# lijx10/DeepI2P

Measured on AMD Instinct MI355X. Metric: frames/sec (img+pc infer + 60-restart GN pose) KITTI 20k-pt, 1/2/4/8 GPU, higher is better.
Workload: dtype f32 network (fp32-input MFMA; 3x3 convolutions, GEMM-shaped point layers and the per-point head: bf16 MFMA on exact three-way fp32 splits, fp32 accumulation) + f64 solver

## Files before the change

### deepi2p_amd/_lib.py

```python
import ctypes
import os

import torch

_HERE = os.path.dirname(os.path.abspath(__file__))
LIB_PATH = os.environ.get("DI2P_LIB") or os.path.join(_HERE, "lib", "libdeepi2p_hip.so")
_lib = None

c_void_p, c_int, c_float, c_double, c_ll = ctypes.c_void_p, ctypes.c_int, ctypes.c_float, ctypes.c_double, ctypes.c_longlong


class DeepI2PHipError(RuntimeError):
    pass


class SrcT(ctypes.Structure):
    _fields_ = [("ptr", c_void_p), ("gidx", c_void_p), ("batch_stride", c_ll), ("row_stride", c_int),
                ("channels", c_int), ("mode", c_int), ("group", c_int), ("pad_", c_int)]


class EpilogueT(ctypes.Structure):
    _fields_ = [("scale", c_void_p), ("shift", c_void_p), ("batch_bias", c_void_p), ("relu", c_int),
                ("group_max", c_int), ("g_table", c_void_p * 2), ("g_idx", c_void_p * 2), ("g_w", c_void_p * 2),
                ("g_nodes", c_int * 2), ("g_k", c_int * 2), ("transpose_out", c_int), ("group_max_out", c_void_p),
                ("planes_out", c_void_p)]


class HeadX3T(ctypes.Structure):
    _fields_ = [("src", c_void_p * 2), ("batch_stride", c_ll * 2), ("row_stride", c_int * 2), ("channels", c_int * 2),
                ("W0p", c_void_p), ("W1p", c_void_p), ("scale_shift", c_void_p), ("relu0", c_int), ("relu1", c_int),
                ("tab", c_void_p * 2), ("idx", c_void_p * 2), ("w", c_void_p * 2), ("nodes", c_int * 2),
                ("W2t", c_void_p), ("scale2", c_void_p), ("shift2", c_void_p), ("relu2", c_int), ("P", c_int)]


class HeadLabelsX3T(ctypes.Structure):
    _fields_ = [("y0", c_void_p), ("batch_stride", c_ll), ("row_stride", c_int), ("K", c_int),
                ("W1p", c_void_p), ("scale1", c_void_p), ("shift1", c_void_p), ("relu1", c_int),
                ("W2p", c_void_p), ("scale2", c_void_p), ("shift2", c_void_p), ("P", c_int),
                ("scores", c_void_p), ("coarse", c_void_p), ("fine", c_void_p)]


class SampleOptT(ctypes.Structure):
    _fields_ = [("mode", c_int), ("crop_top", c_int), ("img_scale", c_double), ("img_H", c_int), ("img_W", c_int), ("Hs", c_int), ("Ws", c_int),
                ("amplitude", c_double * 6), ("color_range", c_double * 8)]
    dataset, crop_bottom, resize_k, max_range = 0, 0, 0, 0.0


SRC_DENSE, SRC_GATHER, SRC_GROUP = 0, 1, 2

_SIGS = {
    "di2p_index_max_forward": [c_void_p, c_void_p, c_void_p, c_int, c_int, c_int, c_int, c_void_p, c_void_p],
    "di2p_index_max_values": [c_void_p, c_void_p, c_void_p, c_void_p, c_void_p, c_int, c_int, c_int, c_int, c_void_p, c_void_p],
    "di2p_ball_query_forward": [c_void_p, c_void_p, c_float, c_int, c_int, c_int, c_int, c_void_p],
    "di2p_knn_nodes": [c_void_p, c_void_p, c_void_p, c_void_p, c_int, c_int, c_int, c_int, c_void_p],
    "di2p_cluster_stats": [c_void_p, c_void_p, c_int, c_void_p, c_void_p, c_void_p, c_int, c_int, c_int, c_void_p],
    "di2p_build_point_input": [c_void_p] * 7 + [c_int, c_int, c_int, c_void_p],
    "di2p_interpolate": [c_void_p] * 4 + [c_int] * 5 + [c_void_p],
    "di2p_gather_neighbors": [c_void_p] * 4 + [c_int] * 4 + [c_void_p],
    "di2p_argmax_channels": [c_void_p, c_void_p, c_int, c_int, c_int, c_ll, c_void_p],
    "di2p_pointwise_gemm": [ctypes.POINTER(SrcT), c_int, c_void_p, c_void_p, c_int, c_int, c_int, c_int,
                            ctypes.POINTER(EpilogueT), c_void_p],
    "di2p_pointwise_gemm_x3": [ctypes.POINTER(SrcT), c_int, c_void_p, c_void_p, c_int, c_int, c_int, c_int,
                               ctypes.POINTER(EpilogueT), c_void_p],
    "di2p_pointwise_gemm_x3p": [c_void_p, c_void_p, c_void_p, c_int, c_int, c_int, c_int, ctypes.POINTER(EpilogueT), c_void_p],
    "di2p_bf16x3_pack": [c_void_p, c_int, c_int, c_void_p, c_void_p],
    "di2p_bf16x3_pack_conv3x3": [c_void_p, c_int, c_int, c_int, c_void_p, c_void_p],
    "di2p_batch_gemv": [c_void_p, c_int, c_int, c_void_p, c_int, c_void_p, c_int, c_void_p],
    "di2p_batch_gemv2": [c_void_p, c_int, c_int, c_void_p, c_int, c_int, c_void_p, c_int, c_void_p, c_int, c_void_p],
    "di2p_attention_pool": [c_void_p, c_void_p, c_void_p, c_int, c_int, c_int, c_int, c_void_p],
    "di2p_point_head": [c_void_p, c_int, c_void_p, c_int, c_void_p, c_void_p, c_void_p, c_void_p, c_int, c_void_p, c_void_p,
                        c_void_p, c_int, c_void_p, c_int, c_int, c_int, c_int, c_void_p],
    "di2p_point_chain": [c_void_p, c_int, c_void_p, c_int, c_void_p, c_void_p, c_void_p, c_void_p, c_int, c_void_p, c_void_p,
                         c_void_p, c_int, c_void_p, c_int, c_int, c_int, c_void_p],
    "di2p_conv2d": [c_void_p] * 6 + [c_int] * 11 + [c_void_p],
    "di2p_conv2d_ws": [c_void_p] * 6 + [c_int] * 11 + [c_void_p, c_ll, c_void_p],
    "di2p_maxpool3x3s2": [c_void_p, c_void_p, c_int, c_int, c_int, c_int, c_void_p],
    "di2p_global_avgpool": [c_void_p, c_void_p, c_int, c_int, c_int, c_void_p],
    "di2p_channel_max": [c_void_p, c_void_p, c_int, c_int, c_int, c_void_p],
    "di2p_initial_guess": [c_void_p] * 5 + [c_int, c_int, c_void_p],
    "di2p_solve_batched": [c_void_p] * 6 + [c_double, c_double, ctypes.POINTER(c_double), ctypes.POINTER(c_double)]
                          + [c_int] * 5 + [c_void_p, c_void_p, c_void_p, c_void_p, c_void_p, c_void_p],
    "di2p_solve_batched_f32": [c_void_p] * 6 + [c_double, c_double, ctypes.POINTER(c_double), ctypes.POINTER(c_double)]
                              + [c_int] * 5 + [c_void_p, c_void_p, c_void_p, c_void_p, c_void_p, c_void_p],
    "di2p_select_best": [c_void_p, c_void_p, c_void_p, c_int, c_int, c_int, c_void_p, c_void_p, c_void_p, c_void_p],
    "di2p_solver_residuals": [c_void_p] * 4 + [c_double, c_double, c_int, c_int, c_int, c_void_p, c_void_p, c_void_p, c_void_p],
    "di2p_f32_to_f64": [c_void_p, c_void_p, c_ll, c_void_p],
    "di2p_farthest_point_sampling": [c_void_p, c_void_p, c_void_p, c_void_p, c_int, c_int, c_int, c_void_p],
    "di2p_gather_points": [c_void_p, c_void_p, c_void_p, c_int, c_int, c_int, c_int, c_void_p],
    "di2p_project_labels": [c_void_p, c_void_p, c_int, c_void_p, c_float, c_float, c_float, c_void_p, c_void_p, c_void_p, c_int, c_int, c_void_p],
    "di2p_label_accuracy": [c_void_p, c_void_p, c_void_p, c_void_p, c_void_p, c_int, c_int, c_void_p],
    "di2p_pnp_ransac": [c_void_p] * 5 + [c_int, c_void_p, c_int, c_double, c_int, c_int, c_int, c_int] + [c_void_p] * 7,
    "di2p_draw_restarts": [ctypes.c_ulonglong, c_int, c_int, c_double, c_double, c_void_p, c_void_p, c_void_p],
    "di2p_random_choice": [ctypes.c_ulonglong, c_int, c_int, c_int, c_int, c_void_p, c_void_p, c_void_p],
    "di2p_random_choice_ragged": [ctypes.c_ulonglong, c_int, c_int, c_void_p, c_int, c_int, c_void_p, c_void_p, c_void_p],
    "di2p_voxel_down_sample": [c_void_p, c_void_p, c_int, c_int, c_int, c_double, c_double, c_int] + [c_void_p] * 9,
    "di2p_estimate_normals": [c_void_p, c_int, c_int, c_double, c_int, c_double] + [c_void_p] * 5,
    "di2p_nearest_raw": [c_void_p, c_void_p, c_void_p, c_int, c_int, c_double] + [c_void_p] * 5,
    "di2p_gather_ragged": [c_void_p] * 6 + [c_int, c_int] + [c_void_p] * 4,
    "di2p_pnp_pack": [c_void_p] * 4 + [c_int, c_int, c_int] + [c_void_p] * 3,
    "di2p_pnp_ransac_epnp": [c_void_p] * 5 + [c_int, c_void_p, c_int, c_double, c_int, c_int] + [c_void_p] * 7,
    "di2p_classifier_loss": [c_void_p] * 4 + [c_int, c_int, c_int, c_float, c_float, c_float] + [c_void_p] * 5,
    "di2p_adam_step": [c_void_p] * 4 + [c_ll, c_int, c_float, c_float, c_float, c_float, c_void_p],
    "di2p_pack_pc_label": [c_void_p, c_void_p, c_void_p, c_void_p, c_void_p, c_void_p, c_int, c_int, c_void_p],
    "di2p_stem_pack": [c_void_p, c_void_p, c_void_p],
    "di2p_conv7x7s2_stem": [c_void_p] * 5 + [c_int] * 4 + [c_void_p],
    "di2p_winograd_weight_transform": [c_void_p, c_void_p, c_int, c_int, c_void_p],
    "di2p_winograd_weight_transform_dgrad": [c_void_p, c_void_p, c_int, c_int, c_void_p],
    "di2p_conv3x3_winograd": [c_void_p] * 6 + [c_int] * 6 + [c_void_p],
    "di2p_conv3x3_x3": [c_void_p] * 6 + [c_int] * 7 + [c_void_p] * 4 + [c_int, c_void_p],
    "di2p_conv3x3_x3_supported": [c_int] * 7,
    "di2p_conv3x3_x3_plan": [c_int] * 7 + [ctypes.POINTER(ctypes.c_int32)],
    "di2p_head_x3_pack": [c_void_p, c_int, c_void_p, c_void_p],
    "di2p_stem_x3_pack": [c_void_p, c_void_p, c_void_p],
    "di2p_stem_x3_supported": [c_int, c_int],
    "di2p_stem_x3": [c_void_p] * 5 + [c_int] * 3 + [c_void_p],
    "di2p_point_head_x3": [ctypes.POINTER(HeadX3T), c_void_p, c_int, c_int, c_void_p],
    "di2p_head_labels_x3_pack": [c_void_p, c_int, c_int, c_void_p, c_void_p],
    "di2p_point_head_labels_x3": [ctypes.POINTER(HeadLabelsX3T), c_int, c_int, c_void_p],
    "di2p_bn_train_forward": [c_void_p] * 9 + [c_float, c_float, c_int, c_int, c_int, c_int, c_void_p, c_void_p],
    "di2p_bn_train_backward": [c_void_p] * 6 + [c_int] + [c_void_p] * 4 + [c_int, c_int, c_int, c_void_p, c_void_p],
    "di2p_channel_sum": [c_void_p, c_void_p, c_int, c_int, c_int, c_void_p, c_void_p],
    "di2p_bmm_rc": [c_void_p, c_ll, c_ll, c_void_p, c_ll, c_ll, c_void_p, c_int, c_int, c_int, c_int, c_float, c_int, c_void_p, c_ll, c_void_p],
    "di2p_rc_vec_ok": [c_void_p, c_ll, c_ll, c_int],
    "di2p_rc_route": [c_int] * 7 + [ctypes.POINTER(ctypes.c_int32)],
    "di2p_pointwise_route": [c_int] * 6 + [ctypes.POINTER(ctypes.c_int32)],
    "di2p_conv2d_route": [c_int] * 12 + [c_ll, ctypes.POINTER(ctypes.c_int32)],
    "di2p_winograd_route": [c_int] * 5 + [ctypes.POINTER(ctypes.c_int32)],
    "di2p_point_chain_route": [c_int] * 6 + [ctypes.POINTER(ctypes.c_int32)],
    "di2p_point_head_route": [c_int] * 8 + [ctypes.POINTER(ctypes.c_int32)],
    "di2p_bmm_km": [c_void_p, c_int, c_ll, c_void_p, c_int, c_ll, c_void_p, c_int, c_int, c_int, c_int, c_float, c_void_p],
    "di2p_gather_backward": [c_void_p, c_void_p, c_void_p, c_int, c_void_p, c_int, c_int, c_int, c_int, c_void_p, c_ll, c_void_p],
    "di2p_conv2d_wgrad": [c_void_p] * 3 + [c_int] * 9 + [c_void_p, c_ll, c_void_p],
    "di2p_conv2d_dgrad": [c_void_p] * 3 + [c_int] * 9 + [c_void_p],
    "di2p_maxpool3x3s2_backward": [c_void_p] * 3 + [c_int] * 4 + [c_void_p],
    "di2p_segment_max_backward": [c_void_p] * 4 + [c_int] * 4 + [c_void_p],
    "di2p_group_max_forward": [c_void_p, c_void_p, c_void_p, c_ll, c_int, c_void_p],
    "di2p_group_max_backward": [c_void_p, c_void_p, c_void_p, c_ll, c_int, c_void_p],
    "di2p_dropout_mask": [ctypes.c_ulonglong, c_int, c_float, c_ll, c_void_p, c_void_p],
    "di2p_apply_mask": [c_void_p, c_void_p, c_float, c_void_p, c_ll, c_void_p],
    "di2p_sample_draws": [ctypes.c_ulonglong, c_void_p, c_int, c_int, ctypes.POINTER(SampleOptT)] + [c_void_p] * 10,
    "di2p_image_prepare": [c_void_p, c_int, c_int, c_int, ctypes.POINTER(SampleOptT), c_void_p, c_void_p, c_int, c_int, c_int, c_void_p, c_void_p,
                           c_void_p],
    "di2p_transform_segments": [c_void_p] * 4 + [c_int, c_int] + [c_void_p] * 3,
    "di2p_gather_ragged_aug": [c_void_p] * 6 + [c_int, c_int, ctypes.c_ulonglong, c_void_p, c_int, c_double, c_double] + [c_void_p] * 4,
    "di2p_random_choice_dseed": [c_void_p, c_int, c_int, c_int, c_int, c_void_p, c_void_p, c_void_p],
    "di2p_random_choice_ragged_dseed": [c_void_p, c_int, c_int, c_void_p, c_int, c_int, c_void_p, c_void_p, c_void_p],
    "di2p_range_shuffle": [c_void_p, c_void_p, c_int, c_int, c_int, c_double, ctypes.c_ulonglong] + [c_void_p] * 6,
    "di2p_gather_ragged_aug_intensity": [c_void_p] * 5 + [c_int, c_int, ctypes.c_ulonglong, c_void_p, c_int, c_double, c_double] + [c_void_p] * 3,
    "di2p_sample_draws_ds": [ctypes.c_ulonglong, c_void_p, c_int, c_int, ctypes.POINTER(SampleOptT), c_int] + [c_void_p] * 10,
    "di2p_image_prepare_ds": [c_void_p, c_int, c_int, c_int, ctypes.POINTER(SampleOptT), c_int, c_int, c_void_p, c_void_p, c_void_p, c_int, c_int,
                              c_void_p, c_void_p, c_void_p],
    "di2p_estimate_normals_cells": [c_void_p, c_int, c_int, c_double, c_int, c_double] + [c_void_p] * 5,
    "di2p_compose_poses": [c_void_p, c_void_p, c_int, c_void_p, c_void_p],
    "di2p_pose_errors": [c_void_p, c_void_p, c_int, c_void_p, c_int, c_int, c_double, c_double, c_void_p, c_void_p, c_void_p, c_void_p],
    "di2p_eval_accumulate": [c_void_p] * 5 + [c_int, c_void_p, c_void_p],
    "di2p_eval_acc_reset": [c_void_p, c_void_p],
    "di2p_enu2cam_points": [c_void_p, c_void_p, c_int, c_int, c_void_p],
    "di2p_vis_classification": [c_void_p] * 6 + [c_int] * 10 + [c_void_p] * 3,
    "di2p_vis_registration": [c_void_p] * 5 + [c_int] * 7 + [c_void_p] * 3,
    "di2p_submap_build": [c_void_p] * 6 + [c_int] * 5 + [c_double, c_double, c_int] + [c_void_p] * 7,
    "di2p_submap_to_camera": [c_void_p] * 4 + [c_int, c_int, c_void_p, c_void_p],
    "di2p_pose_matrices": [c_void_p, c_int, c_void_p, c_void_p],
    "di2p_sweep_transforms": [c_void_p] * 5 + [c_int, c_int] + [c_void_p] * 3,
    "di2p_sweep_accumulate": [c_void_p] * 4 + [c_int] * 6 + [c_float, c_float] + [c_void_p] * 6,
    "di2p_world_trace": [c_void_p, c_void_p, c_int, c_int, c_void_p, c_void_p, c_int, c_void_p, c_void_p, c_void_p],
    "di2p_world_render_camera": [c_void_p, c_void_p, c_int, c_int, c_void_p, c_void_p, c_int, c_int, c_double] + [c_void_p] * 4,
    "di2p_world_render_scan": [c_void_p, c_void_p, c_int, c_int, c_void_p, c_void_p, c_void_p, c_int, c_int] + [c_double] * 4
                              + [ctypes.c_ulonglong, c_void_p, c_int] + [c_void_p] * 5,
    "di2p_world_render_profiles": [c_void_p, c_void_p, c_int, c_int, c_void_p, c_void_p, c_void_p, c_int, c_int] + [c_double] * 4
# ... 24 lines not shown
    "di2p_world_workspace_bytes": [c_int, c_int],
    "di2p_world_profiles_workspace_bytes": [c_int, c_int],
    "di2p_pose_information_workspace_bytes": [c_int, c_int],
}
EXPORTS = sorted(list(_SIGS) + ["di2p_last_error", "di2p_version", "di2p_solve_workspace_bytes", "di2p_solver_set_profile_buffer", "di2p_pnp_workspace_bytes",
                 "di2p_conv2d_workspace_bytes", "di2p_set_option", "di2p_get_option", "di2p_random_choice_workspace_bytes", "di2p_classifier_loss_workspace_bytes", "di2p_normals_cells_candidates"] + list(_WS_SIGS))


def load():
    global _lib
    if _lib is None:
        if not os.path.exists(LIB_PATH):
            raise DeepI2PHipError(
                "libdeepi2p_hip.so not found at %s -- build it with `python -m deepi2p_amd.build` "
                "(there is no CPU fallback)" % LIB_PATH)
        lib = ctypes.CDLL(LIB_PATH)
        for name, args in _SIGS.items():
            fn = getattr(lib, name)
            fn.argtypes = args
            fn.restype = c_int
        lib.di2p_last_error.restype = ctypes.c_char_p
        lib.di2p_version.restype = c_int
        lib.di2p_solve_workspace_bytes.restype = c_ll
        lib.di2p_solve_workspace_bytes.argtypes = [c_int, c_int, c_int]
        lib.di2p_pnp_workspace_bytes.restype = c_ll
        lib.di2p_pnp_workspace_bytes.argtypes = [c_int, c_int, c_int]
        lib.di2p_conv2d_workspace_bytes.restype = c_ll
        lib.di2p_conv2d_workspace_bytes.argtypes = [c_int] * 10
        lib.di2p_classifier_loss_workspace_bytes.restype = c_ll
        lib.di2p_classifier_loss_workspace_bytes.argtypes = [c_int, c_int]
        lib.di2p_random_choice_workspace_bytes.restype = c_ll
        lib.di2p_random_choice_workspace_bytes.argtypes = [c_int, c_int]
        for name, args in _WS_SIGS.items():
            fn = getattr(lib, name)
            fn.argtypes = args
            fn.restype = c_ll
        lib.di2p_normals_cells_candidates.restype = c_int
        lib.di2p_normals_cells_candidates.argtypes = []
        lib.di2p_set_option.restype = c_int
        lib.di2p_set_option.argtypes = [ctypes.c_char_p, c_ll]
        lib.di2p_get_option.restype = c_ll
        lib.di2p_get_option.argtypes = [ctypes.c_char_p]
        lib.di2p_solver_set_profile_buffer.restype = None
        lib.di2p_solver_set_profile_buffer.argtypes = [c_void_p]
        _lib = lib
    return _lib


TIMED = None
TIMED_TAG = None
WORK = None


def call(name, *args):
    lib = load()
    rec = TIMED is not None and name in TIMED
    if rec:
        e0, e1 = torch.cuda.Event(enable_timing=True), torch.cuda.Event(enable_timing=True)
        e0.record()
    rc = getattr(lib, name)(*args)
    if rec:
        e1.record()
        TIMED[name].append((e0, e1, TIMED_TAG))
    if rc != 0:
        raise DeepI2PHipError("%s failed (%d): %s" % (name, rc, lib.di2p_last_error().decode()))


def set_option(name, value):
    if load().di2p_set_option(name.encode(), int(value)) != 0:
        raise DeepI2PHipError("unknown option " + name)


def get_option(name):
    return int(load().di2p_get_option(name.encode()))


class option:

    def __init__(self, name, value):
        self.name, self.value = name, value

    def __enter__(self):
        self.old = get_option(self.name)
        set_option(self.name, self.value)

    def __exit__(self, *exc):
        set_option(self.name, self.old)


def ptr(t):
    return None if t is None else t.data_ptr()


def stream():
    return torch.cuda.current_stream().cuda_stream


def require_cuda(*tensors):
    for t in tensors:
        if t is None:
            continue
        if not t.is_cuda:
            raise RuntimeError("tensor must be a CUDA tensor/variable")
        if not t.is_contiguous():
            raise RuntimeError("tensor must be contiguous")
```

### deepi2p_amd/csrc/common.h

```cpp
#pragma once
#include <hip/hip_runtime.h>
#include <stdint.h>
#include <stdio.h>

#include "../../include/deepi2p_hip.h"

#define DI2P_WAVE 64

void di2p_set_error(const char* fmt, ...);

#define DI2P_CHECK_ARG(cond, msg)                                   \
    do {                                                            \
        if (!(cond)) {                                              \
            di2p_set_error("%s: %s", __func__, msg);                \
            return -1;                                              \
        }                                                           \
    } while (0)

#define DI2P_RETURN_LAUNCH()                                                        \
    do {                                                                            \
        hipError_t e_ = hipGetLastError();                                          \
        if (e_ != hipSuccess) {                                                     \
            di2p_set_error("%s: launch failed: %s", __func__, hipGetErrorString(e_)); \
            return (int)e_;                                                         \
        }                                                                           \
        return 0;                                                                   \
    } while (0)

static inline int di2p_cdiv(long long a, long long b) { return (int)((a + b - 1) / b); }

#define DI2P_OPTIONS(X) \
    X(CONV_NOSPLIT, "conv_nosplit", "DI2P_CONV_NOSPLIT", 0)                        \
    X(CONV_DEPTH1, "conv_depth1", "DI2P_CONV_DEPTH1", 0)                           \
    X(PW_NOVEC, "pw_novec", "DI2P_PW_NOVEC", 0)                                    \
    X(SOLVER_NOCULL, "solver_nocull", "DI2P_SOLVER_NOCULL", 0)                     \
    X(SOLVER_NOPREFILTER, "solver_noprefilter", "DI2P_SOLVER_NOPREFILTER", 0)      \
    X(SOLVER_TIER_SWEEPS, "solver_tier_sweeps", "DI2P_SOLVER_TIER_SWEEPS", 0)      \
    X(WINO_COB, "wino_cob", "DI2P_WINO_COB", 0)                                    \
    X(CONV_NOWINOGRAD, "conv_nowinograd", "DI2P_CONV_NOWINOGRAD", 0)               \
    X(WINO_KC, "wino_kc", "DI2P_WINO_KC", 0)                                       \
    X(CONV_NOSTEM, "conv_nostem", "DI2P_CONV_NOSTEM", 0)                           \
    X(WINO_REG, "wino_reg", "DI2P_WINO_REG", 0)                                    \
    X(SOLVER_NOCACHE, "solver_nocache", "DI2P_SOLVER_NOCACHE", 0)                  \
    X(SOLVER_PREP_SINGLE, "solver_prep_single", "DI2P_SOLVER_PREP_SINGLE", 0)      \
    X(SOLVER_PREP_BITONIC, "solver_prep_bitonic", "DI2P_SOLVER_PREP_BITONIC", 0)   \
    X(PW_X3, "pw_x3", "DI2P_PW_X3", 1)                                             \
    X(PW_NOCHAIN, "pw_nochain", "DI2P_PW_NOCHAIN", 0)                              \
    X(HEAD_REG, "head_reg", "DI2P_HEAD_REG", 0)                                    \
    X(CONV_S2SCALAR, "conv_s2scalar", "DI2P_CONV_S2SCALAR", 0)                     \
    X(CONV_X3, "conv_x3", "DI2P_CONV_X3", 31)                                      \
    X(CONV_X3_CFG, "conv_x3_cfg", "DI2P_CONV_X3_CFG", -1)                          \
    X(HEAD_X3, "head_x3", "DI2P_HEAD_X3", 1)                                       \
    X(HEAD_X3_TAB, "head_x3_tab", "DI2P_HEAD_X3_TAB", 1)                           \
    X(STEM_X3, "stem_x3", "DI2P_STEM_X3", 1)                                       \
    X(BN_UNFUSED, "bn_unfused", "DI2P_BN_UNFUSED", 0)                              \
    X(PW_X3_PLANES, "pw_x3_planes", "DI2P_PW_X3_PLANES", 1)                        \
    X(CONV_DGRAD_DENSE, "conv_dgrad_dense", "DI2P_CONV_DGRAD_DENSE", 0)            \
    X(RC_TILE64, "rc_tile64", "DI2P_RC_TILE64", 0)
enum Di2pOption {
#define DI2P_OPT_ENUM(ID, NAME, ENV, DEF) DI2P_OPT_##ID,
    DI2P_OPTIONS(DI2P_OPT_ENUM)
#undef DI2P_OPT_ENUM
    DI2P_OPT_COUNT
};
long long di2p_opt(int id);
int di2p_cu_count();
int di2p_allow_dynamic_lds(const void* kernel, size_t bytes, const char* who);
void di2p_pack_a32(const float* Wt, int K, int M, int tiles, int tile_stride, int step_stride, void* Wp, void* stream);
```

### deepi2p_amd/csrc/gemm.hip

```cpp
#include "bf16x3.h"
#include "mfma_tile.h"

#include <stdint.h>
#include <stdlib.h>

namespace {

struct LoaderWt {
    const float* Wt;
    int K, M;
    __device__ __forceinline__ float load(int k, int m) const { return (k < K && m < M) ? Wt[k * M + m] : 0.0f; }
};

struct SrcDev {
    const float* ptr[DI2P_MAX_SRC];
    const int* gidx[DI2P_MAX_SRC];
    long long batch_stride[DI2P_MAX_SRC];
    int row_stride[DI2P_MAX_SRC];
    int c_end[DI2P_MAX_SRC];
    int mode[DI2P_MAX_SRC];
    int group[DI2P_MAX_SRC];
    int n_src;
};

// ... 400 lines not shown
    __syncthreads();
    {
        LoaderWt4 la{tl.W1t, HEAD_M, HEAD_M};
        EpiDev e1{};
        e1.scale = tl.sc1; e1.shift = tl.sh1; e1.relu = tl.relu1; e1.group_max = 1;
        EpiPointwise ep{e1, nullptr, b, HEAD_M, N};
        ep.lds_tile = hbuf; ep.lds_n0 = j_blk; ep.lds_ld = HEAD_BN;
        mfma_gemm_block_blds<HeadCfg>(stage, la, hbuf, HEAD_BN, ep, HEAD_M, 0, j_blk);
    }
    __syncthreads();
    const int lane = threadIdx.x & 63, p = threadIdx.x >> 6;
    const int n = j_blk + lane;
    if (p < tl.P) {
        float a = 0.0f;
        for (int k0 = 0; k0 < HEAD_M; k0 += 16) {
            float w[16], h[16];
#pragma unroll
            for (int u = 0; u < 16; ++u) { w[u] = tl.W2t[(k0 + u) * tl.P + p]; h[u] = hbuf[(k0 + u) * HEAD_BN + lane]; }
#pragma unroll
            for (int u = 0; u < 16; ++u) a = fmaf(w[u], h[u], a);
        }
        if (tl.sc2) a *= tl.sc2[p];
        if (tl.sh2) a += tl.sh2[p];
        if (tl.relu2) a = fmaxf(a, 0.0f);
        if (n < N) out[((long long)b * tl.P + p) * N + n] = a;
    }
}

struct ChainTail {
    const float* W1t;
    const float* sc1;
    const float* sh1;
    const float* W2t;
    const float* sc2;
    const float* sh2;
    int relu1, relu2;
};

__device__ __forceinline__ void chain_rows_to_ksteps(const float (&v)[16], float* f) {
#pragma unroll
    for (int g = 0; g < 4; ++g) {
        auto p = __builtin_amdgcn_permlane32_swap(__float_as_uint(v[4 * g + 0]), __float_as_uint(v[4 * g + 1]), false, false);
        auto q = __builtin_amdgcn_permlane32_swap(__float_as_uint(v[4 * g + 2]), __float_as_uint(v[4 * g + 3]), false, false);
        f[4 * g + 0] = __uint_as_float(p[0]);
        f[4 * g + 1] = __uint_as_float(q[0]);
        f[4 * g + 2] = __uint_as_float(p[1]);
        f[4 * g + 3] = __uint_as_float(q[1]);
    }
}

#ifndef DI2P_CHAIN_WAVES
#define DI2P_CHAIN_WAVES 2
#endif
template <int M, int KS0, int NL, int TN>
__global__ __launch_bounds__(256) __attribute__((amdgpu_waves_per_eu(DI2P_CHAIN_WAVES, 8))) void point_chain_kernel(const float* __restrict__ X, long long x_bs, int x_rs, const float* __restrict__ W0t,
                                                           int K0, EpiDev e0, ChainTail tl, float* __restrict__ Y, int N, int nblk, int total) {
    constexpr int TM = M / 32, KS = M / 2, KSMAX = KS0 > KS ? KS0 : KS;
    extern __shared__ __attribute__((aligned(16))) float lds[];
    float* w0 = lds;
    float* w1 = w0 + 2 * KS0 * M;
    float* w2 = w1 + M * M;
    float* ss = w2 + (NL == 3 ? M * M : 0);
    for (int i = threadIdx.x; i < 2 * KS0 * M; i += 256) w0[i] = i < K0 * M ? W0t[i] : 0.0f;
    for (int i = threadIdx.x; i < M * M; i += 256) w1[i] = tl.W1t[i];
    if (NL == 3)
        for (int i = threadIdx.x; i < M * M; i += 256) w2[i] = tl.W2t[i];
    {
        const float* rows[6] = {e0.scale, e0.shift, tl.sc1, tl.sh1, NL == 3 ? tl.sc2 : nullptr, NL == 3 ? tl.sh2 : nullptr};
#pragma unroll
        for (int q = 0; q < 6; ++q)
            if (rows[q] && threadIdx.x < M) ss[q * M + threadIdx.x] = rows[q][threadIdx.x];
    }
    __syncthreads();
    if (e0.scale) e0.scale = ss;
    if (e0.shift) e0.shift = ss + M;
    const int lane = threadIdx.x & 63, wave = __builtin_amdgcn_readfirstlane(threadIdx.x >> 6);
    const int l31 = lane & 31, half = lane >> 5;
    EpiDev e1{}, e2{};
    e1.scale = tl.sc1 ? ss + 2 * M : nullptr; e1.shift = tl.sh1 ? ss + 3 * M : nullptr; e1.relu = tl.relu1; e1.group_max = 1;
    e2.scale = tl.sc2 ? ss + 4 * M : nullptr; e2.shift = tl.sh2 ? ss + 5 * M : nullptr; e2.relu = tl.relu2; e2.group_max = 1;

    float fn[TN][KS0];
    auto request = [&](int g) {
        const int fb = g / nblk, blk = g - fb * nblk;
        const float* Xb = X + (long long)fb * x_bs;
#pragma unroll
        for (int s = 0; s < KS0; ++s) {
            const int k = 2 * s + half;
#pragma unroll
            for (int j = 0; j < TN; ++j) {
                const float x = Xb[(long long)min(k, K0 - 1) * x_rs + min((blk * TN + j) * 32 + l31, N - 1)];
                fn[j][s] = k < K0 ? x : 0.0f;
            }
        }
    };
    const int g0 = blockIdx.x * 4 + wave, stride = gridDim.x * 4;
    if (g0 < total) request(g0);
    for (int g = g0; g < total; g += stride) {
        const int b = g / nblk, blk = g - b * nblk;
        EpiPointwise ep0{e0, nullptr, b, M, N}, ep1{e1, nullptr, b, M, N}, ep2{e2, nullptr, b, M, N};
        int n[TN], nc[TN];
#pragma unroll
        for (int j = 0; j < TN; ++j) { n[j] = (blk * TN + j) * 32 + l31; nc[j] = min(n[j], N - 1); }
        float f[TN][KSMAX];
#pragma unroll
        for (int j = 0; j < TN; ++j)
#pragma unroll
            for (int s = 0; s < KS0; ++s) f[j][s] = fn[j][s];
        request(min(g + stride, total - 1));
        f32x16 acc[TM][TN];
        auto zero = [&]() {
#pragma unroll
            for (int i = 0; i < TM; ++i)
#pragma unroll
                for (int j = 0; j < TN; ++j)
#pragma unroll
                    for (int r = 0; r < 16; ++r) acc[i][j][r] = 0.0f;
        };
        auto layer = [&](const float* w, auto ks_tag) {
            constexpr int STEPS = decltype(ks_tag)::value;
            const float* wl = w + half * M + l31;
#pragma unroll
            for (int s = 0; s < STEPS; ++s) {
                float a[TM];
#pragma unroll
                for (int i = 0; i < TM; ++i) a[i] = wl[2 * s * M + i * 32];
#pragma unroll
                for (int i = 0; i < TM; ++i)
#pragma unroll
                    for (int j = 0; j < TN; ++j) acc[i][j] = __builtin_amdgcn_mfma_f32_32x32x2f32(a[i], f[j][s], acc[i][j], 0, 0, 0);
            }
        };
        auto to_operands = [&](const EpiPointwise& ep) {
#pragma unroll
            for (int j = 0; j < TN; ++j)
#pragma unroll
                for (int i = 0; i < TM; ++i) {
                    float v[16];
                    ep.apply(i * 32 + 4 * half, nc[j], acc[i][j], v);
                    chain_rows_to_ksteps(v, &f[j][i * 16]);
                }
        };
        auto to_memory = [&](const EpiPointwise& ep) {
#pragma unroll
            for (int j = 0; j < TN; ++j)
#pragma unroll
                for (int i = 0; i < TM; ++i) {
                    float v[16];
                    ep.apply(i * 32 + 4 * half, nc[j], acc[i][j], v);
                    if (n[j] < N) {
#pragma unroll
                        for (int r = 0; r < 16; ++r)
                            Y[((long long)b * M + i * 32 + 4 * half + (r & 3) + 8 * (r >> 2)) * N + n[j]] = v[r];
                    }
                }
        };
        zero();
        layer(w0, std::integral_constant<int, KS0>{});
        to_operands(ep0);
        zero();
        layer(w1, std::integral_constant<int, KS>{});
        if (NL == 3) {
// ... 145 lines not shown
    const float* score;
    int HW, Mn, n;
    bool valid;
    __device__ __forceinline__ void column(int j) { n = j; valid = j < Mn; }
    __device__ __forceinline__ void begin_tile(int) {}
    __device__ __forceinline__ float load(int k) const { return (valid && k < HW) ? score[(long long)k * Mn + n] : 0.0f; }
};
struct EpiMean {
    float* out;
    int C, Mn;
    float inv_div;
    __device__ __forceinline__ void tile(int mrow0, int n, const f32x16& acc) {
        if (n >= Mn) return;
#pragma unroll
        for (int r = 0; r < 16; ++r) {
            const int m = mrow0 + (r & 3) + 8 * (r >> 2);
            if (m < C) out[(long long)m * Mn + n] = acc[r] / inv_div;
        }
    }
};
template <class Cfg>
__global__ __launch_bounds__(Cfg::THREADS) void attention_pool_kernel(const float* __restrict__ feat, const float* __restrict__ score,
                                                                       float* __restrict__ out, int C, int HW, int Mn) {
    extern __shared__ float lds[];
    const int b = blockIdx.z;
    LoaderFeat la{feat + (long long)b * C * HW, HW, C};
    LoaderScore lb{score + (long long)b * HW * Mn, HW, Mn, 0, false};
    EpiMean ep{out + (long long)b * C * Mn, C, Mn, (float)HW};
    mfma_gemm_block<Cfg>(lds, la, lb, ep, HW, blockIdx.y * Cfg::BM, blockIdx.x * Cfg::BN);
}

__device__ __forceinline__ float gemv_slice(const float* __restrict__ Wt, int M, int mc, int k0, const float* __restrict__ vb, int Kv, int slice) {
    const int per = (Kv + 3) / 4;
    const int kb = slice * per, ke = min(kb + per, Kv);
    float a0 = 0.0f, a1 = 0.0f, a2 = 0.0f, a3 = 0.0f;
    int k = kb;
    for (; k + 3 < ke; k += 4) {
        a0 += Wt[(long long)(k0 + k) * M + mc] * vb[k];
        a1 += Wt[(long long)(k0 + k + 1) * M + mc] * vb[k + 1];
        a2 += Wt[(long long)(k0 + k + 2) * M + mc] * vb[k + 2];
        a3 += Wt[(long long)(k0 + k + 3) * M + mc] * vb[k + 3];
    }
    for (; k < ke; ++k) a0 += Wt[(long long)(k0 + k) * M + mc] * vb[k];
    return (a0 + a1) + (a2 + a3);
}

__global__ __launch_bounds__(256) void batch_gemv_kernel(const float* __restrict__ Wt, int M, int k0, const float* __restrict__ v,
                                                         int Kv, int k1, const float* __restrict__ v1, int Kv1,
                                                         float* __restrict__ out) {
    __shared__ float part[2][4][64];
    const int b = blockIdx.y;
    const int lane = threadIdx.x & 63, slice = threadIdx.x >> 6;
    const int m = blockIdx.x * 64 + lane;
    const int mc = min(m, M - 1);
    part[0][slice][lane] = gemv_slice(Wt, M, mc, k0, v + (long long)b * Kv, Kv, slice);
    if (v1) part[1][slice][lane] = gemv_slice(Wt, M, mc, k1, v1 + (long long)b * Kv1, Kv1, slice);
    __syncthreads();
    if (slice == 0 && m < M) {
        float r = (part[0][0][lane] + part[0][1][lane]) + (part[0][2][lane] + part[0][3][lane]);
        if (v1) r += (part[1][0][lane] + part[1][1][lane]) + (part[1][2][lane] + part[1][3][lane]);
        out[(long long)b * M + m] = r;
    }
}

template <class Cfg>
void launch_pw(const SrcDev& s, const float* Wt, float* Y, int B, int M, int K, int N, const EpiDev& e, hipStream_t st) {
    const dim3 grid(di2p_cdiv(N, Cfg::BN), di2p_cdiv(M, Cfg::BM), B);
    hipLaunchKernelGGL(pointwise_gemm_kernel<Cfg>, grid, dim3(Cfg::THREADS), Cfg::LDS_FLOATS * sizeof(float), st, s, Wt, Y, M, K, N, e);
}

template <class Cfg>
void launch_pw_vec(bool dense, bool d2, const SrcDev& s, const float* Wt, float* Y, int B, int M, int K, int N, const EpiDev& e, hipStream_t st) {
    const dim3 grid(di2p_cdiv(N, Cfg::BN), di2p_cdiv(M, Cfg::BM), B);
    if (dense && d2)
        hipLaunchKernelGGL((pointwise_gemm_vec_kernel<Cfg, true, true>), grid, dim3(Cfg::THREADS), Cfg::LDS_FLOATS * sizeof(float), st, s, Wt, Y, M, K, N, e);
    else if (dense)
        hipLaunchKernelGGL((pointwise_gemm_vec_kernel<Cfg, true>), grid, dim3(Cfg::THREADS), Cfg::LDS_FLOATS * sizeof(float), st, s, Wt, Y, M, K, N, e);
    else if (d2)
        hipLaunchKernelGGL((pointwise_gemm_vec_kernel<Cfg, false, true>), grid, dim3(Cfg::THREADS), Cfg::LDS_FLOATS * sizeof(float), st, s, Wt, Y, M, K, N, e);
    else
        hipLaunchKernelGGL((pointwise_gemm_vec_kernel<Cfg, false>), grid, dim3(Cfg::THREADS), Cfg::LDS_FLOATS * sizeof(float), st, s, Wt, Y, M, K, N, e);
}


constexpr int X3_BM = 128, X3_BN = 128, X3_BK = 32, X3_KG = X3_BK / 8;


__device__ __forceinline__ void x3_clear(f32x16 (&acc)[2][2]) {
#pragma unroll
    for (int i = 0; i < 2; ++i)
#pragma unroll
        for (int j = 0; j < 2; ++j)
#pragma unroll
            for (int r = 0; r < 16; ++r) acc[i][j][r] = 0.0f;
}

__device__ __forceinline__ void x3_aload(const u32x4_t* __restrict__ Wp, int Mp, int kg, int row, u32x4_t (&af)[2][3]) {
#pragma unroll
    for (int i = 0; i < 2; ++i) {
        const u32x4_t* p = Wp + ((long long)kg * Mp + row + i * 32) * 3;
#pragma unroll
        for (int q = 0; q < 3; ++q) af[i][q] = p[q];
    }
}

__device__ __forceinline__ void x3_bfrag(const u32x2_t* bq, int sub, int half, int n, u32x4_t (&bf)[2][3]) {
// ... 516 lines not shown
    const HeadRoute rt = head_route(K0, n_src, srcs[0].channels, reg_range, e.g_table[0] && e.g_table[1] && e.g_k[0] == 3 && e.g_k[1] == 3, B, N,
                                    di2p_cu_count());
    if (rt.reg) {
        constexpr int KS0 = 48;
        const int nblk = rt.nblk;
        const long long total = rt.total;
        DI2P_CHECK_ARG(total < (1ll << 30), "too many column blocks");
        const int wgs = rt.wgs;
        const size_t lds_reg = (size_t)(2 * KS0 * HEAD_M + HEAD_M * HEAD_M + HEAD_M * 4 + 4 * HEAD_M) * sizeof(float);
        if (rt.g33) {
            if (di2p_allow_dynamic_lds((const void*)point_head_reg_kernel<true, KS0>, lds_reg, __func__)) return -1;
            hipLaunchKernelGGL((point_head_reg_kernel<true, KS0>), dim3(wgs), dim3(512), lds_reg, (hipStream_t)stream, s, W0t, K0, e, tl, out, N, nblk, (int)total);
        } else {
            if (di2p_allow_dynamic_lds((const void*)point_head_reg_kernel<false, KS0>, lds_reg, __func__)) return -1;
            hipLaunchKernelGGL((point_head_reg_kernel<false, KS0>), dim3(wgs), dim3(512), lds_reg, (hipStream_t)stream, s, W0t, K0, e, tl, out, N, nblk, (int)total);
        }
        DI2P_RETURN_LAUNCH();
    }
    const size_t lds = (HeadCfg::LDS_FLOATS + HEAD_M * HEAD_BN) * sizeof(float);
    if (rt.g33) {
        if (di2p_allow_dynamic_lds((const void*)point_head_kernel<true>, lds, __func__)) return -1;
        hipLaunchKernelGGL(point_head_kernel<true>, dim3(di2p_cdiv(N, HEAD_BN), B), dim3(HeadCfg::THREADS), lds, (hipStream_t)stream, s, W0t, K0, e, tl, out, N);
    } else {
        if (di2p_allow_dynamic_lds((const void*)point_head_kernel<false>, lds, __func__)) return -1;
        hipLaunchKernelGGL(point_head_kernel<false>, dim3(di2p_cdiv(N, HEAD_BN), B), dim3(HeadCfg::THREADS), lds, (hipStream_t)stream, s, W0t, K0, e, tl, out, N);
    }
    DI2P_RETURN_LAUNCH();
}

extern "C" int di2p_point_chain(const di2p_src_t* srcs, int n_src, const float* W0t, int K0, const di2p_epilogue_t* epi0,
                                const float* W1t, const float* scale1, const float* shift1, int relu1, const float* W2t,
                                const float* scale2, const float* shift2, int relu2, float* Y, int B, int M, int N, void* stream) {
    DI2P_CHECK_ARG(srcs && n_src == 1 && W0t && W1t && epi0, "fused chain: one dense source");
    DI2P_CHECK_ARG(M == 32 || M == 64, "fused chain: width 32 or 64 (use the separate layers otherwise)");
    DI2P_CHECK_ARG(K0 <= M, "fused chain: at most M input channels");
    DI2P_CHECK_ARG(B >= 0 && N >= 1 && K0 >= 1, "bad size");
    DI2P_CHECK_ARG(epi0->group_max <= 1 && !epi0->transpose_out && !epi0->planes_out, "fused chain: layer 0 takes scale/shift/relu/bias/gathered only");
    if (B == 0) return 0;
    DI2P_CHECK_ARG(Y && srcs[0].ptr && srcs[0].channels == K0 && srcs[0].mode == DI2P_SRC_DENSE, "fused chain: one dense source of K0 channels");
    DI2P_CHECK_ARG((long long)srcs[0].channels * srcs[0].row_stride < (1ll << 31), "per-frame source extent must fit 31 bits");
    EpiDev e;
    if (pw_epilogue(__func__, epi0, nullptr, M, N, false, e)) return -1;
    ChainTail tl{W1t, scale1, shift1, W2t, scale2, shift2, relu1, relu2};
    const float* X = srcs[0].ptr;
    const long long x_bs = srcs[0].batch_stride;
    const int x_rs = (int)srcs[0].row_stride;
    hipStream_t st = (hipStream_t)stream;
    const ChainRoute rt = chain_route(M, K0, W2t != nullptr, B, N, di2p_cu_count());
    DI2P_CHECK_ARG(rt.total < (1ll << 30), "too many column blocks");
#define DI2P_CHAIN_LAUNCH(MM, KS0, NL, TN)                                                                                          \
    do {                                                                                                                            \
        const size_t lds = (size_t)(2 * (KS0) * (MM) + ((NL) - 1) * (MM) * (MM) + 6 * (MM)) * sizeof(float);                        \
        hipLaunchKernelGGL((point_chain_kernel<MM, KS0, NL, TN>), dim3(rt.wgs), dim3(256), lds, st, X, x_bs, x_rs, W0t, K0, e, tl, Y, N, \
                           rt.nblk, (int)rt.total);                                                                                 \
    } while (0)
    const bool three = rt.layers == 3;
    if (M == 32) {
        if (rt.ks0 == 4) { if (three) DI2P_CHAIN_LAUNCH(32, 4, 3, DI2P_CHAIN_TN32); else DI2P_CHAIN_LAUNCH(32, 4, 2, DI2P_CHAIN_TN32); }
        else             { if (three) DI2P_CHAIN_LAUNCH(32, 16, 3, DI2P_CHAIN_TN32); else DI2P_CHAIN_LAUNCH(32, 16, 2, DI2P_CHAIN_TN32); }
    } else {
        if (rt.ks0 == 16) { if (three) DI2P_CHAIN_LAUNCH(64, 16, 3, DI2P_CHAIN_TN64); else DI2P_CHAIN_LAUNCH(64, 16, 2, DI2P_CHAIN_TN64); }
        else              { if (three) DI2P_CHAIN_LAUNCH(64, 32, 3, DI2P_CHAIN_TN64); else DI2P_CHAIN_LAUNCH(64, 32, 2, DI2P_CHAIN_TN64); }
    }
#undef DI2P_CHAIN_LAUNCH
    DI2P_RETURN_LAUNCH();
}

extern "C" int di2p_point_chain_route(int M, int K0, int layers, int B, int N, int cus, int32_t* out) {
    DI2P_CHECK_ARG(out && (M == 32 || M == 64) && K0 >= 1 && K0 <= M && (layers == 2 || layers == 3) && B >= 1 && N >= 1 && cus >= 1, "bad args");
    const ChainRoute rt = chain_route(M, K0, layers == 3, B, N, cus);
    DI2P_CHECK_ARG(rt.total < (1ll << 30), "too many column blocks");
    out[0] = M; out[1] = rt.ks0; out[2] = rt.layers; out[3] = rt.tn; out[4] = rt.nblk; out[5] = (int)rt.total; out[6] = rt.wgs; out[7] = rt.w;
    return 0;
}

extern "C" int di2p_point_head_route(int K0, int n_src, int c0, int reg_range, int g33, int B, int N, int cus, int32_t* out) {
    DI2P_CHECK_ARG(out && K0 >= 1 && n_src >= 1 && n_src <= DI2P_MAX_SRC && c0 >= 1 && c0 <= K0 && B >= 1 && N >= 4 && N % 4 == 0 && cus >= 1, "bad args");
    const HeadRoute rt = head_route(K0, n_src, c0, reg_range != 0, g33 != 0, B, N, cus);
    DI2P_CHECK_ARG(!rt.reg || rt.total < (1ll << 30), "too many column blocks");
    out[0] = rt.reg; out[1] = rt.g33; out[2] = rt.bn; out[3] = rt.nblk; out[4] = (int)rt.total; out[5] = rt.wgs;
    return 0;
}

extern "C" int di2p_batch_gemv(const float* Wt, int M, int k0, const float* v, int Kv, float* out, int B, void* stream) {
    DI2P_CHECK_ARG(Wt && v && out && M >= 1 && Kv >= 1 && k0 >= 0 && B >= 0, "bad args");
    if (B == 0) return 0;
    hipLaunchKernelGGL(batch_gemv_kernel, dim3(di2p_cdiv(M, 64), B), dim3(256), 0, (hipStream_t)stream, Wt, M, k0, v, Kv, 0,
                       (const float*)nullptr, 0, out);
    DI2P_RETURN_LAUNCH();
}

extern "C" int di2p_batch_gemv2(const float* Wt, int M, int k0, const float* v0, int Kv0, int k1, const float* v1, int Kv1,
                                float* out, int B, void* stream) {
    DI2P_CHECK_ARG(Wt && v0 && v1 && out && M >= 1 && Kv0 >= 1 && Kv1 >= 1 && k0 >= 0 && k1 >= 0 && B >= 0, "bad args");
    if (B == 0) return 0;
    hipLaunchKernelGGL(batch_gemv_kernel, dim3(di2p_cdiv(M, 64), B), dim3(256), 0, (hipStream_t)stream, Wt, M, k0, v0, Kv0, k1, v1, Kv1, out);
    DI2P_RETURN_LAUNCH();
}

extern "C" int di2p_attention_pool(const float* feat, const float* score, float* out, int B, int C, int HW, int Mn, void* stream) {
    DI2P_CHECK_ARG(feat && score && out && B >= 0 && C >= 1 && HW >= 1 && Mn >= 1, "bad args");
    if (B == 0) return 0;
    using Cfg = Cfg64x64;
    hipLaunchKernelGGL(attention_pool_kernel<Cfg>, dim3(di2p_cdiv(Mn, Cfg::BN), di2p_cdiv(C, Cfg::BM), B), dim3(Cfg::THREADS),
                       Cfg::LDS_FLOATS * sizeof(float), (hipStream_t)stream, feat, score, out, C, HW, Mn);
    DI2P_RETURN_LAUNCH();
}
```

### deepi2p_amd/csrc/head_x3.hip

```cpp
#include <stdint.h>

#include <type_traits>

#include "bf16x3.h"
#include "common.h"

namespace {

using bf16x3::u32x4_t;
using bf16x3::f32x16;

constexpr int HX_M = 128, HX_TM = 4, HX_TROW = HX_M + 4;

struct HxArgs {
    const float* src[2]; long long src_bs[2]; int src_rs[2]; int c0, K0;
    const u32x4_t* W0p; const u32x4_t* W1p;
    const float* ss;
    const float* tab[2]; const int* idx[2]; const float* gw[2]; int nodes[2];
    const float* W2t; const float* sc2; const float* sh2;
    float* out;
    int relu0, relu1, relu2, P, N, nblk, total, parts;
};

template <bool TAB_LDS, int KS0, int NW, int MINW, bool SYNC, bool DEEP, bool LEAN = false>
__global__ __launch_bounds__(NW * 64, MINW) void point_head_x3_kernel(const HxArgs a) {
    extern __shared__ __attribute__((aligned(16))) float lds[];
    float* ssl = lds;
    float* w2l = ssl + 4 * HX_M;
    float* tabl = w2l + 4 * HX_M;
    const int tid = threadIdx.x, lane = tid & 63, wave = __builtin_amdgcn_readfirstlane(tid >> 6);
    const int nl = lane & 31, h = lane >> 5;
    for (int i = tid; i < 4 * HX_M; i += NW * 64) {
        ssl[i] = a.ss[i];
        w2l[i] = (i & 3) < a.P ? a.W2t[(i >> 2) * a.P + (i & 3)] : 0.0f;
    }
    int g_first, g_stride, g_end, fb_fixed = 0;
    if (TAB_LDS) {
        const int fb = blockIdx.x / a.parts, part = blockIdx.x - fb * a.parts;
        fb_fixed = fb;
#pragma unroll
        for (int t = 0; t < 2; ++t) {
            const float* T = a.tab[t] + (long long)fb * a.nodes[t] * HX_M;
            float* L = tabl + (t == 0 ? 0 : a.nodes[0] * HX_TROW);
            for (int i = tid; i < a.nodes[t] * (HX_M / 4); i += NW * 64) {
                const int node = i / (HX_M / 4), c4 = i - node * (HX_M / 4);
                *reinterpret_cast<float4*>(L + node * HX_TROW + 4 * c4) = *reinterpret_cast<const float4*>(T + node * HX_M + 4 * c4);
            }
        }
        g_first = fb * a.nblk + part * NW + wave; g_stride = a.parts * NW; g_end = (fb + 1) * a.nblk;
    } else {
        g_first = blockIdx.x * NW + wave; g_stride = gridDim.x * NW; g_end = a.total;
    }
    __syncthreads();
    const __amdgpu_buffer_rsrc_t w0r = __builtin_amdgcn_make_buffer_rsrc((void*)a.W0p, 0, (a.K0 / 16) * HX_TM * 3 * 1024, 0x00020000);
    const __amdgpu_buffer_rsrc_t w1r = __builtin_amdgcn_make_buffer_rsrc((void*)a.W1p, 0, (HX_M / 16) * HX_TM * 3 * 1024, 0x00020000);

    int gi_n[6];
    float gw_n[6], x_n[KS0][8];
    const int trips = SYNC ? (g_end - (g_first - wave) + g_stride - 1) / g_stride : 0;
    for (int it = 0, g0 = g_first; SYNC ? it < trips : g0 < g_end; ++it, g0 += g_stride) {
        const bool live = g0 < g_end;
        const int g = SYNC ? min(g0, g_end - 1) : g0;
        asm volatile("" ::: "memory");
        int hq = 4 * h;
        asm volatile("" : "+v"(hq));
        const int fb = TAB_LDS ? fb_fixed : __builtin_amdgcn_readfirstlane(g / a.nblk);
        const int n = (g - fb * a.nblk) * 32 + nl, nc = min(n, a.N - 1);
        auto request_nb = [&](int gg, int (&gi_)[6], float (&gw_)[6]) __attribute__((always_inline)) {
            const int fq = TAB_LDS ? fb_fixed : __builtin_amdgcn_readfirstlane(gg / a.nblk);
            const int nq = min((gg - fq * a.nblk) * 32 + nl, a.N - 1);
#pragma unroll
            for (int t = 0; t < 2; ++t)
#pragma unroll
// ... 124 lines not shown
            for (int q2 = 0; q2 < 2; ++q2)
#pragma unroll
                for (int j = 0; j < 4; ++j) {
                    float X = v[8 * q2 + j], Y = v[8 * q2 + 4 + j];
                    asm volatile("s_nop 1\n\tv_permlane32_swap_b32 %0, %1" : "+v"(X), "+v"(Y));
                    f1[2 * i + q2][j] = X;
                    f1[2 * i + q2][4 + j] = Y;
                }
        }
#pragma unroll
        for (int i = 0; i < HX_TM; ++i)
#pragma unroll
            for (int r = 0; r < 16; ++r) acc[i][r] = 0.0f;
        {
            u32x4_t bfr[2][3];
            bf16x3::split8(f1[0], bfr[0][0], bfr[0][1], bfr[0][2]);
#pragma unroll
            for (int s = 0; s < 2 * HX_TM; ++s) {
                __builtin_amdgcn_sched_barrier(0);
                if (s + 1 < 2 * HX_TM) bf16x3::split8(f1[s + 1], bfr[(s + 1) & 1][0], bfr[(s + 1) & 1][1], bfr[(s + 1) & 1][2]);
                kstep(s & 1, bfr[s & 1], w1r, s + 1 < 2 * HX_TM ? s + 1 : -1);
#pragma unroll
                for (int u = 0; u < 6 * HX_TM; ++u) { __builtin_amdgcn_sched_group_barrier(0x008, 1, 0); __builtin_amdgcn_sched_group_barrier(0x002, 3, 0); }
            }
            __builtin_amdgcn_sched_barrier(0);
        }
        __builtin_amdgcn_sched_barrier(0);
        {
            const int gn = min(g + g_stride, g_end - 1);
            request_nb(gn, gi_n, gw_n);
#pragma unroll
            for (int s = 0; s < KS0; ++s) x_load(gn, s, x_n[s]);
        }
        __builtin_amdgcn_sched_barrier(0);
        float part[4] = {0.0f, 0.0f, 0.0f, 0.0f};
#pragma unroll
        for (int i = 0; i < HX_TM; ++i)
#pragma unroll
            for (int gq = 0; gq < 4; ++gq) {
                if (gq & 1) __builtin_amdgcn_sched_barrier(0);
                const int row = 32 * i + 8 * gq + hq;
                const float4 sc = *reinterpret_cast<const float4*>(ssl + 2 * HX_M + row);
                const float4 sh = *reinterpret_cast<const float4*>(ssl + 3 * HX_M + row);
                float y[4] = {acc[i][4 * gq + 0] * sc.x + sh.x, acc[i][4 * gq + 1] * sc.y + sh.y, acc[i][4 * gq + 2] * sc.z + sh.z, acc[i][4 * gq + 3] * sc.w + sh.w};
#pragma unroll
                for (int j = 0; j < 4; ++j) {
                    if (a.relu1) y[j] = fmaxf(y[j], 0.0f);
                    const float4 w = *reinterpret_cast<const float4*>(w2l + 4 * (row + j));
                    part[0] = fmaf(w.x, y[j], part[0]); part[1] = fmaf(w.y, y[j], part[1]);
                    part[2] = fmaf(w.z, y[j], part[2]); part[3] = fmaf(w.w, y[j], part[3]);
                }
                if (LEAN) asm volatile("" : "+v"(part[0]), "+v"(part[1]), "+v"(part[2]), "+v"(part[3]));
            }
#pragma unroll
        for (int p = 0; p < 4; ++p) {
            const float other = __builtin_bit_cast(float, __builtin_amdgcn_ds_bpermute((lane ^ 32) * 4, __builtin_bit_cast(int, part[p])));
            float o = (hq ? other : part[p]) + (hq ? part[p] : other);
            if (p < a.P) {
                if (a.sc2) o *= a.sc2[p];
                if (a.sh2) o += a.sh2[p];
                if (a.relu2) o = fmaxf(o, 0.0f);
                if (n < a.N && hq == 0 && live) a.out[((long long)fb * a.P + p) * a.N + n] = o;
            }
        }
    }
}

__global__ __launch_bounds__(256) void pack_a32_kernel(const float* __restrict__ Wt, unsigned short* __restrict__ Wp, int K, int M, int tiles,
                                                       int tile_stride, int step_stride) {
    const long long t = (long long)blockIdx.x * 256 + threadIdx.x;
    const int ks = K / 16;
    if (t >= (long long)tiles * ks * 64) return;
    const int lane = (int)(t & 63), s = (int)((t >> 6) % ks), tile = (int)((t >> 6) / ks);
    const int row = 32 * tile + (lane & 31), k0 = 16 * s + 8 * (lane >> 5);
    unsigned short* d = Wp + (((long long)tile * tile_stride + (long long)s * step_stride) * 3 * 64 + lane) * 8;
#pragma unroll
    for (int e = 0; e < 8; ++e) {
        const float v = row < M ? Wt[(long long)(k0 + e) * M + row] : 0.0f;
        float pl[3];
        bf16x3::split(v, pl[0], pl[1], pl[2]);
#pragma unroll
        for (int p = 0; p < 3; ++p) d[p * 64 * 8 + e] = bf16x3::bits(pl[p]);
    }
}

}

void di2p_pack_a32(const float* Wt, int K, int M, int tiles, int tile_stride, int step_stride, void* Wp, void* stream) {
    hipLaunchKernelGGL(pack_a32_kernel, dim3(di2p_cdiv((long long)tiles * (K / 16) * 64, 256)), dim3(256), 0, (hipStream_t)stream, Wt,
                       (unsigned short*)Wp, K, M, tiles, tile_stride, step_stride);
}

extern "C" long long di2p_head_x3_packed_bytes(int K) { return K >= 16 && K % 16 == 0 ? (long long)(K / 16) * HX_TM * 3 * 1024 : 0; }

extern "C" int di2p_head_x3_pack(const float* Wt, int K, void* Wp, void* stream) {
    DI2P_CHECK_ARG(Wt && Wp && K >= 16 && K % 16 == 0, "needs K % 16 == 0 (and 128 output channels)");
    DI2P_CHECK_ARG(((uintptr_t)Wp & 15) == 0, "packed weights must be 16-byte aligned");
    di2p_pack_a32(Wt, K, HX_M, HX_TM, 1, HX_TM, Wp, stream);
    DI2P_RETURN_LAUNCH();
}

extern "C" int di2p_point_head_x3(const di2p_head_x3_t* hd, float* out, int B, int N, void* stream) {
    DI2P_CHECK_ARG(hd && out, "null pointer");
    DI2P_CHECK_ARG(B >= 0 && N >= 1, "bad size");
    DI2P_CHECK_ARG(hd->src[0] && hd->src[1] && hd->W0p && hd->W1p && hd->scale_shift && hd->W2t, "null operand");
    DI2P_CHECK_ARG(hd->channels[0] >= 16 && hd->channels[0] % 16 == 0 && hd->channels[1] >= 16 && hd->channels[1] % 16 == 0, "source channels must be multiples of 16");
    DI2P_CHECK_ARG(hd->P >= 1 && hd->P <= 4, "1..4 outputs");
    for (int t = 0; t < 2; ++t) DI2P_CHECK_ARG(hd->tab[t] && hd->idx[t] && hd->nodes[t] >= 1, "both gathered tables (3 neighbours each) are required");
    DI2P_CHECK_ARG(((uintptr_t)hd->W0p & 15) == 0 && ((uintptr_t)hd->W1p & 15) == 0 && ((uintptr_t)hd->tab[0] & 15) == 0 && ((uintptr_t)hd->tab[1] & 15) == 0 &&
                   ((uintptr_t)hd->scale_shift & 15) == 0, "16-byte alignment of the packed weights, the tables and the scale / shift rows");
    for (int t = 0; t < 2; ++t)
        DI2P_CHECK_ARG((long long)hd->channels[t] * hd->row_stride[t] * 4 < (1ll << 31), "per-frame source extent must fit 31 bits");
    if (B == 0) return 0;
    HxArgs a{};
    for (int t = 0; t < 2; ++t) {
        a.src[t] = hd->src[t]; a.src_bs[t] = hd->batch_stride[t]; a.src_rs[t] = hd->row_stride[t];
        a.tab[t] = hd->tab[t]; a.idx[t] = hd->idx[t]; a.gw[t] = hd->w[t]; a.nodes[t] = hd->nodes[t];
    }
    a.c0 = hd->channels[0]; a.K0 = hd->channels[0] + hd->channels[1];
    a.W0p = (const u32x4_t*)hd->W0p; a.W1p = (const u32x4_t*)hd->W1p; a.ss = hd->scale_shift;
    a.W2t = hd->W2t; a.sc2 = hd->scale2; a.sh2 = hd->shift2; a.out = out;
    a.relu0 = hd->relu0; a.relu1 = hd->relu1; a.relu2 = hd->relu2; a.P = hd->P; a.N = N;
    a.nblk = di2p_cdiv(N, 32); a.total = B * a.nblk;
    hipStream_t st = (hipStream_t)stream;
    const size_t lds_small = (size_t)8 * HX_M * sizeof(float);
    const size_t lds_tab = lds_small + (size_t)(hd->nodes[0] + hd->nodes[1]) * HX_TROW * sizeof(float);
    const long long opt = di2p_opt(DI2P_OPT_HEAD_X3_TAB);
    DI2P_CHECK_ARG(a.K0 == 96, "this build instantiates the head for 96 dense channels (32 + 64: first_pointnet + second_pointnet)");
    if (opt != 0 && lds_tab <= 160 * 1024) {
        const int cus = di2p_cu_count();
        int parts = di2p_cdiv(cus, B);
        while (parts > 1 && a.nblk < parts * 16) --parts;
        a.parts = parts;
        if (opt == 2) {
            if (di2p_allow_dynamic_lds((const void*)point_head_x3_kernel<true, 6, 4, 1, false, true>, lds_tab, __func__)) return -1;
            hipLaunchKernelGGL((point_head_x3_kernel<true, 6, 4, 1, false, true>), dim3(B * parts), dim3(256), lds_tab, st, a);
        } else {
            if (di2p_allow_dynamic_lds((const void*)point_head_x3_kernel<true, 6, 8, 2, false, false, true>, lds_tab, __func__)) return -1;
            hipLaunchKernelGGL((point_head_x3_kernel<true, 6, 8, 2, false, false, true>), dim3(B * parts), dim3(512), lds_tab, st, a);
        }
    } else {
        const int grid = (int)(a.total / 4 < 1ll * di2p_cu_count() ? di2p_cdiv(a.total, 4) : di2p_cu_count());
        hipLaunchKernelGGL((point_head_x3_kernel<false, 6, 4, 1, false, true>), dim3(grid), dim3(256), lds_small, st, a);
    }
    DI2P_RETURN_LAUNCH();
}
```

### deepi2p_amd/csrc/solver_aux.hip

```cpp
#include "common.h"
#include "pose_diff.h"
#include "solver_model.h"

namespace {

__global__ __launch_bounds__(64) void select_best_kernel(const double* __restrict__ params, const double* __restrict__ cost,
                                                         const int* __restrict__ has_inside, int np, int R, int* __restrict__ best,
                                                         double* __restrict__ P, double* __restrict__ best_cost) {
    const int f = blockIdx.x, lane = threadIdx.x;
    double bc = __builtin_inf();
    int bi = 0x7fffffff;
    for (int r = lane; r < R; r += 64) {
        const double c = cost[(long long)f * R + r];
        if (c < bc || (c == bc && r < bi)) { bc = c; bi = r; }
    }
#pragma unroll
    for (int o = 32; o > 0; o >>= 1) {
        const double oc = __shfl_xor(bc, o);
        const int oi = __shfl_xor(bi, o);
        if (oc < bc || (oc == bc && oi < bi)) { bc = oc; bi = oi; }
    }
    if (lane != 0) return;
    double* Pf = P + (long long)f * 16;
    for (int i = 0; i < 16; ++i) Pf[i] = (i % 5 == 0) ? 1.0 : 0.0;
    if (has_inside && has_inside[f] == 0) {
        best[f] = -1;
        best_cost[f] = 1e4;
        return;
    }
    if (bi == 0x7fffffff) bi = 0;
    params_to_pose(params + ((long long)f * R + bi) * np, np, Pf);
    best[f] = bi;
    best_cost[f] = cost[(long long)f * R + bi];
}

__global__ __launch_bounds__(1024) void initial_guess_kernel(const double* __restrict__ points, const int* __restrict__ labels,
                                                             double* __restrict__ yaw0, int* __restrict__ labels_out,
                                                             int* __restrict__ has_inside, int N) {
    __shared__ double s_a[1024], s_b[1024], s_c[1024];
    const int f = blockIdx.x, tid = threadIdx.x;
    const double* px = points + (long long)f * 3 * N;
    const double* pz = px + 2 * (long long)N;
    const int* lab = labels + (long long)f * N;
    double sx = 0, sz = 0, cnt = 0;
    for (int n = tid; n < N; n += 1024)
        if (lab[n] == 1) { sx += px[n]; sz += pz[n]; cnt += 1.0; }
    s_a[tid] = sx; s_b[tid] = sz; s_c[tid] = cnt;
    __syncthreads();
    for (int o = 512; o > 0; o >>= 1) {
        if (tid < o) { s_a[tid] += s_a[tid + o]; s_b[tid] += s_b[tid + o]; s_c[tid] += s_c[tid + o]; }
        __syncthreads();
    }
    const double count = s_c[0];
    const double mx = s_a[0] / count, mz = s_b[0] / count;
    __syncthreads();
    if (!(count > 0.0)) {
        if (tid == 0) { yaw0[f] = 0.0; has_inside[f] = 0; }
        for (int n = tid; n < N; n += 1024) labels_out[(long long)f * N + n] = lab[n];
        return;
    }
    const double kPi = 3.14159265358979323846;
    double a = fmod(atan2(mz, mx) - kPi / 2 + kPi, 2 * kPi);
    if (a < 0) a += 2 * kPi;
    a -= kPi;
    const double c = cos(a), s = sin(a);
    double zmin = __builtin_inf();
    for (int n = tid; n < N; n += 1024)
        if (lab[n] == 1) zmin = fmin(zmin, -s * px[n] + c * pz[n]);
    s_a[tid] = zmin;
    __syncthreads();
    for (int o = 512; o > 0; o >>= 1) {
        if (tid < o) s_a[tid] = fmin(s_a[tid], s_a[tid + o]);
        __syncthreads();
    }
    const double thr = s_a[0] - 10.0;
    for (int n = tid; n < N; n += 1024) {
        const double zr = -s * px[n] + c * pz[n];
        labels_out[(long long)f * N + n] = zr > thr ? lab[n] : -1;
    }
    if (tid == 0) { yaw0[f] = a; has_inside[f] = 1; }
}

template <int NP>
__global__ __launch_bounds__(256) void residuals_kernel(const double* __restrict__ points, const int* __restrict__ labels,
                                                        const double* __restrict__ Kmat, const double* __restrict__ params, double H,
                                                        double W, int N, double* __restrict__ residuals, int* __restrict__ counts,
                                                        double* __restrict__ cost_out) {
    __shared__ int s_scan[256];
    __shared__ double s_cost[256];
    __shared__ int s_base;
    const int f = blockIdx.x, tid = threadIdx.x;
    const double* px = points + (long long)f * 3 * N;
    const int* lab = labels + (long long)f * N;
    const double* Kf = Kmat + (long long)f * 9;
    const Cam k{Kf[0], Kf[4], Kf[2], Kf[5], H - 1.0, W - 1.0};
    const double* x = params + (long long)f * NP;
    double xr[NP];
    for (int i = 0; i < NP; ++i) xr[i] = x[i];
    Rot<NP> rot;
    make_rot<NP>(xr, rot);
    double* out = residuals + (long long)f * 3 * N;
    if (tid == 0) s_base = 0;
    double cost = 0.0;
    __syncthreads();
    for (int n0 = 0; n0 < N; n0 += 256) {
        const int n = n0 + tid;
        int nr = 0;
        double rv[3] = {0, 0, 0};
        if (n < N && (lab[n] == 0 || lab[n] == 1)) {
            const Proj p = project_point<NP>(rot, xr, k, px[n], px[N + n], px[2 * (long long)N + n]);
            nr = lab[n] == 1 ? 3 : 1;
            residual_rows<false>(lab[n], p.pix_x, p.pix_y, p.p2, k, rv);
            const double s = rv[0] * rv[0] + rv[1] * rv[1] + rv[2] * rv[2];
            cost += 0.5 * log1p(s);
            const double sq = sqrt(1.0 / (1.0 + s));
            for (int i = 0; i < 3; ++i) rv[i] *= sq;
        }
        s_scan[tid] = nr;
        __syncthreads();
        for (int o = 1; o < 256; o <<= 1) {
            const int v = tid >= o ? s_scan[tid - o] : 0;
            __syncthreads();
            s_scan[tid] += v;
            __syncthreads();
        }
        const int excl = s_scan[tid] - nr + s_base;
        for (int i = 0; i < nr; ++i) out[excl + i] = rv[i];
        __syncthreads();
        if (tid == 255) s_base += s_scan[255];
        __syncthreads();
// ... 191 lines not shown
    }
    status[f] = st;
    sigma_t[f] = sqrt(tr_t);
    sigma_r[f] = sqrt(tr_r) * (180.0 / 3.14159265358979323846);
}

__global__ __launch_bounds__(64) void restart_consensus_kernel(const double* __restrict__ params, const double* __restrict__ cost,
                                                               const int* __restrict__ best, const int* __restrict__ has_inside, int np, int R,
                                                               double t_tol, double r_tol_deg, int* __restrict__ finite_out,
                                                               int* __restrict__ agree_out, double* __restrict__ gap) {
    const int f = blockIdx.x, lane = threadIdx.x;
    const int b = best[f];
    if ((has_inside && has_inside[f] == 0) || b < 0 || b >= R) {
        if (lane == 0) { finite_out[f] = 0; agree_out[f] = 0; gap[f] = __builtin_nan(""); }
        return;
    }
    double G[16], A[16];
    params_to_pose(params + ((long long)f * R + b) * np, np, G);
    int n_finite = 0, n_agree = 0;
    double other = __builtin_inf();
    for (int r = lane; r < R; r += 64) {
        const double c = cost[(long long)f * R + r];
        if (!isfinite(c)) continue;
        n_finite += 1;
        params_to_pose(params + ((long long)f * R + r) * np, np, A);
        double t, ang;
        di2p_pose_diff(A, G, t, ang);
        if (t < t_tol && ang < r_tol_deg) n_agree += 1;
        else other = fmin(other, c);
    }
#pragma unroll
    for (int o = 32; o > 0; o >>= 1) {
        n_finite += __shfl_xor(n_finite, o);
        n_agree += __shfl_xor(n_agree, o);
        other = fmin(other, __shfl_xor(other, o));
    }
    if (lane == 0) { finite_out[f] = n_finite; agree_out[f] = n_agree; gap[f] = other - cost[(long long)f * R + b]; }
}

}

extern "C" int di2p_select_best(const double* params, const double* cost, const int32_t* has_inside, int is_2d, int F, int R,
                                int32_t* best, double* P, double* best_cost, void* stream) {
    DI2P_CHECK_ARG(params && cost && best && P && best_cost && F >= 0 && R >= 1, "bad args");
    if (F == 0) return 0;
    hipLaunchKernelGGL(select_best_kernel, dim3(F), dim3(64), 0, (hipStream_t)stream, params, cost, has_inside, is_2d ? 4 : 6, R, best, P, best_cost);
    DI2P_RETURN_LAUNCH();
}

extern "C" int di2p_initial_guess(const double* points, const int32_t* labels, double* yaw0, int32_t* labels_out,
                                  int32_t* has_inside, int F, int N, void* stream) {
    DI2P_CHECK_ARG(points && labels && yaw0 && labels_out && has_inside && F >= 0 && N >= 0, "bad args");
    if (F == 0) return 0;
    hipLaunchKernelGGL(initial_guess_kernel, dim3(F), dim3(1024), 0, (hipStream_t)stream, points, labels, yaw0, labels_out, has_inside, N);
    DI2P_RETURN_LAUNCH();
}

extern "C" int di2p_solver_residuals(const double* points, const int32_t* labels, const double* K, const double* params, double H,
                                     double W, int is_2d, int F, int N, double* residuals, int32_t* counts, double* cost,
                                     void* stream) {
    DI2P_CHECK_ARG(points && labels && K && params && residuals && counts && cost && F >= 0 && N >= 0, "bad args");
    if (F == 0) return 0;
    if (is_2d)
        hipLaunchKernelGGL(residuals_kernel<4>, dim3(F), dim3(256), 0, (hipStream_t)stream, points, labels, K, params, H, W, N, residuals, counts, cost);
    else
        hipLaunchKernelGGL(residuals_kernel<6>, dim3(F), dim3(256), 0, (hipStream_t)stream, points, labels, K, params, H, W, N, residuals, counts, cost);
    DI2P_RETURN_LAUNCH();
}

static int info_chunks(int N) { return N > 0 ? (N + INFO_CHUNK - 1) / INFO_CHUNK : 1; }

extern "C" long long di2p_pose_information_workspace_bytes(int F, int N) {
    if (F < 0 || N < 0) return 0;
    return (long long)F * info_chunks(N) * INFO_STRIDE * (long long)sizeof(double);
}

extern "C" int di2p_pose_information(const float* points, const int32_t* labels, const double* K, const double* params, double H, double W,
                                     int is_2d, int F, int N, double* info, double* grad, double* cost, int32_t* active, void* workspace,
                                     void* stream) {
    DI2P_CHECK_ARG(F >= 0 && N >= 0, "bad size");
    if (F == 0) return 0;
    DI2P_CHECK_ARG(points && labels && K && params && info && grad && cost && active && workspace, "null pointer");
    const int C = info_chunks(N);
    DI2P_CHECK_ARG(C <= 65535, "N too large");
    double* partial = (double*)workspace;
    if (is_2d) {
        hipLaunchKernelGGL(info_partial_kernel<4>, dim3(F, C), dim3(256), 0, (hipStream_t)stream, points, labels, K, params, H, W, N, C, partial);
        hipLaunchKernelGGL(info_finish_kernel<4>, dim3(F), dim3(64), 0, (hipStream_t)stream, (const double*)partial, C, info, grad, cost, active);
    } else {
        hipLaunchKernelGGL(info_partial_kernel<6>, dim3(F, C), dim3(256), 0, (hipStream_t)stream, points, labels, K, params, H, W, N, C, partial);
        hipLaunchKernelGGL(info_finish_kernel<6>, dim3(F), dim3(64), 0, (hipStream_t)stream, (const double*)partial, C, info, grad, cost, active);
    }
    DI2P_RETURN_LAUNCH();
}

extern "C" int di2p_gather_best_params(const double* params, const int32_t* best, int is_2d, int F, int R, double* out, void* stream) {
    DI2P_CHECK_ARG(F >= 0 && R >= 1, "bad size (F >= 0, R >= 1)");
    if (F == 0) return 0;
    DI2P_CHECK_ARG(params && best && out, "null pointer");
    const int np = is_2d ? 4 : 6;
    hipLaunchKernelGGL(gather_best_kernel, dim3(di2p_cdiv((long long)F * np, 64)), dim3(64), 0, (hipStream_t)stream, params, best, F, R, np, out);
    DI2P_RETURN_LAUNCH();
}

extern "C" int di2p_pose_covariance(const double* info, const double* params, const int32_t* has_inside, const double* lb_host,
                                    const double* ub_host, int is_2d, int F, double* cov, int32_t* free_mask, int32_t* status, double* sigma_t,
                                    double* sigma_r, void* stream) {
// ... 23 lines not shown
```

### deepi2p_amd/networks.py

```python
import torch
import torch.nn as nn

from . import _lib, ops
from .ops import Src

BN_EPS = 1e-5


class _Holder(nn.Module):
    pass


def _register(root, key, tensor, is_buffer):
    parts = key.split(".")
    mod = root
    for p in parts[:-1]:
        if p not in mod._modules:
            mod.add_module(p, _Holder())
        mod = mod._modules[p]
    if is_buffer:
        mod.register_buffer(parts[-1], tensor)
    else:
        mod.register_parameter(parts[-1], nn.Parameter(tensor, requires_grad=False))

# ... 129 lines not shown
    return x


def _run_split_pn(dense_srcs, dense_rows, node_feats, node_rows, idx, layers, N):
    Wt, scale, shift, act = layers[0]
    M = Wt.shape[1]
    B = node_feats.shape[0]
    head = (Wt[dense_rows[0]:dense_rows[1]], scale, shift, act)
    chain = [head] + list(layers[1:])
    if ops.point_chain_ok(dense_srcs, chain, N):
        G = ops.pointwise_gemm([Src(node_feats)], Wt[node_rows[0]:node_rows[1]], M, node_feats.shape[2], transpose_out=True)
        return ops.point_chain(dense_srcs, chain, N, gathered=[(G, idx.reshape(B, N, 1), None)])
    x = _run_split_layer(dense_srcs, dense_rows, node_feats, node_rows, idx, layers[0], N)
    return _run_pn(x, layers[1:])


class PCEncoder(_PackedModule):
    def __init__(self, opt, Ca: int, Cb: int, Cg: int, prefix=""):
        super().__init__()
        self.opt, self.Ca, self.Cb, self.Cg = opt, Ca, Cb, Cg
        spec = (_pn_spec("first_pointnet", 7, [Ca // 2] * 3, True)
                + _pn_spec("second_pointnet", Ca, [Ca, Ca], True)
                + _c2d_spec("knnlayer.layers_before.0", 3 + Ca, Cb) + _c2d_spec("knnlayer.layers_before.1", Cb, Cb)
                + _c2d_spec("knnlayer.layers_after.0", 2 * Cb, 2 * Cb) + _c2d_spec("knnlayer.layers_after.1", 2 * Cb, Cb)
                + _pn_spec("final_pointnet", 3 + Cb, [Cg // 2, Cg], True))
        _materialise(self, spec)

    def _pack(self):
        if self._packed is None:
            sd = self._sd()
            p = {"first": _pn_pack(sd, "first_pointnet"), "second": _pn_pack(sd, "second_pointnet"),
                 "final": _pn_pack(sd, "final_pointnet")}
            for name in ("layers_before.0", "layers_before.1", "layers_after.0", "layers_after.1"):
                q = "knnlayer." + name
                p[name] = _fold(sd, q + ".conv", q + ".norm")
            self._packed = p
        return self._packed

    def _group_index(self, B, Mb, K, device):
        key = (B, Mb, K, str(device))
        cache = self.__dict__.setdefault("_gidx_cache", {})
        if key not in cache:
            cache[key] = (torch.arange(Mb * K, dtype=torch.int32, device=device) // K).unsqueeze(0).expand(B, -1).contiguous()
            torch.cuda.current_stream().synchronize()
        return cache[key]

    def forward_device(self, pc, intensity, sn, node_a, node_b):
        if pc.size(2) != self.opt.input_pt_num:
            raise RuntimeError("N must equal opt.input_pt_num (the reference bakes it in, networks_pc.py:44-45)")
        p = self._pack()
        B, N, Ma, Mb = pc.size(0), pc.size(2), node_a.size(2), node_b.size(2)
        idx_a, w_a = ops.knn_nodes(pc, node_a, self.opt.k_interp_point_a, want_weights=True)
        cluster_mean, mask, min_idx = ops.cluster_stats(pc, idx_a, Ma)
        pc_centers, aug = ops.build_point_input(pc, intensity, sn, cluster_mean, min_idx)
        first = _run_pn(aug, p["first"])
        _, first_max = ops.index_max(first, min_idx, Ma, return_values=True, mask=mask)
        Ch = first.shape[1]
        second = _run_split_pn([Src(first)], (0, Ch), first_max, (Ch, 2 * Ch), min_idx, p["second"], N)
        _, node_a_features = ops.index_max(second, min_idx, Ma, return_values=True, mask=mask)
        K = self.opt.k_ab
        knn_I = ops.knn_nodes(node_b, cluster_mean, K)
        coord = ops.gather_neighbors(cluster_mean, node_b, knn_I)
        y = _run_split_layer([Src(coord)], (0, 3), node_a_features, (3, 3 + node_a_features.shape[1]), knn_I.view(B, Mb * K),
                             p["layers_before.0"], Mb * K)
        pow2 = K & (K - 1) == 0 and K <= 32
        Cb1 = p["layers_before.1"][0].shape[1]
        pl = [pow2 and ops.x3_planes_link(p["layers_before.1"], p["layers_after.0"][0][Cb1:2 * Cb1], B, Mb * K),
              pow2 and ops.x3_planes_link(p["layers_after.0"], p["layers_after.1"][0], B, Mb * K)]
        if pow2:
            y, fmax = _run_layer([Src(y)], p["layers_before.1"], Mb * K, group_max=K, also_full=True, planes_out=pl[0])
            Cb = y.shape[1]
        else:
            y = _run_layer([Src(y)], p["layers_before.1"], Mb * K)
            Cb = y.shape[1]
            fmax = ops.channel_max(y.view(B, Cb * Mb, K)).view(B, Cb, Mb)
        y = _run_split_layer([y if pl[0] else Src(y)], (Cb, 2 * Cb), fmax, (0, Cb), self._group_index(B, Mb, K, pc.device), p["layers_after.0"], Mb * K,
                             planes_out=pl[1])
        if pow2:
            node_b_features = _run_layer([y if pl[1] else Src(y)], p["layers_after.1"], Mb * K, group_max=K)
        else:
            y = _run_layer([Src(y)], p["layers_after.1"], Mb * K)
            node_b_features = ops.channel_max(y.view(B, y.shape[1] * Mb, K)).view(B, y.shape[1], Mb)
        final = _run_layer([Src(node_b), Src(node_b_features)], p["final"][0], Mb)
        final = _run_pn(final, p["final"][1:])
        global_feature = ops.channel_max(final).unsqueeze(2)
        ref_tuple = (pc_centers, cluster_mean, idx_a, first, second, node_a_features, node_b_features, global_feature)
        return ref_tuple, dict(w_a=w_a, min_idx=min_idx, mask=mask, knn_I=knn_I)

    def forward(self, pc, intensity, sn, node_a, node_b):
        t, _ = self.forward_device(pc, intensity, sn, node_a, node_b)
        return t[0], t[1], t[2].long(), t[3], t[4], t[5], t[6], t[7]


def _block_conv3x3(blk, n, x, stride, residual=None):
    Wt, sc, sh, _ = blk["c" + n]
    Cout = Wt.shape[1]
    kernel, cfg = ops.conv_route(x.shape, (Cout, x.shape[1], 3, 3), stride, 1)
    if kernel == "x3" and stride == 2:
        _, sd_, shd, _ = blk["ds"]
        return ops.conv3x3_x3(x, blk["X" + n], Cout, sc, sh, 2, True, downsample=(blk["Xd"], sd_, shd), cfg=cfg)
    if kernel == "x3":
        return ops.conv3x3_x3(x, blk["X" + n], Cout, sc, sh, 1, True, residual=residual, cfg=cfg), None
    if kernel == "winograd":
        return ops.conv3x3_winograd(x, blk["U" + n], sc, sh, True, residual=residual), None
    return ops.conv2d(x, Wt, sc, sh, 3, 3, stride, 1, True, residual=residual, tap_major=True), None


class ImageEncoder(_PackedModule):
# ... 63 lines not shown
                identity = x
                if "ds" in blk:
                    Wd, sd_, shd, _ = blk["ds"]
                    identity = ops.conv2d(x, Wd, sd_, shd, 1, 1, blk["stride"], 0, False, tap_major=True)
            x, _ = _block_conv3x3(blk, "2", y, 1, identity)
            if blk["last_of_stage"]:
                stage_out[blk["stage"]] = x
        return stage_out[3], stage_out[4], ops.global_avgpool(stage_out[4])


class KeypointDetector(_PackedModule):
    fuse_head = True

    def __init__(self, opt):
        super().__init__()
        self.opt = opt
        self.pc_encoder = PCEncoder(opt, Ca=64, Cb=256, Cg=512)
        self.img_encoder = ImageEncoder(opt)
        self.H_fine_res = int(round(opt.img_H / opt.img_fine_resolution_scale))
        self.W_fine_res = int(round(opt.img_W / opt.img_fine_resolution_scale))
        L = self.H_fine_res * self.W_fine_res
        spec = (_pn_spec("node_b_attention_pn", 256 + 512, [256, L], False)
                + _pn_spec("node_b_pn", 256 + 512 + 512 + 512, [1024, 512, 512], False)
                + _pn_spec("node_a_attention_pn", 64 + 512, [256, L * 4], False)
                + _pn_spec("node_a_pn", 64 + 256 + 512, [512, 128, 128], False))
        if opt.is_fine_resolution:
            spec += _pn_spec("per_point_pn", 736, [256, 256, 2 + L], False)
        else:
            spec += _pn_spec("per_point_pn", 736, [128, 128, 2], False)
        _materialise(self, spec)

    def _pack(self):
        if self._packed is None:
            sd = {k: v for k, v in self.state_dict().items() if not k.startswith(("pc_encoder.", "img_encoder."))}
            p = {n: _pn_pack(sd, n) for n in ("node_b_attention_pn", "node_b_pn", "node_a_attention_pn", "node_a_pn", "per_point_pn")}
            Wt = p["node_b_pn"][0][0]
            p["node_b_pn_dense_Wt"] = torch.cat((Wt[0:256], Wt[768:1280]), dim=0).contiguous()
            l0, l1, l2 = p["per_point_pn"]
            if (l0[0].is_cuda and tuple(l0[0].shape) == (736, 128) and tuple(l1[0].shape) == (128, 128) and l2[0].shape[0] == 128
                    and l2[0].shape[1] <= 4 and not l0[0].requires_grad):
                ones = torch.ones(128, device=l0[0].device)
                p["head_x3"] = {"W0p": ops.head_x3_pack(l0[0][640:736].contiguous()), "W1p": ops.head_x3_pack(l1[0]),
                                "ss": torch.stack((l0[1] if l0[1] is not None else ones, l0[2], l1[1] if l1[1] is not None else ones, l1[2])).contiguous(),
                                "relu0": l0[3], "relu1": l1[3], "W2t": l2[0], "sc2": l2[1], "sh2": l2[2], "relu2": l2[3]}
            if (l0[0].is_cuda and l0[0].shape[1] == 256 and tuple(l1[0].shape) == (256, 256) and l2[0].shape[0] == 256 and l2[0].shape[1] >= 3
                    and not l2[3] and not l0[0].requires_grad):
                p["head_labels_x3"] = {"W1p": ops.head_labels_pack(l1[0]), "W2p": ops.head_labels_pack(l2[0]), "P": int(l2[0].shape[1]),
                                       "sc1": l1[1] if l1[1] is not None else torch.ones(256, device=l1[0].device), "sh1": l1[2],
                                       "relu1": l1[3], "sc2": l2[1], "sh2": l2[2]}
            self._packed = p
        return self._packed

    def forward(self, pc, intensity, sn, node_a, node_b, img):
        p, B, N, first, second, idx_a, idx_pb, gathered = self._trunk(pc, intensity, sn, node_a, node_b, img)
        Wt, sc, sh, act = p["per_point_pn"][0]
        M0 = Wt.shape[1]
        G_a, ex_w_a = gathered[0][0], gathered[0][2]
        G_b, w_pb = gathered[1][0], gathered[1][2]
        l1, l2 = p["per_point_pn"][1], p["per_point_pn"][2]
        if ("head_x3" in p and self.fuse_head and _lib.get_option("head_x3") and first.shape[1] == 32 and second.shape[1] == 64
                and idx_a.shape[-1] == 3 and idx_pb.shape[-1] == 3):
            scores = ops.point_head_x3(first, second, p["head_x3"],
                                       [(G_a, idx_a.reshape(B, N, 3), ex_w_a), (G_b, idx_pb.reshape(B, N, 3), w_pb)], N)
        elif M0 == 128 and l1[0].shape[1] == 128 and l2[0].shape[1] <= 4 and N % 4 == 0 and self.fuse_head:
            scores = ops.point_head([Src(first), Src(second)], (Wt[640:736], sc, sh, act), l1, l2, N, gathered=gathered)
        else:
            h = ops.pointwise_gemm([Src(first), Src(second)], Wt[640:736], M0, N, scale=sc, shift=sh, relu=act, gathered=gathered)
            scores = _run_pn(h, p["per_point_pn"][1:], x3=False if M0 == 128 else None)
        coarse = scores[:, 0:2, :]
        if self.opt.is_fine_resolution:
            return coarse, scores[:, 2:, :]
        return coarse

    def predict_labels(self, pc, intensity, sn, node_a, node_b, img, scores_out=None):
        if not self.opt.is_fine_resolution:
            return ops.argmax_channels(self.forward(pc, intensity, sn, node_a, node_b, img)), None
        p, B, N, first, second, idx_a, idx_pb, gathered = self._trunk(pc, intensity, sn, node_a, node_b, img)
        Wt, sc, sh, act = p["per_point_pn"][0]
        M0 = Wt.shape[1]
        h = ops.pointwise_gemm([Src(first), Src(second)], Wt[640:736], M0, N, scale=sc, shift=sh, relu=act, gathered=gathered)
        if "head_labels_x3" not in p:
            raise RuntimeError("predict_labels: the fine head has no labels-only kernel for per_point_pn %s"
                               % [tuple(l[0].shape) for l in p["per_point_pn"]])
        return ops.point_head_labels(h, p["head_labels_x3"], N, scores_out=scores_out)

    def _trunk(self, pc, intensity, sn, node_a, node_b, img):
        ops.require_cuda(pc, intensity, sn, node_a, node_b, img)
        p = self._pack()
        B, N, Ma, Mb = pc.size(0), pc.size(2), node_a.size(2), node_b.size(2)
        (pc_center, cluster_mean, idx_a, first, second, node_a_features, node_b_features, global_feature), ex = \
            self.pc_encoder.forward_device(pc, intensity, sn, node_a, node_b)
        s16, s32, iglob = self.img_encoder(img)
        s16f = s16.view(B, s16.size(1), -1)
        s32f = s32.view(B, s32.size(1), -1)
        ig = iglob.view(B, -1)
        gf = global_feature.view(B, -1)

        Wt, sc, sh, act = p["node_b_attention_pn"][0]
        h = ops.pointwise_gemm([Src(node_b_features)], Wt[0:256], Wt.shape[1], Mb, scale=sc, shift=sh, relu=act,
                               batch_bias=ops.batch_gemv(Wt, 256, ig))
        score_b = _run_pn(h, p["node_b_attention_pn"][1:])
        w_s32 = ops.attention_pool(s32f, score_b)
        Wt, sc, sh, act = p["node_b_pn"][0]
        bias = ops.batch_gemv2(Wt, 256, gf, 1280, ig)
        h = ops.pointwise_gemm([Src(node_b_features), Src(w_s32)], p["node_b_pn_dense_Wt"], Wt.shape[1], Mb,
                               scale=sc, shift=sh, relu=act, batch_bias=bias)
        up_b = _run_pn(h, p["node_b_pn"][1:])
        idx_pb, w_pb = ops.knn_nodes(pc, node_b, self.opt.k_interp_point_b, want_weights=True)
        Wt, sc, sh, act = p["node_a_attention_pn"][0]
        h = ops.pointwise_gemm([Src(node_a_features)], Wt[0:64], Wt.shape[1], Ma, scale=sc, shift=sh, relu=act,
                               batch_bias=ops.batch_gemv(Wt, 64, ig))
        score_a = _run_pn(h, p["node_a_attention_pn"][1:])
        w_s16 = ops.attention_pool(s16f, score_a)
        idx_ab, w_ab = ops.knn_nodes(node_a, node_b, self.opt.k_interp_ab, want_weights=True)
        interp_ab = ops.interpolate(up_b, idx_ab, w_ab)
        h = _run_layer([Src(node_a_features), Src(interp_ab), Src(w_s16)], p["node_a_pn"][0], Ma)
        up_a = _run_pn(h, p["node_a_pn"][1:])
        Wt, sc, sh, act = p["per_point_pn"][0]
        M0 = Wt.shape[1]
        G_a = ops.pointwise_gemm([Src(up_a)], Wt[0:128], M0, Ma, transpose_out=True)
        G_b = ops.pointwise_gemm([Src(up_b)], Wt[128:640], M0, Mb, transpose_out=True)
        gathered = [(G_a, idx_a, ex["w_a"]), (G_b, idx_pb, w_pb)]
        return p, B, N, first, second, idx_a, idx_pb, gathered

    def intermediates(self, pc, intensity, sn, node_a, node_b, img):
        p = self._pack()
        B, N, Ma, Mb = pc.size(0), pc.size(2), node_a.size(2), node_b.size(2)
        t, ex = self.pc_encoder.forward_device(pc, intensity, sn, node_a, node_b)
        s16, s32, iglob = self.img_encoder(img)
        return dict(pc_center=t[0], cluster_mean=t[1], a_min_k_idx=t[2], first_pn_out=t[3], second_pn_out=t[4],
                    node_a_features=t[5], node_b_features=t[6], global_feature=t[7], s16=s16, s32=s32, img_global=iglob,
                    w_a=ex["w_a"], knn_I=ex["knn_I"])


def model_state_dict_convert_auto(sd):
    if len(sd) and all(k.startswith("module.") for k in sd):
        return {k[len("module."):]: v for k, v in sd.items()}
    return sd


class MMClassifer:

    fine = True

    def __init__(self, opt, writer=None):
        self.opt = opt
        self.writer = writer
        opt.is_fine_resolution = self.fine if not hasattr(opt, "is_fine_resolution") else opt.is_fine_resolution
        self.device = getattr(opt, "device", torch.device("cuda", 0))
        self.detector = KeypointDetector(opt).to(self.device).eval()
        self.pc = self.intensity = self.sn = self.node_a = self.node_b = self.P = self.img = self.K = None

    def load_model(self, model_path):
        self.detector.load_state_dict(model_state_dict_convert_auto(torch.load(model_path, map_location="cpu")))

    def set_input(self, pc, intensity, sn, node_a, node_b, P, img, K):
        def put(name, t):
            cur = getattr(self, name)
            if cur is None or cur.shape != t.shape or cur.dtype != t.dtype:
                cur = torch.empty(t.shape, dtype=t.dtype, device=self.device)
                setattr(self, name, cur)
            cur.copy_(t, non_blocking=True)
        for n, t in (("pc", pc), ("intensity", intensity), ("sn", sn), ("node_a", node_a), ("node_b", node_b),
                     ("P", P), ("img", img), ("K", K)):
            put(n, t)

    def forward(self, pc, intensity, sn, node_a, node_b, img):
        return self.detector(pc, intensity, sn, node_a, node_b, img)

    def _trainer(self):
        if getattr(self, "_trainer_obj", None) is None:
            from .training import ClassifierTrainer
            self._trainer_obj = ClassifierTrainer(self.detector, self.opt, lr=self._lr())
        return self._trainer_obj

    def _lr(self):
        if getattr(self, "old_lr_detector", None) is None:
            self.old_lr_detector = float(getattr(self.opt, "lr", 1e-3))
        return self.old_lr_detector

    def save_network(self, network, save_filename):
        import os
        save_path = os.path.join(getattr(self.opt, "checkpoints_dir", "."), save_filename)
        torch.save({k: v.detach().clone().cpu() for k, v in network.state_dict().items()}, save_path)

    def update_learning_rate(self, ratio):
        lr_detector = max(self._lr() * ratio, 0.00001)
        if getattr(self, "_trainer_obj", None) is not None:
            self._trainer_obj.adam.lr = lr_detector
        print('update detector learning rate: %f -> %f' % (self.old_lr_detector, lr_detector))
        self.old_lr_detector = lr_detector

    def _record(self, L, prefix):
        setattr(self, prefix + "_loss_dict", {"loss": L["loss"], "coarse": L["coarse"], "fine": L["fine"]})
        setattr(self, prefix + "_accuracy", {"coarse_accuracy": L["coarse_accuracy"], "fine_accuracy": L["fine_accuracy"]})

    def optimize(self):
        self.detector.train()
        self._record(self._trainer().optimize(self.pc, self.intensity, self.sn, self.node_a, self.node_b, self.img, self.K, self.P), "train")

    def test_model(self):
        self._record(self._trainer().test_model(self.pc, self.intensity, self.sn, self.node_a, self.node_b, self.img, self.K, self.P), "test")
        self.detector.eval()

    def inference_labels(self):
        out = self.forward(self.pc, self.intensity, self.sn, self.node_a, self.node_b, self.img)
        return ops.argmax_channels(out[0] if self.opt.is_fine_resolution else out)

    def inference_labels_fine(self):
        return self.detector.predict_labels(self.pc, self.intensity, self.sn, self.node_a, self.node_b, self.img)

    def inference_pass(self):
        out = self.forward(self.pc, self.intensity, self.sn, self.node_a, self.node_b, self.img)
        if self.opt.is_fine_resolution:
            coarse, fine = out
            return ops.argmax_channels(coarse).long(), ops.argmax_channels(fine).long()
        return ops.argmax_channels(out).long()


class MMClassiferCoarse(MMClassifer):

    fine = False

    def __init__(self, opt, writer=None):
        opt.is_fine_resolution = False
        super().__init__(opt, writer)
```

### deepi2p_amd/ops.py

```python
import ctypes
import weakref

import torch

from . import _lib
from ._lib import EpilogueT, SrcT, call, ptr, require_cuda, stream

_f32, _i32, _f64 = torch.float32, torch.int32, torch.float64
MAX_GK = 16


def _chk(t, dtype, name):
    if t.dtype != dtype:
        raise RuntimeError("%s must be %s, got %s" % (name, dtype, t.dtype))


def _work(name, macs):
    if _lib.WORK is not None:
        _lib.WORK[name] = _lib.WORK.get(name, 0) + macs


def index_max(data, index, K, return_values=False, mask=None):
    require_cuda(data, index, mask)
    _chk(data, _f32, "data")
# ... 322 lines not shown
        e.planes_out = ptr(Y.t)
        if group_max > 1:
            Ymax = torch.empty((B, M, Nout), dtype=_f32, device=Wt.device)
            e.group_max_out = ptr(Ymax)
        y_ptr = None
    elif also_full and group_max > 1:
        Y = torch.empty((B, M, N), dtype=_f32, device=Wt.device)
        Ymax = torch.empty((B, M, Nout), dtype=_f32, device=Wt.device)
        e.group_max_out = ptr(Ymax)
        y_ptr = ptr(Y)
    else:
        Y = torch.empty((B, Nout, M) if transpose_out else (B, M, Nout), dtype=_f32, device=Wt.device)
        y_ptr = ptr(Y)
    if Wp is not None:
        _work("di2p_pointwise_gemm_x3", B * M * K * N)
        if from_planes:
            call("di2p_pointwise_gemm_x3p", ptr(srcs[0].t), ptr(Wp), y_ptr, B, M, K, N, ctypes.byref(e), stream())
        else:
            call("di2p_pointwise_gemm_x3", arr, len(srcs), ptr(Wp), y_ptr, B, M, K, N, ctypes.byref(e), stream())
        return (Y, Ymax) if Ymax is not None else Y
    _work("di2p_pointwise_gemm", B * M * K * N)
    call("di2p_pointwise_gemm", arr, len(srcs), ptr(Wt), ptr(Y), B, M, K, N, ctypes.byref(e), stream())
    return (Y, Ymax) if Ymax is not None else Y


def point_head(srcs, layer0, layer1, layer2, N, batch_bias=None, gathered=None):
    Wt0, sc0, sh0, act0 = layer0
    Wt1, sc1, sh1, act1 = layer1
    Wt2, sc2, sh2, act2 = layer2
    B = srcs[0].t.shape[0]
    M, P = Wt0.shape[1], Wt2.shape[1]
    require_cuda(Wt0, Wt1, Wt2, sc0, sh0, sc1, sh1, sc2, sh2, batch_bias)
    e = EpilogueT()
    e.scale, e.shift, e.batch_bias = ptr(sc0), ptr(sh0), ptr(batch_bias)
    e.relu, e.group_max, e.transpose_out = int(bool(act0)), 1, 0
    _fill_gathered(e, gathered, B, M, N)
    out = torch.empty((B, P, N), dtype=_f32, device=Wt0.device)
    _work("di2p_point_head", B * N * (Wt0.shape[0] * M + M * M + M * P))
    call("di2p_point_head", _fill_srcs(srcs), len(srcs), ptr(Wt0), Wt0.shape[0], ctypes.byref(e), ptr(Wt1), ptr(sc1), ptr(sh1),
         int(bool(act1)), ptr(Wt2), ptr(sc2), ptr(sh2), int(bool(act2)), ptr(out), B, M, P, N, stream())
    return out


def head_x3_pack(Wt):
    require_cuda(Wt)
    K, M = Wt.shape
    if M != 128 or K % 16 or not Wt.is_contiguous():
        raise RuntimeError("head_x3_pack needs a contiguous f32[K,128] with K % 16 == 0")
    Wp = torch.empty((_lib.load().di2p_head_x3_packed_bytes(K),), dtype=torch.uint8, device=Wt.device)
    call("di2p_head_x3_pack", ptr(Wt), K, ptr(Wp), stream())
    return Wp


def point_head_x3(src0, src1, packed, gathered, N):
    require_cuda(src0, src1, packed["W0p"], packed["W1p"], packed["ss"], packed["W2t"], packed["sc2"], packed["sh2"])
    B = src0.shape[0]
    P = packed["W2t"].shape[1]
    k0 = int(src0.shape[1]) + int(src1.shape[1])
    hb = _lib.load().di2p_head_x3_packed_bytes
    if k0 % 16 or packed["W0p"].numel() * packed["W0p"].element_size() != hb(k0) or packed["W1p"].numel() * packed["W1p"].element_size() != hb(128):
        raise RuntimeError("point_head_x3: W0p / W1p must be head_x3_pack of the [%d,128] dense rows and of the [128,128] second layer" % k0)
    for name, n in (("ss", 4 * 128), ("W2t", 128 * P), ("sc2", P), ("sh2", P)):
        if packed[name] is None and name in ("sc2", "sh2"):
            continue
        _chk(packed[name], _f32, "point_head_x3 " + name)
        if packed[name].numel() < n:
            raise RuntimeError("point_head_x3: %s holds %d values, needs %d" % (name, packed[name].numel(), n))
    if tuple(packed["W2t"].shape) != (128, P) or not 1 <= P <= 4:
        raise RuntimeError("point_head_x3: W2t must be f32[128,P] with P <= 4")
    h = _lib.HeadX3T()
    for t, x in enumerate((src0, src1)):
        _chk(x, _f32, "head source")
        if x.dim() != 3 or x.shape[2] != N or x.stride(2) != 1:
            raise RuntimeError("head sources must be [B, ch, N] with unit column stride")
        h.src[t], h.batch_stride[t], h.row_stride[t], h.channels[t] = ptr(x), x.stride(0), x.stride(1), x.shape[1]
    for t, (tab, gi, gw) in enumerate(gathered):
        require_cuda(tab, gi, gw)
        _chk(tab, _f32, "gathered table")
        _chk(gi, _i32, "gathered index")
        if tuple(tab.shape[0::2]) != (B, 128) or tuple(gi.shape) != (B, N, 3) or (gw is not None and tuple(gw.shape) != (B, N, 3)):
            raise RuntimeError("the head takes node tables [B,nodes,128] with three neighbours per point")
        h.tab[t], h.idx[t], h.w[t], h.nodes[t] = ptr(tab), ptr(gi), ptr(gw), tab.shape[1]
    h.W0p, h.W1p, h.scale_shift = ptr(packed["W0p"]), ptr(packed["W1p"]), ptr(packed["ss"])
    h.relu0, h.relu1, h.relu2, h.P = int(bool(packed["relu0"])), int(bool(packed["relu1"])), int(bool(packed["relu2"])), P
    h.W2t, h.scale2, h.shift2 = ptr(packed["W2t"]), ptr(packed["sc2"]), ptr(packed["sh2"])
    out = torch.empty((B, P, N), dtype=_f32, device=src0.device)
    _work("di2p_point_head_x3", B * N * ((src0.shape[1] + src1.shape[1]) * 128 + 128 * 128 + 128 * P))
    call("di2p_point_head_x3", ctypes.byref(h), ptr(out), B, N, stream())
    return out


def head_labels_pack(Wt):
    require_cuda(Wt)
    _chk(Wt, _f32, "head_labels_pack weights")
    if Wt.dim() != 2 or Wt.shape[0] % 16 or Wt.shape[0] < 16:
        raise RuntimeError("head_labels_pack needs a contiguous f32[K,M] with K % 16 == 0")
    K, M = int(Wt.shape[0]), int(Wt.shape[1])
    Wp = torch.empty((_lib.load().di2p_head_labels_x3_packed_bytes(K, M),), dtype=torch.uint8, device=Wt.device)
    call("di2p_head_labels_x3_pack", ptr(Wt), K, M, ptr(Wp), stream())
    return Wp


def point_head_labels(y0, packed, N, scores_out=None):
    require_cuda(y0, packed["W1p"], packed["W2p"], packed["sc1"], packed["sh1"], packed["sc2"], packed["sh2"], scores_out)
    _chk(y0, _f32, "point_head_labels y0")
    P = int(packed["P"])
    if y0.dim() != 3 or y0.shape[1] != 256 or y0.shape[2] != N or y0.stride(2) != 1:
        raise RuntimeError("point_head_labels: y0 must be f32[B,256,N] with unit column stride")
    B = int(y0.shape[0])
    hb = _lib.load().di2p_head_labels_x3_packed_bytes
    if P < 3 or packed["W1p"].numel() * packed["W1p"].element_size() != hb(256, 256) or packed["W2p"].numel() * packed["W2p"].element_size() != hb(256, P):
        raise RuntimeError("point_head_labels: W1p / W2p must be head_labels_pack of the [256,256] layer 1 and of the [256,%d] layer 2 (P >= 3)" % P)
    for name, n in (("sc1", 256), ("sh1", 256), ("sc2", P), ("sh2", P)):
        if packed[name] is None:
            if name in ("sc2", "sh2"):
                continue
            raise RuntimeError("point_head_labels: %s is required" % name)
        _chk(packed[name], _f32, "point_head_labels " + name)
        if packed[name].numel() != n:
            raise RuntimeError("point_head_labels: %s holds %d values, needs %d" % (name, packed[name].numel(), n))
    if scores_out is not None:
        _chk(scores_out, _f32, "point_head_labels scores_out")
        if tuple(scores_out.shape) != (B, P, N) or scores_out.device != y0.device:
            raise RuntimeError("point_head_labels: scores_out must be f32[%d,%d,%d] on the device of y0" % (B, P, N))
    h = _lib.HeadLabelsX3T()
    h.y0, h.batch_stride, h.row_stride, h.K = ptr(y0), y0.stride(0), y0.stride(1), 256
    h.W1p, h.scale1, h.shift1, h.relu1 = ptr(packed["W1p"]), ptr(packed["sc1"]), ptr(packed["sh1"]), int(bool(packed["relu1"]))
    h.W2p, h.scale2, h.shift2, h.P = ptr(packed["W2p"]), ptr(packed["sc2"]), ptr(packed["sh2"]), P
    coarse = torch.empty((B, N), dtype=_i32, device=y0.device)
    fine = torch.empty((B, N), dtype=_i32, device=y0.device)
    h.scores, h.coarse, h.fine = ptr(scores_out), ptr(coarse), ptr(fine)
    _work("di2p_point_head_labels_x3", B * N * 256 * (256 + P))
    call("di2p_point_head_labels_x3", ctypes.byref(h), B, N, stream())
    return coarse, fine


def point_chain_ok(srcs, layers, N):
    if len(layers) not in (2, 3) or len(srcs) != 1 or _lib.get_option("pw_nochain"):
        return False
    M = layers[0][0].shape[1]
    if M not in (32, 64) or layers[0][0].shape[0] > M or any(tuple(l[0].shape) != (M, M) for l in layers[1:]):
        return False
    if any(l[0].requires_grad or not l[0].is_contiguous() for l in layers):
        return False
    return srcs[0].mode == _lib.SRC_DENSE and srcs[0].t.stride(2) == 1


def point_chain(srcs, layers, N, batch_bias=None, gathered=None):
    Wt0, sc0, sh0, act0 = layers[0]
    Wt1, sc1, sh1, act1 = layers[1]
    Wt2, sc2, sh2, act2 = layers[2] if len(layers) == 3 else (None, None, None, False)
    B = srcs[0].t.shape[0]
    M = Wt0.shape[1]
    require_cuda(Wt0, Wt1, Wt2, sc0, sh0, sc1, sh1, sc2, sh2, batch_bias)
    e = EpilogueT()
    e.scale, e.shift, e.batch_bias = ptr(sc0), ptr(sh0), ptr(batch_bias)
    e.relu, e.group_max, e.transpose_out = int(bool(act0)), 1, 0
    _fill_gathered(e, gathered, B, M, N)
    out = torch.empty((B, M, N), dtype=_f32, device=Wt0.device)
    _work("di2p_point_chain", B * N * (Wt0.shape[0] * M + (len(layers) - 1) * M * M))
    call("di2p_point_chain", _fill_srcs(srcs), len(srcs), ptr(Wt0), Wt0.shape[0], ctypes.byref(e), ptr(Wt1), ptr(sc1), ptr(sh1),
         int(bool(act1)), ptr(Wt2), ptr(sc2), ptr(sh2), int(bool(act2)), ptr(out), B, M, N, stream())
    return out


def batch_gemv(Wt, k0, v):
    require_cuda(Wt, v)
    B, Kv = v.shape
    M = Wt.shape[1]
    out = torch.empty((B, M), dtype=_f32, device=Wt.device)
    call("di2p_batch_gemv", ptr(Wt), M, int(k0), ptr(v), Kv, ptr(out), B, stream())
    return out


def batch_gemv2(Wt, k0, v0, k1, v1):
    require_cuda(Wt, v0, v1)
    B = v0.shape[0]
    M = Wt.shape[1]
    out = torch.empty((B, M), dtype=_f32, device=Wt.device)
    call("di2p_batch_gemv2", ptr(Wt), M, int(k0), ptr(v0), v0.shape[1], int(k1), ptr(v1), v1.shape[1], ptr(out), B, stream())
    return out


def attention_pool(feat, score):
    require_cuda(feat, score)
    B, C, HW = feat.shape
    Mn = score.shape[2]
    out = torch.empty((B, C, Mn), dtype=_f32, device=feat.device)
    call("di2p_attention_pool", ptr(feat), ptr(score), ptr(out), B, C, HW, Mn, stream())
    return out


def _conv_operands(who, x, Cout, KH, KW, stride, pad, scale, shift, residual):
    _chk(x, _f32, who + " input")
    if x.dim() != 4:
        raise RuntimeError("%s takes x f32[B,Cin,H,W]" % who)
    B, Cin, H, W = x.shape
    OH, OW = (H + 2 * pad - KH) // stride + 1, (W + 2 * pad - KW) // stride + 1
    for name, v in (("scale", scale), ("shift", shift)):
        if v is None or v.dtype != _f32:
            raise RuntimeError("%s %s must be %s, got %s" % (who, name, _f32, None if v is None else v.dtype))
        if v.numel() < Cout:
            raise RuntimeError("%s: %s holds %d values, needs %d" % (who, name, v.numel(), Cout))
    if residual is not None:
        _chk(residual, _f32, who + " residual")
        if residual.shape != (B, Cout, OH, OW):
            raise RuntimeError("%s: residual must be f32%s, got %s" % (who, (B, Cout, OH, OW), tuple(residual.shape)))
    return B, Cin, H, W, OH, OW


def conv_route(x_shape, w_shape, stride, pad, training=False):
    B, Cin, H, W = x_shape
    Cout, _, KH, KW = w_shape
    if KH == KW == 3 and pad == 1 and Cin % 16 == 0 and stride in (1, 2):
        bit = 4 if stride == 2 else max(0, min(3, int(Cout).bit_length() - 7))
        wanted = not training or (stride == 1 and (B >= 16 or Cout >= 256))
        if wanted and _lib.get_option("conv_x3") >> bit & 1 and conv3x3_x3_supported(x_shape, Cout, stride):
            small = training and B < 16 and _lib.get_option("conv_x3_cfg") < 0 and conv3x3_x3_supported(x_shape, Cout, stride, cfg=3)
            return "x3", 3 if small else -1
        if stride == 1 and Cout % 32 == 0 and W % 2 == 0 and W >= 4 and (training or not _lib.get_option("conv_nowinograd")):
            return "winograd", None
    return ("direct_tap" if Cin % 16 == 0 else "direct"), None


def conv2d(x, Wt, scale, shift, KH, KW, stride, pad, relu, residual=None, tap_major=False):
    require_cuda(x, Wt, scale, shift, residual)
    _chk(Wt, _f32, "conv2d Wt")
    Cout = Wt.shape[-1]
    B, Cin, H, W, OH, OW = _conv_operands("conv2d", x, Cout, KH, KW, stride, pad, scale, shift, residual)
    if tuple(Wt.shape) != (KH * KW * Cin, Cout):
        raise RuntimeError("conv2d: Wt must be f32[KH*KW*Cin, Cout] = [%d, %d], got %s" % (KH * KW * Cin, Cout, tuple(Wt.shape)))
    y = torch.empty((B, Cout, OH, OW), dtype=_f32, device=x.device)
    args = (ptr(x), ptr(Wt), ptr(scale), ptr(shift), ptr(residual), ptr(y), B, Cin, H, W, Cout, KH, KW,
            stride, pad, int(bool(relu)), int(bool(tap_major)))
# ... 161 lines not shown
    require_cuda(w)
    U = torch.empty((16, Cin, Cout), dtype=_f32, device=w.device)
    call("di2p_winograd_weight_transform", ptr(w), ptr(U), Cin, Cout, stream())
    return U


def winograd_weights_dgrad(weight):
    Cout, Cin, KH, KW = weight.shape
    if (KH, KW) != (3, 3) or weight.dtype != _f32:
        raise RuntimeError("winograd_weights_dgrad needs an f32 3x3 filter bank")
    w = weight.detach().contiguous()
    require_cuda(w)
    U = torch.empty((16, Cout, Cin), dtype=_f32, device=w.device)
    call("di2p_winograd_weight_transform_dgrad", ptr(w), ptr(U), Cout, Cin, stream())
    return U


def conv3x3_winograd(x, U, scale, shift, relu, residual=None):
    require_cuda(x, U, scale, shift, residual)
    _chk(U, _f32, "conv3x3_winograd U")
    Cout = U.shape[-1]
    B, Cin, H, W, _, _ = _conv_operands("conv3x3_winograd", x, Cout, 3, 3, 1, 1, scale, shift, residual)
    if tuple(U.shape) != (16, Cin, Cout):
        raise RuntimeError("U must be f32[16, Cin, Cout] = [16, %d, %d], got %s" % (Cin, Cout, tuple(U.shape)))
    y = torch.empty((B, Cout, H, W), dtype=_f32, device=x.device)
    _work("di2p_conv3x3_winograd", B * Cout * Cin * 16 * ((H + 1) // 2) * ((W + 1) // 2))
    call("di2p_conv3x3_winograd", ptr(x), ptr(U), ptr(scale), ptr(shift), ptr(residual), ptr(y), B, Cin, H, W, Cout, int(bool(relu)), stream())
    return y


def maxpool3x3s2(x):
    require_cuda(x)
    B, C, H, W = x.shape
    y = torch.empty((B, C, (H - 1) // 2 + 1, (W - 1) // 2 + 1), dtype=_f32, device=x.device)
    call("di2p_maxpool3x3s2", ptr(x), ptr(y), B, C, H, W, stream())
    return y


def global_avgpool(x):
    require_cuda(x)
    B, C, H, W = x.shape
    y = torch.empty((B, C, 1, 1), dtype=_f32, device=x.device)
    call("di2p_global_avgpool", ptr(x), ptr(y), B, C, H * W, stream())
    return y


def _dbl3(v):
    a = (ctypes.c_double * 3)()
    for i in range(3):
        a[i] = float(v[i])
    return a


def initial_guess(points64, labels):
    require_cuda(points64, labels)
    F, _, N = points64.shape
    yaw0 = torch.empty((F,), dtype=_f64, device=points64.device)
    labels_out = torch.empty_like(labels)
    has_inside = torch.empty((F,), dtype=_i32, device=points64.device)
    call("di2p_initial_guess", ptr(points64), ptr(labels), ptr(yaw0), ptr(labels_out), ptr(has_inside), F, N, stream())
    return yaw0, labels_out, has_inside


def solve_batched(points, labels, K, init_y, init_T, H, W, lb, ub, max_iter, is_2d, yaw0=None, sweeps=None, workspace=None):
    require_cuda(points, labels, K, init_y, init_T, yaw0, workspace)
    _chk(labels, _i32, "labels")
    _chk(K, _f64, "K")
    _chk(init_y, _f64, "init_y")
    _chk(init_T, _f64, "init_T")
    F, _, N = points.shape
    R = init_y.shape[1]
    npar = 4 if is_2d else 6
    params = torch.empty((F, R, npar), dtype=_f64, device=points.device)
    cost = torch.empty((F, R), dtype=_f64, device=points.device)
    iters = torch.empty((F, R), dtype=_i32, device=points.device)
    name = "di2p_solve_batched" if points.dtype == _f64 else "di2p_solve_batched_f32"
    if points.dtype not in (_f64, _f32):
        raise RuntimeError("points must be float64 or float32")
    need = _lib.load().di2p_solve_workspace_bytes(F, R, N)
    if workspace is None:
        ws = torch.empty((need,), dtype=torch.uint8, device=points.device)
    else:
        ws = workspace
        _chk(ws, torch.uint8, "workspace")
        if ws.device != points.device:
            raise RuntimeError("workspace must be on the points' device")
        if ws.numel() < need:
            raise RuntimeError("workspace has %d bytes, di2p_solve_workspace_bytes(%d, %d, %d) = %d" % (ws.numel(), F, R, N, need))
    call(name, ptr(points), ptr(labels), ptr(K), ptr(init_y), ptr(init_T), ptr(yaw0), float(H), float(W), _dbl3(lb),
         _dbl3(ub), int(max_iter), int(bool(is_2d)), F, R, N, ptr(params), ptr(cost), ptr(iters), ptr(sweeps), ptr(ws), stream())
    return params, cost, iters


def select_best(params, cost, is_2d, has_inside=None):
    require_cuda(params, cost, has_inside)
    F, R = cost.shape
    best = torch.empty((F,), dtype=_i32, device=cost.device)
    P = torch.empty((F, 4, 4), dtype=_f64, device=cost.device)
    bc = torch.empty((F,), dtype=_f64, device=cost.device)
    call("di2p_select_best", ptr(params), ptr(cost), ptr(has_inside), int(bool(is_2d)), F, R, ptr(best), ptr(P), ptr(bc), stream())
    return best, P, bc


def solver_residuals(points64, labels, K, params, H, W, is_2d):
    require_cuda(points64, labels, K, params)
    F, _, N = points64.shape
    res = torch.empty((F, 3 * N), dtype=_f64, device=points64.device)
    counts = torch.empty((F,), dtype=_i32, device=points64.device)
    cost = torch.empty((F,), dtype=_f64, device=points64.device)
    call("di2p_solver_residuals", ptr(points64), ptr(labels), ptr(K), ptr(params), float(H), float(W), int(bool(is_2d)),
         F, N, ptr(res), ptr(counts), ptr(cost), stream())
    return res, counts, cost

# ... 99 lines not shown
```

### deepi2p_amd/pipeline.py

```python
import time

import torch

from . import ops

INPUT_NAMES = ("pc", "intensity", "sn", "node_a", "node_b", "img")
K_NAME = "K"
P_NAME, MASK_NAME = "P", "frame_mask"
VISUALIZE = (None, "registration", "classification", "both")


class Slot:

    def __init__(self, index, stream):
        self.index, self.stream = index, stream
        self.devs, self.cur, self.host = [{}], 0, {}
        self.graphs = {}
        self.set_done = [torch.cuda.Event(), torch.cuda.Event()]
        self.done = torch.cuda.Event(enable_timing=True)
        self.start = torch.cuda.Event(enable_timing=True)
        self.outputs = None
        self.busy = False
        self.host_flat, self.dev_flats = None, []
        self.copy_bytes = None
# ... 132 lines not shown
                                 "or build an executor for that shape" % (k, tuple(host_batch[k].shape), tuple(slot.host[k].shape)))
        if self.evaluate:
            self._validate_truth(slot, host_batch)

    def _validate_truth(self, slot, host_batch):
        B = slot.host[MASK_NAME].shape[0]
        if P_NAME not in host_batch:
            raise ValueError("evaluate=True: the host batch has no ground-truth pose %r ([B,3,4] or [B,4,4])" % P_NAME)
        if tuple(host_batch[P_NAME].shape) not in ((B, 3, 4), (B, 4, 4)):
            raise ValueError("evaluate=True: %r must be [%d,3,4] or [%d,4,4], got %s" % (P_NAME, B, B, tuple(host_batch[P_NAME].shape)))
        if MASK_NAME in host_batch and tuple(host_batch[MASK_NAME].shape) != (B,):
            raise ValueError("evaluate=True: %r must be i32 [%d], got %s" % (MASK_NAME, B, tuple(host_batch[MASK_NAME].shape)))

    def _stage(self, slot, host_batch):
        for k in INPUT_NAMES:
            slot.host[k].copy_(host_batch[k])
        if K_NAME in host_batch:
            slot.host[K_NAME].copy_(host_batch[K_NAME])
        else:
            slot.host[K_NAME].copy_(self._K64_host)
        if self.evaluate:
            self._stage_truth(slot, host_batch)

    def _stage_truth(self, slot, host_batch):
        P = slot.host[P_NAME]
        P.copy_(torch.eye(4, dtype=torch.float64))
        if P_NAME in host_batch:
            gt = torch.as_tensor(host_batch[P_NAME])
            P[:, :gt.shape[1]].copy_(gt)
        if MASK_NAME in host_batch:
            slot.host[MASK_NAME].copy_(torch.as_tensor(host_batch[MASK_NAME]))
        else:
            slot.host[MASK_NAME].fill_(1)

    def _stage_example(self, slot, example_batch):
        self._stage(slot, {k: example_batch[k] for k in INPUT_NAMES + (P_NAME, MASK_NAME) if k in example_batch})

    def _slot_ready(self, slot):
        """Called once per slot when its buffers exist."""

    def _step(self, slot, with_h2d):
        if with_h2d:
            slot.copy_in()
        d = slot.dev
        if self.step_fn is not None:
            return self.step_fn(slot, d)
        return self._solve_part(slot, self._net_part(slot))

    def _net_part(self, slot):
        d = slot.dev
        if self.pnp:
            coarse, fine = self.mm.detector.predict_labels(d["pc"], d["intensity"], d["sn"], d["node_a"], d["node_b"], d["img"])
            return {"pred": coarse, "fine_pred": fine}
        logits = self.mm.detector(d["pc"], d["intensity"], d["sn"], d["node_a"], d["node_b"], d["img"])
        coarse = logits[0] if isinstance(logits, tuple) else logits
        net = {"pred": ops.argmax_channels(coarse)}
        if isinstance(logits, tuple):
            net["fine_pred"] = ops.argmax_channels(logits[1])
        return net

    def _solve_part(self, slot, net):
        d = slot.dev
        if self.pnp:
            coarse, fine = self.labels_override if self.labels_override is not None else (net["pred"], net["fine_pred"])
            out = self.pipe(d["pc"], coarse, fine, d[K_NAME], self.restarts)
            out.update(net)
            return self._finish(slot, out)
        labels = self.labels_override if self.labels_override is not None else net["pred"]
        kw = {"confidence": True} if self.confidence else {}
        out = self.pipe(d["pc"], labels, d[K_NAME], self.restarts, **kw)
        out.update(net)
        return self._finish(slot, out)

    def _finish(self, slot, out):
        if self.evaluate:
            out = self._eval_part(slot, out)
        return out if self.visualize is None else self._vis_part(slot, out)

    def _eval_truth(self, slot):
        d = slot.dev
        return d[P_NAME], d[P_NAME].to(torch.float32), d[K_NAME].to(torch.float32), d[MASK_NAME]

    def _eval_part(self, slot, out):
        from . import evaluation, prep
        d = slot.dev
        P_gt, P32, K32, mask = self._eval_truth(slot)
        fine_scale = 1.0 / self.pipe.scale if self.pnp else 32
        if self.visualize in ("classification", "both"):
            coarse_gt, fine_gt, slot.vis_pxpy = prep.project_labels(d["pc"], P32, K32, self.pipe.H, self.pipe.W, fine_scale, want_pxpy=True)
        else:
            coarse_gt, fine_gt = prep.project_labels(d["pc"], P32, K32, self.pipe.H, self.pipe.W, fine_scale)
        fine_pred = out.get("fine_pred")
        accuracy = prep.label_accuracy(out["pred"], coarse_gt, fine_pred, fine_gt if fine_pred is not None else None)
        rte, rre, flags = evaluation.pose_errors(out["P"], P_gt, None if self.pnp else out["cost"], frame=getattr(self.pipe, "frame", "cam"))
        slot.eval_acc.update(rte, rre, flags, mask, accuracy)
        out.update(rte=rte, rre=rre, flags=flags, accuracy=accuracy, coarse_gt=coarse_gt, fine_gt=fine_gt)
        return out

    def _vis_part(self, slot, out):
        from . import evaluation, visualization
        d = slot.dev
        if "registration" in slot.vis:
            pc, P = d["pc"], out["P"]
            if getattr(self.pipe, "enu", False):
                pc, P = evaluation.enu2cam_points(pc), out["P_cam"]
            out["vis_registration"] = visualization.registration_overlay_into(pc, P, d[K_NAME], out["pred"], d["img"], *slot.vis["registration"])
        if "classification" in slot.vis:
            canvas, workspace = slot.vis["classification"]
            fine_pred = out.get("fine_pred")
# ... 254 lines not shown
```

### deepi2p_amd/registration.py

```python
import math

import numpy as np
import torch

from . import ops

__version__ = "deepi2p_amd-1"


def _hip_dev():
    if not torch.cuda.is_available():
        raise RuntimeError("deepi2p_amd.registration needs a HIP device (there is no CPU fallback)")
    return torch.device("cuda", torch.cuda.current_device())


def solvePGivenK_batched(points, labels, K, init_y_angles, init_Ts, H, W, t_xyz_lower_bound, t_xyz_upper_bound,
                         max_iter, is_2d, return_all=False):
    dev = _hip_dev()
    pts = torch.as_tensor(np.ascontiguousarray(points, dtype=np.float64), device=dev).unsqueeze(0)
    lab = torch.as_tensor(np.ascontiguousarray(labels).astype(np.int32), device=dev).unsqueeze(0)
    Kt = torch.as_tensor(np.ascontiguousarray(K, dtype=np.float64), device=dev).reshape(1, 3, 3)
    ys = torch.as_tensor(np.ascontiguousarray(init_y_angles, dtype=np.float64), device=dev).reshape(1, -1)
    R = ys.shape[1]
    Ts = torch.as_tensor(np.ascontiguousarray(init_Ts, dtype=np.float64), device=dev).reshape(1, R, 3)
    params, cost, iters = ops.solve_batched(pts, lab, Kt, ys, Ts, H, W, t_xyz_lower_bound, t_xyz_upper_bound,
                                            max_iter, is_2d)
    npar = params.shape[2]
    _, P, _ = ops.select_best(params.view(R, 1, npar), cost.view(R, 1), is_2d)
    best, _, _ = ops.select_best(params, cost, is_2d)
    out = (P.cpu().numpy(), cost.view(-1).cpu().numpy(), int(best.item()))
    if return_all:
        out = out + (params.view(R, npar).cpu().numpy(), iters.view(-1).cpu().numpy())
    return out


def solvePGivenK(points, labels, K, init_y_angle, init_T, H, W, t_xyz_lower_bound, t_xyz_upper_bound, max_iter,
                 is_debug, is_2d):
    dev = _hip_dev()
    pts = torch.as_tensor(np.ascontiguousarray(points, dtype=np.float64), device=dev).unsqueeze(0)
    lab = torch.as_tensor(np.ascontiguousarray(labels).astype(np.int32), device=dev).unsqueeze(0)
    Kt = torch.as_tensor(np.ascontiguousarray(K, dtype=np.float64), device=dev).reshape(1, 3, 3)
    ys = torch.tensor([[float(init_y_angle)]], dtype=torch.float64, device=dev)
    Ts = torch.as_tensor(np.ascontiguousarray(init_T, dtype=np.float64), device=dev).reshape(1, 1, 3)
    params, cost, iters = ops.solve_batched(pts, lab, Kt, ys, Ts, H, W, t_xyz_lower_bound, t_xyz_upper_bound,
                                            max_iter, is_2d)
    _, P, _ = ops.select_best(params, cost, is_2d)
    res, counts, fcost = ops.solver_residuals(pts, lab, Kt, params.view(1, -1), H, W, is_2d)
    n = int(counts.item())
    if is_debug:
        print("deepi2p_amd solvePGivenK: iterations=%d final_cost=%.6g" % (int(iters.item()), float(fcost.item())))
    return P[0].cpu().numpy(), float(fcost.item()), res[0, :n].cpu().numpy()


def get_P_diff(P_pred_np, P_gt_np):
    from scipy.spatial.transform import Rotation
    P_diff = np.dot(np.linalg.inv(P_pred_np), P_gt_np)
    t_diff = np.linalg.norm(P_diff[0:3, 3])
    angles = Rotation.from_matrix(P_diff[0:3, 0:3]).as_euler("xzy", degrees=True)
# ... 48 lines not shown
def solve_P_random_perturb(pc_np, coarse_predictions_np, K_np, H, W, init_t_amplitude, init_y_angle, ry_sigma,
                           t_lowerbound, t_upperbound, iteration_num, is_2d, thread_num=None, rng=None,
                           restarts=None, max_iter=500):
    if restarts is None:
        ys, Ts = restart_list(init_y_angle, ry_sigma, init_t_amplitude, iteration_num, thread_num, rng)
    else:
        ys, Ts = restarts
    if len(ys) == 0:
        return None, 1e20, None
    P, cost, best, params, _ = solvePGivenK_batched(pc_np, coarse_predictions_np, K_np, ys, Ts, H, W, t_lowerbound,
                                                    t_upperbound, max_iter, is_2d, return_all=True)
    dev = _hip_dev()
    pts = torch.as_tensor(np.ascontiguousarray(pc_np, dtype=np.float64), device=dev).unsqueeze(0)
    lab = torch.as_tensor(np.ascontiguousarray(coarse_predictions_np).astype(np.int32), device=dev).unsqueeze(0)
    Kt = torch.as_tensor(np.ascontiguousarray(K_np, dtype=np.float64), device=dev).reshape(1, 3, 3)
    res, counts, _ = ops.solver_residuals(pts, lab, Kt, torch.as_tensor(params[best:best + 1], device=dev), H, W, is_2d)
    return P[best], float(cost[best]), res[0, :int(counts.item())].cpu().numpy()


class RegistrationPipeline:
    CONFIDENCE_KEYS = ("info", "grad", "cov", "cov_status", "free_mask", "sigma_t", "sigma_r", "active", "agree", "finite", "gap")

    def __init__(self, H, W, R=60, ry_sigma=10 * math.pi / 180, init_t_amplitude=10.0,
                 t_lowerbound=(-5, -0.1, -10), t_upperbound=(5, 0.1, 10), max_iter=500, is_2d=True, seed=0, frame="cam",
                 confidence=False, agree_tol=(2.0, 5.0)):
        from . import evaluation
        self.enu, self.frame = bool(evaluation.check_frame(frame)), frame
        self.confidence = bool(confidence)
        self.agree_tol = (float(agree_tol[0]), float(agree_tol[1]))
        self._convert = {}
        self.H, self.W, self.R = H, W, R
        self.ry_sigma, self.amp = ry_sigma, init_t_amplitude
        self.lb, self.ub = list(t_lowerbound), list(t_upperbound)
        self.max_iter, self.is_2d = max_iter, is_2d
        self.rng = np.random.default_rng(seed)

    def draw(self, F, device):
        noise, Ts = draw_restarts(self.rng, self.R, self.ry_sigma, self.amp, F=F)
        return (torch.as_tensor(noise, dtype=torch.float64, device=device),
                torch.as_tensor(Ts, dtype=torch.float64, device=device))

    def draw_on_device(self, F, device, seed):
        noise = torch.empty((F, self.R), dtype=torch.float64, device=device)
        Ts = torch.empty((F, self.R, 3), dtype=torch.float64, device=device)
        ops.call("di2p_draw_restarts", int(seed), F, self.R, float(self.ry_sigma), float(self.amp), ops.ptr(noise), ops.ptr(Ts),
                 ops.stream())
        return noise, Ts

    def __call__(self, pc_f32, labels_i32, K_f64, restarts, confidence=None):
        F, _, N = pc_f32.shape
        if self.enu:
            from . import evaluation
            pc_f32 = evaluation.enu2cam_points(pc_f32)
        pts64 = torch.empty((F, 3, N), dtype=torch.float64, device=pc_f32.device)
        ops.call("di2p_f32_to_f64", ops.ptr(pc_f32), ops.ptr(pts64), F * 3 * N, ops.stream())
        yaw0, lab_front, has_inside = ops.initial_guess(pts64, labels_i32)
        noise, Ts = restarts
        sweeps = torch.empty(noise.shape, dtype=torch.int32, device=pc_f32.device)
        params, cost, iters = ops.solve_batched(pc_f32, lab_front, K_f64, noise, Ts, self.H, self.W, self.lb, self.ub,
                                                self.max_iter, self.is_2d, yaw0=yaw0, sweeps=sweeps)
        best, P, bc = ops.select_best(params, cost, self.is_2d, has_inside=has_inside)
        out = dict(P=P, cost=bc, best=best, yaw0=yaw0, costs=cost, iters=iters, sweeps=sweeps, params=params, labels_front=lab_front)
        if self.enu:
            out["P_cam"], out["P"] = P, compose_convert(self._convert, P)
        if self.confidence if confidence is None else confidence:
            out.update(self._confidence(pc_f32, lab_front, K_f64, params, cost, best, has_inside))
        return out

    def _confidence(self, pc_f32, lab_front, K_f64, params, cost, best, has_inside):
        x = ops.gather_best_params(params, best, self.is_2d)
        info, grad, _, active = ops.pose_information(pc_f32, lab_front, K_f64, x, self.H, self.W, self.is_2d)
        cov, free_mask, status, sigma_t, sigma_r = ops.pose_covariance(info, x, self.lb, self.ub, self.is_2d, has_inside=has_inside)
        finite, agree, gap = ops.restart_consensus(params, cost, best, self.is_2d, self.agree_tol[0], self.agree_tol[1], has_inside=has_inside)
        return dict(info=info, grad=grad, cov=cov, cov_status=status, free_mask=free_mask, sigma_t=sigma_t, sigma_r=sigma_r, active=active,
                    agree=agree, finite=finite, gap=gap)


def compose_convert(cache, P_cam):
    key = (P_cam.device, P_cam.shape[0])
    if key not in cache:
        from . import evaluation
        cache[key] = evaluation.convert_matrices(P_cam.shape[0], P_cam.device)
    P = torch.empty_like(P_cam)
    ops.call("di2p_compose_poses", ops.ptr(P_cam), ops.ptr(cache[key]), P_cam.shape[0], ops.ptr(P), ops.stream())
    return P
```

### include/deepi2p_hip.h

```cpp
#ifndef DEEPI2P_HIP_H
#define DEEPI2P_HIP_H

#include <stdint.h>

#ifdef __cplusplus
extern "C" {
#endif

const char* di2p_last_error(void);
int di2p_version(void);
int di2p_set_option(const char* name, long long value);
long long di2p_get_option(const char* name);

int di2p_index_max_forward(const float* data, const int32_t* index, int32_t* max_idx,
                           int B, int C, int N, int K, void* workspace, void* stream);
int di2p_index_max_values(const float* data, const int32_t* index, const float* mask, float* max_val,
                          int32_t* max_idx, int B, int C, int N, int K, void* workspace, void* stream);

int di2p_ball_query_forward(const float* node_to_point_dist, int32_t* out_idx, float radius, int K,
                            int B, int M, int N, void* stream);

int di2p_knn_nodes(const float* query, const float* nodes, int32_t* idx, float* weights,
                   int B, int Nq, int M, int k, void* stream);
int di2p_cluster_stats(const float* pc, const int32_t* knn_idx, int idx_stride, float* cluster_mean,
// ... 9 lines not shown

#define DI2P_MAX_SRC 3
#define DI2P_MAX_GK 16
enum { DI2P_SRC_DENSE = 0,
       DI2P_SRC_GATHER = 1,
       DI2P_SRC_GROUP = 2     };
typedef struct {
    const float* ptr;
    const int32_t* gidx;
    long long batch_stride;
    int row_stride;
    int channels;
    int mode;
    int group;
    int pad_;
} di2p_src_t;

typedef struct {
    const float* scale;
    const float* shift;
    const float* batch_bias;
    int relu;
    int group_max;
    const float* g_table[2];
    const int32_t* g_idx[2];
    const float* g_w[2];
    int g_nodes[2];
    int g_k[2];
    int transpose_out;
    float* group_max_out;
    void* planes_out;
} di2p_epilogue_t;

int di2p_pointwise_gemm(const di2p_src_t* srcs_host, int n_src, const float* Wt, float* Y,
                        int B, int M, int K, int N, const di2p_epilogue_t* epi_host, void* stream);
long long di2p_bf16x3_packed_bytes(int K, int M);
int di2p_bf16x3_pack(const float* Wt, int K, int M, void* Wp, void* stream);
int di2p_bf16x3_pack_conv3x3(const float* W, int Cout, int Cin, int dgrad, void* Wp, void* stream);
int di2p_pointwise_gemm_x3(const di2p_src_t* srcs_host, int n_src, const void* Wp, float* Y,
                           int B, int M, int K, int N, const di2p_epilogue_t* epi_host, void* stream);
long long di2p_bf16x3_planes_bytes(int B, int C, int N);
int di2p_pointwise_gemm_x3p(const void* planes, const void* Wp, float* Y,
                            int B, int M, int K, int N, const di2p_epilogue_t* epi_host, void* stream);

int di2p_point_head(const di2p_src_t* srcs_host, int n_src, const float* W0t, int K0, const di2p_epilogue_t* epi0_host,
                    const float* W1t, const float* scale1, const float* shift1, int relu1,
                    const float* W2t, const float* scale2, const float* shift2, int relu2,
                    float* out, int B, int M, int P, int N, void* stream);

int di2p_point_chain(const di2p_src_t* srcs_host, int n_src, const float* W0t, int K0, const di2p_epilogue_t* epi0_host,
                     const float* W1t, const float* scale1, const float* shift1, int relu1, const float* W2t,
                     const float* scale2, const float* shift2, int relu2, float* Y, int B, int M, int N, void* stream);

int di2p_batch_gemv(const float* Wt, int M, int k0, const float* v, int Kv, float* out, int B, void* stream);
int di2p_batch_gemv2(const float* Wt, int M, int k0, const float* v0, int Kv0, int k1, const float* v1, int Kv1,
                     float* out, int B, void* stream);

int di2p_attention_pool(const float* feat, const float* score, float* out, int B, int C, int HW, int Mn, void* stream);

int di2p_conv2d(const float* x, const float* Wt, const float* scale, const float* shift,
                const float* residual, float* y, int B, int Cin, int H, int W, int Cout,
                int KH, int KW, int stride, int pad, int relu, int tap_major, void* stream);
int di2p_conv2d_ws(const float* x, const float* Wt, const float* scale, const float* shift,
                   const float* residual, float* y, int B, int Cin, int H, int W, int Cout,
                   int KH, int KW, int stride, int pad, int relu, int tap_major,
                   void* workspace, long long workspace_bytes, void* stream);
long long di2p_conv2d_workspace_bytes(int B, int Cin, int H, int W, int Cout, int KH, int KW, int stride, int pad,
                                      int tap_major);
int di2p_winograd_weight_transform(const float* weight, float* U, int Cin, int Cout, void* stream);
int di2p_winograd_weight_transform_dgrad(const float* weight, float* U, int Cin_g, int Cout_g, void* stream);
int di2p_conv3x3_winograd(const float* x, const float* U, const float* scale, const float* shift, const float* residual, float* y, int B,
                          int Cin, int H, int W, int Cout, int relu, void* stream);
int di2p_pointwise_route(int M, int K, int N, int B, int dense, int wt_aligned, int32_t* out);
int di2p_conv2d_route(int B, int Cin, int H, int W, int Cout, int KH, int KW, int stride, int pad, int tap_major, int x_aligned,
                      int wt_aligned, long long workspace_bytes, int32_t* out);
int di2p_winograd_route(int B, int Cin, int H, int W, int Cout, int32_t* out);
int di2p_point_chain_route(int M, int K0, int layers, int B, int N, int cus, int32_t* out);
int di2p_point_head_route(int K0, int n_src, int c0, int reg_range, int g33, int B, int N, int cus, int32_t* out);
typedef struct {
    const float* src[2]; long long batch_stride[2]; int row_stride[2]; int channels[2];
    const void* W0p; const void* W1p; const float* scale_shift; int relu0, relu1;
    const float* tab[2]; const int32_t* idx[2]; const float* w[2]; int nodes[2];
    const float* W2t; const float* scale2; const float* shift2; int relu2, P;
} di2p_head_x3_t;
long long di2p_head_x3_packed_bytes(int K);
int di2p_head_x3_pack(const float* Wt, int K, void* Wp, void* stream);
int di2p_point_head_x3(const di2p_head_x3_t* h, float* out, int B, int N, void* stream);
typedef struct {
    const float* y0; long long batch_stride; int row_stride; int K;
    const void* W1p; const float* scale1; const float* shift1; int relu1;
    const void* W2p; const float* scale2; const float* shift2; int P;
    float* scores; int32_t* coarse; int32_t* fine;
} di2p_head_labels_x3_t;
long long di2p_head_labels_x3_packed_bytes(int K, int P);
int di2p_head_labels_x3_pack(const float* Wt, int K, int P, void* Wp, void* stream);
int di2p_point_head_labels_x3(const di2p_head_labels_x3_t* h, int B, int N, void* stream);
int di2p_conv3x3_x3_supported(int B, int Cin, int H, int W, int Cout, int stride, int cfg);
int di2p_conv3x3_x3_plan(int B, int Cin, int H, int W, int Cout, int stride, int cfg, int32_t* out);
int di2p_conv3x3_x3(const float* x, const void* Wp, const float* scale, const float* shift, const float* residual, float* y, int B,
                    int Cin, int H, int W, int Cout, int stride, int relu, const void* Wp_ds, const float* scale_ds,
                    const float* shift_ds, float* y_ds, int cfg, void* stream);
int di2p_stem_pack(const float* weight, float* Wp, void* stream);
int di2p_conv7x7s2_stem(const float* x, const float* Wp, const float* scale, const float* shift, float* y, int B, int H, int W, int relu,
                        void* stream);
int di2p_maxpool3x3s2(const float* x, float* y, int B, int C, int H, int W, void* stream);
long long di2p_stem_x3_packed_bytes(void);
int di2p_stem_x3_pack(const float* weight, void* Wp, void* stream);
int di2p_stem_x3_supported(int H, int W);
int di2p_stem_x3(const float* x, const void* Wp, const float* scale, const float* shift, float* y, int B, int H, int W, void* stream);
int di2p_global_avgpool(const float* x, float* y, int B, int C, int HW, void* stream);
int di2p_channel_max(const float* x, float* y, int B, int C, int N, void* stream);

int di2p_initial_guess(const double* points, const int32_t* labels, double* yaw0, int32_t* labels_out,
                       int32_t* has_inside, int F, int N, void* stream);
int di2p_solve_batched(const double* points, const int32_t* labels, const double* K,
                       const double* init_y, const double* init_T, const double* yaw0,
                       double H, double W, const double* lb_host, const double* ub_host,
                       int max_iter, int is_2d, int F, int R, int N,
                       double* params, double* cost, int32_t* iters, int32_t* sweeps , void* workspace, void* stream);
int di2p_solve_batched_f32(const float* points, const int32_t* labels, const double* K,
                           const double* init_y, const double* init_T, const double* yaw0,
                           double H, double W, const double* lb_host, const double* ub_host,
                           int max_iter, int is_2d, int F, int R, int N,
                           double* params, double* cost, int32_t* iters, int32_t* sweeps , void* workspace, void* stream);
long long di2p_solve_workspace_bytes(int F, int R, int N);
void di2p_solver_set_profile_buffer(void* buf);
int di2p_select_best(const double* params, const double* cost, const int32_t* has_inside, int is_2d,
                     int F, int R, int32_t* best, double* P, double* best_cost, void* stream);
int di2p_solver_residuals(const double* points, const int32_t* labels, const double* K,
                          const double* params, double H, double W, int is_2d, int F, int N,
                          double* residuals, int32_t* counts, double* cost, void* stream);

int di2p_farthest_point_sampling(const float* pts, const int32_t* init_idx, int32_t* idx_out, float* nodes_out,
                                 int B, int M, int k, void* stream);
int di2p_gather_points(const float* src, const int32_t* idx, float* out, int B, int C, int Nsrc, int Nout, void* stream);
int di2p_project_labels(const float* pc, const float* P, int p_rows, const float* K, float H, float W, float fine_scale,
                        int32_t* coarse, int32_t* fine, float* pxpy, int B, int N, void* stream);
int di2p_label_accuracy(const int32_t* coarse_pred, const int32_t* coarse_gt, const int32_t* fine_pred,
                        const int32_t* fine_gt, float* out, int B, int N, void* stream);
int di2p_pack_pc_label(const float* pc, const int32_t* coarse_pred, const int32_t* coarse_gt, const int32_t* fine_pred,
                       const int32_t* fine_gt, double* out, int B, int N, void* stream);

long long di2p_pnp_workspace_bytes(int F, int N, int iters);
int di2p_pnp_pack(const float* pc, const int32_t* coarse, const int32_t* fine, const float* pixels, int W_fine, int F, int N,
                  float* corr, int32_t* n_corr, void* stream);
int di2p_pnp_ransac(const float* pc, const int32_t* coarse, const int32_t* fine, const float* pixels,
                    const double* K_scaled, int W_fine, const int32_t* samples, int iters, double reproj_err,
                    int refine_rounds, int refine_iters, int F, int N, double* P_out, double* outlier_ratio, int32_t* n_inliers,
                    int32_t* n_corr, int32_t* best, void* workspace, void* stream);
int di2p_pnp_ransac_epnp(const float* pc, const int32_t* coarse, const int32_t* fine, const float* pixels,
                         const double* K_scaled, int W_fine, const int32_t* samples, int iters, double reproj_err, int F, int N,
                         double* P_out, double* outlier_ratio, int32_t* n_inliers, int32_t* n_corr, int32_t* best,
                         void* workspace, void* stream);

int di2p_f32_to_f64(const float* in, double* out, long long n, void* stream);

int di2p_draw_restarts(unsigned long long seed, int F, int R, double ry_sigma, double t_amplitude, double* ry_noise,
                       double* init_T, void* stream);
long long di2p_random_choice_workspace_bytes(int B, int n_src);
int di2p_random_choice(unsigned long long seed, int stream_id, int B, int n_src, int n_out, int32_t* idx_out, void* workspace,
                       void* stream);

long long di2p_random_choice_ragged_workspace_bytes(int B, int max_src);
int di2p_random_choice_ragged(unsigned long long seed, int stream_id, int B, const int32_t* offsets, int max_src, int n_out, int32_t* idx_out,
                              void* workspace, void* stream);

long long di2p_scan_prep_workspace_bytes(int B, int cap);
// ... 154 lines not shown
```

Before: 5152.

## Fuse point input build, head argmax, batched gemvs, and f32 initial guess

Adds four default-on paths. The point-input construction (centering by cluster mean, intensity, normals) is folded into the first point-chain layer. The head kernel writes argmax labels directly. Several batch gemvs become one multi-segment launch. The initial guess reads f32 points directly. Together these aim to cut launches, intermediate tensors and the f32-to-f64 conversion pass, at the cost of more kernel variants and a possible precision difference in the initial guess.

```diff
diff --git a/deepi2p_amd/_lib.py b/deepi2p_amd/_lib.py
--- a/deepi2p_amd/_lib.py
+++ b/deepi2p_amd/_lib.py
@@ -31,6 +31,11 @@
                 ("W0p", c_void_p), ("W1p", c_void_p), ("scale_shift", c_void_p), ("relu0", c_int), ("relu1", c_int),
                 ("tab", c_void_p * 2), ("idx", c_void_p * 2), ("w", c_void_p * 2), ("nodes", c_int * 2),
                 ("W2t", c_void_p), ("scale2", c_void_p), ("shift2", c_void_p), ("relu2", c_int), ("P", c_int)]
+
+
+class GemvSegT(ctypes.Structure):
+    _fields_ = [("Wt", c_void_p), ("M", c_int), ("k0", c_int), ("v0", c_void_p), ("Kv0", c_int), ("k1", c_int), ("v1", c_void_p), ("Kv1", c_int),
+                ("out", c_void_p)]
 
 
 class HeadLabelsX3T(ctypes.Structure):
@@ -67,17 +72,21 @@
     "di2p_bf16x3_pack_conv3x3": [c_void_p, c_int, c_int, c_int, c_void_p, c_void_p],
     "di2p_batch_gemv": [c_void_p, c_int, c_int, c_void_p, c_int, c_void_p, c_int, c_void_p],
     "di2p_batch_gemv2": [c_void_p, c_int, c_int, c_void_p, c_int, c_int, c_void_p, c_int, c_void_p, c_int, c_void_p],
+    "di2p_batch_gemv_multi": [ctypes.POINTER(GemvSegT), c_int, c_int, c_void_p],
     "di2p_attention_pool": [c_void_p, c_void_p, c_void_p, c_int, c_int, c_int, c_int, c_void_p],
     "di2p_point_head": [c_void_p, c_int, c_void_p, c_int, c_void_p, c_void_p, c_void_p, c_void_p, c_int, c_void_p, c_void_p,
                         c_void_p, c_int, c_void_p, c_int, c_int, c_int, c_int, c_void_p],
     "di2p_point_chain": [c_void_p, c_int, c_void_p, c_int, c_void_p, c_void_p, c_void_p, c_void_p, c_int, c_void_p, c_void_p,
                          c_void_p, c_int, c_void_p, c_int, c_int, c_int, c_void_p],
+    "di2p_point_chain_input": [c_void_p] * 5 + [c_int, c_void_p, c_void_p, c_void_p, c_void_p, c_void_p, c_void_p, c_int, c_void_p, c_void_p,
+                               c_void_p, c_int, c_void_p, c_int, c_int, c_int, c_void_p],
     "di2p_conv2d": [c_void_p] * 6 + [c_int] * 11 + [c_void_p],
     "di2p_conv2d_ws": [c_void_p] * 6 + [c_int] * 11 + [c_void_p, c_ll, c_void_p],
     "di2p_maxpool3x3s2": [c_void_p, c_void_p, c_int, c_int, c_int, c_int, c_void_p],
     "di2p_global_avgpool": [c_void_p, c_void_p, c_int, c_int, c_int, c_void_p],
     "di2p_channel_max": [c_void_p, c_void_p, c_int, c_int, c_int, c_void_p],
     "di2p_initial_guess": [c_void_p] * 5 + [c_int, c_int, c_void_p],
+    "di2p_initial_guess_f32": [c_void_p] * 5 + [c_int, c_int, c_void_p],
     "di2p_solve_batched": [c_void_p] * 6 + [c_double, c_double, ctypes.POINTER(c_double), ctypes.POINTER(c_double)]
                           + [c_int] * 5 + [c_void_p, c_void_p, c_void_p, c_void_p, c_void_p, c_void_p],
     "di2p_solve_batched_f32": [c_void_p] * 6 + [c_double, c_double, ctypes.POINTER(c_double), ctypes.POINTER(c_double)]
@@ -115,6 +124,7 @@
     "di2p_stem_x3_supported": [c_int, c_int],
     "di2p_stem_x3": [c_void_p] * 5 + [c_int] * 3 + [c_void_p],
     "di2p_point_head_x3": [ctypes.POINTER(HeadX3T), c_void_p, c_int, c_int, c_void_p],
+    "di2p_point_head_x3_labels": [ctypes.POINTER(HeadX3T), c_void_p, c_void_p, c_int, c_int, c_void_p],
     "di2p_head_labels_x3_pack": [c_void_p, c_int, c_int, c_void_p, c_void_p],
     "di2p_point_head_labels_x3": [ctypes.POINTER(HeadLabelsX3T), c_int, c_int, c_void_p],
     "di2p_bn_train_forward": [c_void_p] * 9 + [c_float, c_float, c_int, c_int, c_int, c_int, c_void_p, c_void_p],
@@ -245,16 +255,17 @@
 WORK = None
 
 
-def call(name, *args):
+def call(name, *args, book=None):
     lib = load()
-    rec = TIMED is not None and name in TIMED
+    book = book or name
+    rec = TIMED is not None and book in TIMED
     if rec:
         e0, e1 = torch.cuda.Event(enable_timing=True), torch.cuda.Event(enable_timing=True)
         e0.record()
     rc = getattr(lib, name)(*args)
     if rec:
         e1.record()
-        TIMED[name].append((e0, e1, TIMED_TAG))
+        TIMED[book].append((e0, e1, TIMED_TAG))
     if rc != 0:
         raise DeepI2PHipError("%s failed (%d): %s" % (name, rc, lib.di2p_last_error().decode()))
 
diff --git a/deepi2p_amd/csrc/common.h b/deepi2p_amd/csrc/common.h
--- a/deepi2p_amd/csrc/common.h
+++ b/deepi2p_amd/csrc/common.h
@@ -56,7 +56,11 @@
     X(BN_UNFUSED, "bn_unfused", "DI2P_BN_UNFUSED", 0)                              \
     X(PW_X3_PLANES, "pw_x3_planes", "DI2P_PW_X3_PLANES", 1)                        \
     X(CONV_DGRAD_DENSE, "conv_dgrad_dense", "DI2P_CONV_DGRAD_DENSE", 0)            \
-    X(RC_TILE64, "rc_tile64", "DI2P_RC_TILE64", 0)
+    X(RC_TILE64, "rc_tile64", "DI2P_RC_TILE64", 0)                                 \
+    X(GUESS_F32, "guess_f32", "DI2P_GUESS_F32", 1)                                 \
+    X(GEMV_MULTI, "gemv_multi", "DI2P_GEMV_MULTI", 1)                              \
+    X(HEAD_LABELS, "head_labels", "DI2P_HEAD_LABELS", 1)                           \
+    X(CHAIN_INPUT, "chain_input", "DI2P_CHAIN_INPUT", 1)
 enum Di2pOption {
 #define DI2P_OPT_ENUM(ID, NAME, ENV, DEF) DI2P_OPT_##ID,
     DI2P_OPTIONS(DI2P_OPT_ENUM)
diff --git a/deepi2p_amd/csrc/gemm.hip b/deepi2p_amd/csrc/gemm.hip
--- a/deepi2p_amd/csrc/gemm.hip
+++ b/deepi2p_amd/csrc/gemm.hip
@@ -476,9 +476,15 @@
 #ifndef DI2P_CHAIN_WAVES
 #define DI2P_CHAIN_WAVES 2
 #endif
-template <int M, int KS0, int NL, int TN>
+struct ChainPointIn {
+    const float* pc; const float* intensity; const float* sn; const float* cluster_mean; const int* min_idx;
+    float* centers;
+    int nodes;
+};
+template <int M, int KS0, int NL, int TN, bool PIN = false>
 __global__ __launch_bounds__(256) __attribute__((amdgpu_waves_per_eu(DI2P_CHAIN_WAVES, 8))) void point_chain_kernel(const float* __restrict__ X, long long x_bs, int x_rs, const float* __restrict__ W0t,
-                                                           int K0, EpiDev e0, ChainTail tl, float* __restrict__ Y, int N, int nblk, int total) {
+                                                           int K0, EpiDev e0, ChainTail tl, float* __restrict__ Y, int N, int nblk, int total, ChainPointIn pin) {
+    static_assert(!PIN || KS0 == 4, "the point input has seven rows");
     constexpr int TM = M / 32, KS = M / 2, KSMAX = KS0 > KS ? KS0 : KS;
     extern __shared__ __attribute__((aligned(16))) float lds[];
     float* w0 = lds;
@@ -505,8 +511,31 @@
     e2.scale = tl.sc2 ? ss + 4 * M : nullptr; e2.shift = tl.sh2 ? ss + 5 * M : nullptr; e2.relu = tl.relu2; e2.group_max = 1;
 
     float fn[TN][KS0];
-    auto request = [&](int g) {
+    auto request = [&](int g, bool first_visit) {
         const int fb = g / nblk, blk = g - fb * nblk;
+        if constexpr (PIN) {
+            const long long fN = (long long)fb * N;
+            const float* p = pin.pc + 3 * fN;
+            const float* nrm = pin.sn + 3 * fN;
+            const float* cm = pin.cluster_mean + (long long)fb * 3 * pin.nodes;
+            float* ctr_out = pin.centers + 3 * fN;
+#pragma unroll
+            for (int j = 0; j < TN; ++j) {
+                const int nj = (blk * TN + j) * 32 + l31, col = min(nj, N - 1);
+                const bool store = first_visit && nj < N;
+                const int node = pin.min_idx[fN + col];
+                const float c01 = cm[half * pin.nodes + node], c2 = cm[2 * pin.nodes + node];
+                if (store) ctr_out[(long long)half * N + col] = c01;
+                if (store && half == 0) ctr_out[2 * (long long)N + col] = c2;
+                fn[j][0] = __fsub_rn(p[(long long)half * N + col], c01);
+                const float zi = half ? pin.intensity[fN + col] : p[2 * (long long)N + col];
+                fn[j][1] = half ? zi : __fsub_rn(zi, c2);
+                fn[j][2] = nrm[(long long)half * N + col];
+                const float s2 = nrm[2 * (long long)N + col];
+                fn[j][3] = half ? 0.0f : s2;
+            }
+            return;
+        }
         const float* Xb = X + (long long)fb * x_bs;
 #pragma unroll
         for (int s = 0; s < KS0; ++s) {
@@ -519,7 +548,7 @@
         }
     };
     const int g0 = blockIdx.x * 4 + wave, stride = gridDim.x * 4;
-    if (g0 < total) request(g0);
+    if (g0 < total) request(g0, true);
     for (int g = g0; g < total; g += stride) {
         const int b = g / nblk, blk = g - b * nblk;
         EpiPointwise ep0{e0, nullptr, b, M, N}, ep1{e1, nullptr, b, M, N}, ep2{e2, nullptr, b, M, N};
@@ -531,7 +560,7 @@
         for (int j = 0; j < TN; ++j)
 #pragma unroll
             for (int s = 0; s < KS0; ++s) f[j][s] = fn[j][s];
-        request(min(g + stride, total - 1));
+        request(min(g + stride, total - 1), g + stride < total);
         f32x16 acc[TM][TN];
         auto zero = [&]() {
 #pragma unroll
@@ -783,6 +812,40 @@
     const int b = blockIdx.y;
     const int lane = threadIdx.x & 63, slice = threadIdx.x >> 6;
     const int m = blockIdx.x * 64 + lane;
+    const int mc = min(m, M - 1);
+    part[0][slice][lane] = gemv_slice(Wt, M, mc, k0, v + (long long)b * Kv, Kv, slice);
+    if (v1) part[1][slice][lane] = gemv_slice(Wt, M, mc, k1, v1 + (long long)b * Kv1, Kv1, slice);
+    __syncthreads();
+    if (slice == 0 && m < M) {
+        float r = (part[0][0][lane] + part[0][1][lane]) + (part[0][2][lane] + part[0][3][lane]);
+        if (v1) r += (part[1][0][lane] + part[1][1][lane]) + (part[1][2][lane] + part[1][3][lane]);
+        out[(long long)b * M + m] = r;
+    }
+}
+
+struct GemvMulti {
+    di2p_gemv_seg_t seg[DI2P_MAX_GEMV_SEG];
+    int first[DI2P_MAX_GEMV_SEG + 1];
+    int n;
+};
+
+__global__ __launch_bounds__(256) void batch_gemv_multi_kernel(const GemvMulti a) {
+    __shared__ float part[2][4][64];
+    int si = 0;
+#pragma unroll
+    for (int i = 1; i < DI2P_MAX_GEMV_SEG; ++i)
+        if (i < a.n && (int)blockIdx.x >= a.first[i]) si = i;
+    const float* Wt = a.seg[0].Wt; const float* v = a.seg[0].v0; const float* v1 = a.seg[0].v1; float* out = a.seg[0].out;
+    int M = a.seg[0].M, k0 = a.seg[0].k0, Kv = a.seg[0].Kv0, k1 = a.seg[0].k1, Kv1 = a.seg[0].Kv1, first = a.first[0];
+#pragma unroll
+    for (int i = 1; i < DI2P_MAX_GEMV_SEG; ++i)
+        if (si == i) {
+            Wt = a.seg[i].Wt; v = a.seg[i].v0; v1 = a.seg[i].v1; out = a.seg[i].out;
+            M = a.seg[i].M; k0 = a.seg[i].k0; Kv = a.seg[i].Kv0; k1 = a.seg[i].k1; Kv1 = a.seg[i].Kv1; first = a.first[i];
+        }
+    const int b = blockIdx.y;
+    const int lane = threadIdx.x & 63, slice = threadIdx.x >> 6;
+    const int m = ((int)blockIdx.x - first) * 64 + lane;
     const int mc = min(m, M - 1);
     part[0][slice][lane] = gemv_slice(Wt, M, mc, k0, v + (long long)b * Kv, Kv, slice);
     if (v1) part[1][slice][lane] = gemv_slice(Wt, M, mc, k1, v1 + (long long)b * Kv1, Kv1, slice);
@@ -1405,7 +1468,7 @@
     do {                                                                                                                            \
         const size_t lds = (size_t)(2 * (KS0) * (MM) + ((NL) - 1) * (MM) * (MM) + 6 * (MM)) * sizeof(float);                        \
         hipLaunchKernelGGL((point_chain_kernel<MM, KS0, NL, TN>), dim3(rt.wgs), dim3(256), lds, st, X, x_bs, x_rs, W0t, K0, e, tl, Y, N, \
-                           rt.nblk, (int)rt.total);                                                                                 \
+                           rt.nblk, (int)rt.total, ChainPointIn{});                                                                 \
     } while (0)
     const bool three = rt.layers == 3;
     if (M == 32) {
@@ -1419,6 +1482,28 @@
     DI2P_RETURN_LAUNCH();
 }
 
+extern "C" int di2p_point_chain_input(const float* pc, const float* intensity, const float* sn, const float* cluster_mean, const int32_t* min_idx,
+                                      int nodes, float* pc_centers, const float* W0t, const di2p_epilogue_t* epi0, const float* W1t,
+                                      const float* scale1, const float* shift1, int relu1, const float* W2t, const float* scale2,
+                                      const float* shift2, int relu2, float* Y, int B, int M, int N, void* stream) {
+    DI2P_CHECK_ARG(W0t && W1t && W2t && epi0, "fused chain on the point input: three layers");
+    DI2P_CHECK_ARG(M == 32, "fused chain on the point input: width 32 (use di2p_build_point_input + the separate layers otherwise)");
+    DI2P_CHECK_ARG(B >= 0 && N >= 1 && nodes >= 1, "bad size");
+    DI2P_CHECK_ARG(epi0->group_max <= 1 && !epi0->transpose_out && !epi0->planes_out, "fused chain: layer 0 takes scale/shift/relu/bias/gathered only");
+    if (B == 0) return 0;
+    DI2P_CHECK_ARG(pc && intensity && sn && cluster_mean && min_idx && pc_centers && Y, "null pointer");
+    EpiDev e;
+    if (pw_epilogue(__func__, epi0, nullptr, M, N, false, e)) return -1;
+    ChainTail tl{W1t, scale1, shift1, W2t, scale2, shift2, relu1, relu2};
+    const ChainPointIn pin{pc, intensity, sn, cluster_mean, min_idx, pc_centers, nodes};
+    const ChainRoute rt = chain_route(M, 7, true, B, N, di2p_cu_count());
+    DI2P_CHECK_ARG(rt.total < (1ll << 30), "too many column blocks");
+    const size_t lds = (size_t)(2 * 4 * 32 + 2 * 32 * 32 + 6 * 32) * sizeof(float);
+    hipLaunchKernelGGL((point_chain_kernel<32, 4, 3, DI2P_CHAIN_TN32, true>), dim3(rt.wgs), dim3(256), lds, (hipStream_t)stream, (const float*)nullptr, 0ll, 0,
+                       W0t, 7, e, tl, Y, N, rt.nblk, (int)rt.total, pin);
+    DI2P_RETURN_LAUNCH();
+}
+
 extern "C" int di2p_point_chain_route(int M, int K0, int layers, int B, int N, int cus, int32_t* out) {
     DI2P_CHECK_ARG(out && (M == 32 || M == 64) && K0 >= 1 && K0 <= M && (layers == 2 || layers == 3) && B >= 1 && N >= 1 && cus >= 1, "bad args");
     const ChainRoute rt = chain_route(M, K0, layers == 3, B, N, cus);
@@ -1448,6 +1533,26 @@
     DI2P_CHECK_ARG(Wt && v0 && v1 && out && M >= 1 && Kv0 >= 1 && Kv1 >= 1 && k0 >= 0 && k1 >= 0 && B >= 0, "bad args");
     if (B == 0) return 0;
     hipLaunchKernelGGL(batch_gemv_kernel, dim3(di2p_cdiv(M, 64), B), dim3(256), 0, (hipStream_t)stream, Wt, M, k0, v0, Kv0, k1, v1, Kv1, out);
+    DI2P_RETURN_LAUNCH();
+}
+
+extern "C" int di2p_batch_gemv_multi(const di2p_gemv_seg_t* segs, int n_seg, int B, void* stream) {
+    DI2P_CHECK_ARG(segs && n_seg >= 1 && n_seg <= DI2P_MAX_GEMV_SEG && B >= 0, "1..DI2P_MAX_GEMV_SEG segments");
+    GemvMulti a{};
+    a.n = n_seg;
+    long long blocks = 0;
+    for (int i = 0; i < n_seg; ++i) {
+        const di2p_gemv_seg_t& s = segs[i];
+        DI2P_CHECK_ARG(s.Wt && s.v0 && s.out && s.M >= 1 && s.Kv0 >= 1 && s.k0 >= 0, "bad segment");
+        DI2P_CHECK_ARG(!s.v1 || (s.Kv1 >= 1 && s.k1 >= 0), "bad second vector of a segment");
+        a.seg[i] = s;
+        a.first[i] = (int)blocks;
+        blocks += di2p_cdiv(s.M, 64);
+        DI2P_CHECK_ARG(blocks < (1ll << 30), "too many output channels");
+    }
+    for (int i = n_seg; i <= DI2P_MAX_GEMV_SEG; ++i) a.first[i] = (int)blocks;
+    if (B == 0) return 0;
+    hipLaunchKernelGGL(batch_gemv_multi_kernel, dim3((unsigned)blocks, B), dim3(256), 0, (hipStream_t)stream, a);
     DI2P_RETURN_LAUNCH();
 }
 
diff --git a/deepi2p_amd/csrc/head_x3.hip b/deepi2p_amd/csrc/head_x3.hip
--- a/deepi2p_amd/csrc/head_x3.hip
+++ b/deepi2p_amd/csrc/head_x3.hip
@@ -19,6 +19,7 @@
     const float* tab[2]; const int* idx[2]; const float* gw[2]; int nodes[2];
     const float* W2t; const float* sc2; const float* sh2;
     float* out;
+    int* labels;
     int relu0, relu1, relu2, P, N, nblk, total, parts;
 };
 
@@ -249,6 +250,8 @@
                 }
                 if (LEAN) asm volatile("" : "+v"(part[0]), "+v"(part[1]), "+v"(part[2]), "+v"(part[3]));
             }
+        float best = 0.0f;
+        int best_p = 0;
 #pragma unroll
         for (int p = 0; p < 4; ++p) {
             const float other = __builtin_bit_cast(float, __builtin_amdgcn_ds_bpermute((lane ^ 32) * 4, __builtin_bit_cast(int, part[p])));
@@ -258,8 +261,11 @@
                 if (a.sh2) o += a.sh2[p];
                 if (a.relu2) o = fmaxf(o, 0.0f);
                 if (n < a.N && hq == 0 && live) a.out[((long long)fb * a.P + p) * a.N + n] = o;
-            }
-        }
+                if (p == 0) best = o;
+                else if (best == best && (o != o || o > best)) { best = o; best_p = p; }
+            }
+        }
+        if (a.labels && n < a.N && hq == 0 && live) a.labels[(long long)fb * a.N + n] = best_p;
     }
 }
 
@@ -297,17 +303,25 @@
     DI2P_RETURN_LAUNCH();
 }
 
+static int point_head_x3(const char* who, const di2p_head_x3_t* hd, float* out, int32_t* labels, int B, int N, void* stream);
 extern "C" int di2p_point_head_x3(const di2p_head_x3_t* hd, float* out, int B, int N, void* stream) {
-    DI2P_CHECK_ARG(hd && out, "null pointer");
-    DI2P_CHECK_ARG(B >= 0 && N >= 1, "bad size");
-    DI2P_CHECK_ARG(hd->src[0] && hd->src[1] && hd->W0p && hd->W1p && hd->scale_shift && hd->W2t, "null operand");
-    DI2P_CHECK_ARG(hd->channels[0] >= 16 && hd->channels[0] % 16 == 0 && hd->channels[1] >= 16 && hd->channels[1] % 16 == 0, "source channels must be multiples of 16");
-    DI2P_CHECK_ARG(hd->P >= 1 && hd->P <= 4, "1..4 outputs");
-    for (int t = 0; t < 2; ++t) DI2P_CHECK_ARG(hd->tab[t] && hd->idx[t] && hd->nodes[t] >= 1, "both gathered tables (3 neighbours each) are required");
-    DI2P_CHECK_ARG(((uintptr_t)hd->W0p & 15) == 0 && ((uintptr_t)hd->W1p & 15) == 0 && ((uintptr_t)hd->tab[0] & 15) == 0 && ((uintptr_t)hd->tab[1] & 15) == 0 &&
+    return point_head_x3(__func__, hd, out, nullptr, B, N, stream);
+}
+extern "C" int di2p_point_head_x3_labels(const di2p_head_x3_t* hd, float* out, int32_t* labels_out, int B, int N, void* stream) {
+    return point_head_x3(__func__, hd, out, labels_out, B, N, stream);
+}
+#define DI2P_HX_CHECK(cond, msg) do { if (!(cond)) { di2p_set_error("%s: %s", who, msg); return -1; } } while (0)
+static int point_head_x3(const char* who, const di2p_head_x3_t* hd, float* out, int32_t* labels, int B, int N, void* stream) {
+    DI2P_HX_CHECK(hd && out, "null pointer");
+    DI2P_HX_CHECK(B >= 0 && N >= 1, "bad size");
+    DI2P_HX_CHECK(hd->src[0] && hd->src[1] && hd->W0p && hd->W1p && hd->scale_shift && hd->W2t, "null operand");
+    DI2P_HX_CHECK(hd->channels[0] >= 16 && hd->channels[0] % 16 == 0 && hd->channels[1] >= 16 && hd->channels[1] % 16 == 0, "source channels must be multiples of 16");
+    DI2P_HX_CHECK(hd->P >= 1 && hd->P <= 4, "1..4 outputs");
+    for (int t = 0; t < 2; ++t) DI2P_HX_CHECK(hd->tab[t] && hd->idx[t] && hd->nodes[t] >= 1, "both gathered tables (3 neighbours each) are required");
+    DI2P_HX_CHECK(((uintptr_t)hd->W0p & 15) == 0 && ((uintptr_t)hd->W1p & 15) == 0 && ((uintptr_t)hd->tab[0] & 15) == 0 && ((uintptr_t)hd->tab[1] & 15) == 0 &&
                    ((uintptr_t)hd->scale_shift & 15) == 0, "16-byte alignment of the packed weights, the tables and the scale / shift rows");
     for (int t = 0; t < 2; ++t)
-        DI2P_CHECK_ARG((long long)hd->channels[t] * hd->row_stride[t] * 4 < (1ll << 31), "per-frame source extent must fit 31 bits");
+        DI2P_HX_CHECK((long long)hd->channels[t] * hd->row_stride[t] * 4 < (1ll << 31), "per-frame source extent must fit 31 bits");
     if (B == 0) return 0;
     HxArgs a{};
     for (int t = 0; t < 2; ++t) {
@@ -316,29 +330,35 @@
     }
     a.c0 = hd->channels[0]; a.K0 = hd->channels[0] + hd->channels[1];
     a.W0p = (const u32x4_t*)hd->W0p; a.W1p = (const u32x4_t*)hd->W1p; a.ss = hd->scale_shift;
-    a.W2t = hd->W2t; a.sc2 = hd->scale2; a.sh2 = hd->shift2; a.out = out;
+    a.W2t = hd->W2t; a.sc2 = hd->scale2; a.sh2 = hd->shift2; a.out = out; a.labels = labels;
     a.relu0 = hd->relu0; a.relu1 = hd->relu1; a.relu2 = hd->relu2; a.P = hd->P; a.N = N;
     a.nblk = di2p_cdiv(N, 32); a.total = B * a.nblk;
     hipStream_t st = (hipStream_t)stream;
     const size_t lds_small = (size_t)8 * HX_M * sizeof(float);
     const size_t lds_tab = lds_small + (size_t)(hd->nodes[0] + hd->nodes[1]) * HX_TROW * sizeof(float);
     const long long opt = di2p_opt(DI2P_OPT_HEAD_X3_TAB);
-    DI2P_CHECK_ARG(a.K0 == 96, "this build instantiates the head for 96 dense channels (32 + 64: first_pointnet + second_pointnet)");
+    DI2P_HX_CHECK(a.K0 == 96, "this build instantiates the head for 96 dense channels (32 + 64: first_pointnet + second_pointnet)");
     if (opt != 0 && lds_tab <= 160 * 1024) {
         const int cus = di2p_cu_count();
         int parts = di2p_cdiv(cus, B);
         while (parts > 1 && a.nblk < parts * 16) --parts;
         a.parts = parts;
         if (opt == 2) {
-            if (di2p_allow_dynamic_lds((const void*)point_head_x3_kernel<true, 6, 4, 1, false, true>, lds_tab, __func__)) return -1;
+            if (di2p_allow_dynamic_lds((const void*)point_head_x3_kernel<true, 6, 4, 1, false, true>, lds_tab, who)) return -1;
             hipLaunchKernelGGL((point_head_x3_kernel<true, 6, 4, 1, false, true>), dim3(B * parts), dim3(256), lds_tab, st, a);
         } else {
-            if (di2p_allow_dynamic_lds((const void*)point_head_x3_kernel<true, 6, 8, 2, false, false, true>, lds_tab, __func__)) return -1;
+            if (di2p_allow_dynamic_lds((const void*)point_head_x3_kernel<true, 6, 8, 2, false, false, true>, lds_tab, who)) return -1;
             hipLaunchKernelGGL((point_head_x3_kernel<true, 6, 8, 2, false, false, true>), dim3(B * parts), dim3(512), lds_tab, st, a);
         }
     } else {
         const int grid = (int)(a.total / 4 < 1ll * di2p_cu_count() ? di2p_cdiv(a.total, 4) : di2p_cu_count());
         hipLaunchKernelGGL((point_head_x3_kernel<false, 6, 4, 1, false, true>), dim3(grid), dim3(256), lds_small, st, a);
     }
-    DI2P_RETURN_LAUNCH();
-}
+    const hipError_t err = hipGetLastError();
+    if (err != hipSuccess) {
+        di2p_set_error("%s: launch failed: %s", who, hipGetErrorString(err));
+        return (int)err;
+    }
+    return 0;
+}
+#undef DI2P_HX_CHECK
diff --git a/deepi2p_amd/csrc/solver_aux.hip b/deepi2p_amd/csrc/solver_aux.hip
--- a/deepi2p_amd/csrc/solver_aux.hip
+++ b/deepi2p_amd/csrc/solver_aux.hip
@@ -34,17 +34,18 @@
     best_cost[f] = cost[(long long)f * R + bi];
 }
 
-__global__ __launch_bounds__(1024) void initial_guess_kernel(const double* __restrict__ points, const int* __restrict__ labels,
+template <typename T>
+__global__ __launch_bounds__(1024) void initial_guess_kernel(const T* __restrict__ points, const int* __restrict__ labels,
                                                              double* __restrict__ yaw0, int* __restrict__ labels_out,
                                                              int* __restrict__ has_inside, int N) {
     __shared__ double s_a[1024], s_b[1024], s_c[1024];
     const int f = blockIdx.x, tid = threadIdx.x;
-    const double* px = points + (long long)f * 3 * N;
-    const double* pz = px + 2 * (long long)N;
+    const T* px = points + (long long)f * 3 * N;
+    const T* pz = px + 2 * (long long)N;
     const int* lab = labels + (long long)f * N;
     double sx = 0, sz = 0, cnt = 0;
     for (int n = tid; n < N; n += 1024)
-        if (lab[n] == 1) { sx += px[n]; sz += pz[n]; cnt += 1.0; }
+        if (lab[n] == 1) { sx += (double)px[n]; sz += (double)pz[n]; cnt += 1.0; }
     s_a[tid] = sx; s_b[tid] = sz; s_c[tid] = cnt;
     __syncthreads();
     for (int o = 512; o > 0; o >>= 1) {
@@ -66,7 +67,7 @@
     const double c = cos(a), s = sin(a);
     double zmin = __builtin_inf();
     for (int n = tid; n < N; n += 1024)
-        if (lab[n] == 1) zmin = fmin(zmin, -s * px[n] + c * pz[n]);
+        if (lab[n] == 1) zmin = fmin(zmin, -s * (double)px[n] + c * (double)pz[n]);
     s_a[tid] = zmin;
     __syncthreads();
     for (int o = 512; o > 0; o >>= 1) {
@@ -75,7 +76,7 @@
     }
     const double thr = s_a[0] - 10.0;
     for (int n = tid; n < N; n += 1024) {
-        const double zr = -s * px[n] + c * pz[n];
+        const double zr = -s * (double)px[n] + c * (double)pz[n];
         labels_out[(long long)f * N + n] = zr > thr ? lab[n] : -1;
     }
     if (tid == 0) { yaw0[f] = a; has_inside[f] = 1; }
@@ -373,7 +374,15 @@
                                   int32_t* has_inside, int F, int N, void* stream) {
     DI2P_CHECK_ARG(points && labels && yaw0 && labels_out && has_inside && F >= 0 && N >= 0, "bad args");
     if (F == 0) return 0;
-    hipLaunchKernelGGL(initial_guess_kernel, dim3(F), dim3(1024), 0, (hipStream_t)stream, points, labels, yaw0, labels_out, has_inside, N);
+    hipLaunchKernelGGL(initial_guess_kernel<double>, dim3(F), dim3(1024), 0, (hipStream_t)stream, points, labels, yaw0, labels_out, has_inside, N);
+    DI2P_RETURN_LAUNCH();
+}
+
+extern "C" int di2p_initial_guess_f32(const float* points, const int32_t* labels, double* yaw0, int32_t* labels_out,
+                                      int32_t* has_inside, int F, int N, void* stream) {
+    DI2P_CHECK_ARG(points && labels && yaw0 && labels_out && has_inside && F >= 0 && N >= 0, "bad args");
+    if (F == 0) return 0;
+    hipLaunchKernelGGL(initial_guess_kernel<float>, dim3(F), dim3(1024), 0, (hipStream_t)stream, points, labels, yaw0, labels_out, has_inside, N);
     DI2P_RETURN_LAUNCH();
 }
 
diff --git a/deepi2p_amd/networks.py b/deepi2p_amd/networks.py
--- a/deepi2p_amd/networks.py
+++ b/deepi2p_amd/networks.py
@@ -205,8 +205,11 @@
         B, N, Ma, Mb = pc.size(0), pc.size(2), node_a.size(2), node_b.size(2)
         idx_a, w_a = ops.knn_nodes(pc, node_a, self.opt.k_interp_point_a, want_weights=True)
         cluster_mean, mask, min_idx = ops.cluster_stats(pc, idx_a, Ma)
-        pc_centers, aug = ops.build_point_input(pc, intensity, sn, cluster_mean, min_idx)
-        first = _run_pn(aug, p["first"])
+        if ops.point_chain_input_ok(p["first"]):
+            pc_centers, first = ops.point_chain_input(pc, intensity, sn, cluster_mean, min_idx, p["first"])
+        else:
+            pc_centers, aug = ops.build_point_input(pc, intensity, sn, cluster_mean, min_idx)
+            first = _run_pn(aug, p["first"])
         _, first_max = ops.index_max(first, min_idx, Ma, return_values=True, mask=mask)
         Ch = first.shape[1]
         second = _run_split_pn([Src(first)], (0, Ch), first_max, (Ch, 2 * Ch), min_idx, p["second"], N)
@@ -376,16 +379,30 @@
         return self._packed
 
     def forward(self, pc, intensity, sn, node_a, node_b, img):
+        return self._forward(pc, intensity, sn, node_a, node_b, img, False)[0]
+
+    def forward_labels(self, pc, intensity, sn, node_a, node_b, img):
+        out, labels = self._forward(pc, intensity, sn, node_a, node_b, img, bool(_lib.get_option("head_labels")))
+        if labels is None:
+            labels = ops.argmax_channels(out[0] if isinstance(out, tuple) else out)
+        return out, labels
+
+    def _forward(self, pc, intensity, sn, node_a, node_b, img, want_labels):
+        labels = None
         p, B, N, first, second, idx_a, idx_pb, gathered = self._trunk(pc, intensity, sn, node_a, node_b, img)
         Wt, sc, sh, act = p["per_point_pn"][0]
         M0 = Wt.shape[1]
         G_a, ex_w_a = gathered[0][0], gathered[0][2]
         G_b, w_pb = gathered[1][0], gathered[1][2]
         l1, l2 = p["per_point_pn"][1], p["per_point_pn"][2]
+        scores_are_coarse = l2[0].shape[1] == 2
         if ("head_x3" in p and self.fuse_head and _lib.get_option("head_x3") and first.shape[1] == 32 and second.shape[1] == 64
                 and idx_a.shape[-1] == 3 and idx_pb.shape[-1] == 3):
             scores = ops.point_head_x3(first, second, p["head_x3"],
-                                       [(G_a, idx_a.reshape(B, N, 3), ex_w_a), (G_b, idx_pb.reshape(B, N, 3), w_pb)], N)
+                                       [(G_a, idx_a.reshape(B, N, 3), ex_w_a), (G_b, idx_pb.reshape(B, N, 3), w_pb)], N,
+                                       want_labels=want_labels and scores_are_coarse)
+            if want_labels and scores_are_coarse:
+                scores, labels = scores
         elif M0 == 128 and l1[0].shape[1] == 128 and l2[0].shape[1] <= 4 and N % 4 == 0 and self.fuse_head:
             scores = ops.point_head([Src(first), Src(second)], (Wt[640:736], sc, sh, act), l1, l2, N, gathered=gathered)
         else:
@@ -393,12 +410,12 @@
             scores = _run_pn(h, p["per_point_pn"][1:], x3=False if M0 == 128 else None)
         coarse = scores[:, 0:2, :]
         if self.opt.is_fine_resolution:
-            return coarse, scores[:, 2:, :]
-        return coarse
+            return (coarse, scores[:, 2:, :]), labels
+        return coarse, labels
 
     def predict_labels(self, pc, intensity, sn, node_a, node_b, img, scores_out=None):
         if not self.opt.is_fine_resolution:
-            return ops.argmax_channels(self.forward(pc, intensity, sn, node_a, node_b, img)), None
+            return self.forward_labels(pc, intensity, sn, node_a, node_b, img)[1], None
         p, B, N, first, second, idx_a, idx_pb, gathered = self._trunk(pc, intensity, sn, node_a, node_b, img)
         Wt, sc, sh, act = p["per_point_pn"][0]
         M0 = Wt.shape[1]
@@ -420,20 +437,26 @@
         ig = iglob.view(B, -1)
         gf = global_feature.view(B, -1)
 
+        if _lib.get_option("gemv_multi"):
+            bias_b_att, bias_b_pn, bias_a_att = ops.batch_gemv_multi([(p["node_b_attention_pn"][0][0], 256, ig),
+                                                                      (p["node_b_pn"][0][0], 256, gf, 1280, ig),
+                                                                      (p["node_a_attention_pn"][0][0], 64, ig)])
+        else:
+            bias_b_att = bias_b_pn = bias_a_att = None
         Wt, sc, sh, act = p["node_b_attention_pn"][0]
         h = ops.pointwise_gemm([Src(node_b_features)], Wt[0:256], Wt.shape[1], Mb, scale=sc, shift=sh, relu=act,
-                               batch_bias=ops.batch_gemv(Wt, 256, ig))
+                               batch_bias=bias_b_att if bias_b_att is not None else ops.batch_gemv(Wt, 256, ig))
         score_b = _run_pn(h, p["node_b_attention_pn"][1:])
         w_s32 = ops.attention_pool(s32f, score_b)
         Wt, sc, sh, act = p["node_b_pn"][0]
-        bias = ops.batch_gemv2(Wt, 256, gf, 1280, ig)
+        bias = bias_b_pn if bias_b_pn is not None else ops.batch_gemv2(Wt, 256, gf, 1280, ig)
         h = ops.pointwise_gemm([Src(node_b_features), Src(w_s32)], p["node_b_pn_dense_Wt"], Wt.shape[1], Mb,
                                scale=sc, shift=sh, relu=act, batch_bias=bias)
         up_b = _run_pn(h, p["node_b_pn"][1:])
         idx_pb, w_pb = ops.knn_nodes(pc, node_b, self.opt.k_interp_point_b, want_weights=True)
         Wt, sc, sh, act = p["node_a_attention_pn"][0]
         h = ops.pointwise_gemm([Src(node_a_features)], Wt[0:64], Wt.shape[1], Ma, scale=sc, shift=sh, relu=act,
-                               batch_bias=ops.batch_gemv(Wt, 64, ig))
+                               batch_bias=bias_a_att if bias_a_att is not None else ops.batch_gemv(Wt, 64, ig))
         score_a = _run_pn(h, p["node_a_attention_pn"][1:])
         w_s16 = ops.attention_pool(s16f, score_a)
         idx_ab, w_ab = ops.knn_nodes(node_a, node_b, self.opt.k_interp_ab, want_weights=True)
@@ -528,18 +551,16 @@
         self.detector.eval()
 
     def inference_labels(self):
-        out = self.forward(self.pc, self.intensity, self.sn, self.node_a, self.node_b, self.img)
-        return ops.argmax_channels(out[0] if self.opt.is_fine_resolution else out)
+        return self.detector.forward_labels(self.pc, self.intensity, self.sn, self.node_a, self.node_b, self.img)[1]
 
     def inference_labels_fine(self):
         return self.detector.predict_labels(self.pc, self.intensity, self.sn, self.node_a, self.node_b, self.img)
 
     def inference_pass(self):
-        out = self.forward(self.pc, self.intensity, self.sn, self.node_a, self.node_b, self.img)
         if self.opt.is_fine_resolution:
-            coarse, fine = out
+            coarse, fine = self.forward(self.pc, self.intensity, self.sn, self.node_a, self.node_b, self.img)
             return ops.argmax_channels(coarse).long(), ops.argmax_channels(fine).long()
-        return ops.argmax_channels(out).long()
+        return self.inference_labels().long()
 
 
 class MMClassiferCoarse(MMClassifer):
diff --git a/deepi2p_amd/ops.py b/deepi2p_amd/ops.py
--- a/deepi2p_amd/ops.py
+++ b/deepi2p_amd/ops.py
@@ -398,7 +398,7 @@
     return Wp
 
 
-def point_head_x3(src0, src1, packed, gathered, N):
+def point_head_x3(src0, src1, packed, gathered, N, want_labels=False):
     require_cuda(src0, src1, packed["W0p"], packed["W1p"], packed["ss"], packed["W2t"], packed["sc2"], packed["sh2"])
     B = src0.shape[0]
     P = packed["W2t"].shape[1]
@@ -432,6 +432,10 @@
     h.W2t, h.scale2, h.shift2 = ptr(packed["W2t"]), ptr(packed["sc2"]), ptr(packed["sh2"])
     out = torch.empty((B, P, N), dtype=_f32, device=src0.device)
     _work("di2p_point_head_x3", B * N * ((src0.shape[1] + src1.shape[1]) * 128 + 128 * 128 + 128 * P))
+    if want_labels:
+        labels = torch.empty((B, N), dtype=_i32, device=src0.device)
+        call("di2p_point_head_x3_labels", ctypes.byref(h), ptr(out), ptr(labels), B, N, stream(), book="di2p_point_head_x3")
+        return out, labels
     call("di2p_point_head_x3", ctypes.byref(h), ptr(out), B, N, stream())
     return out
 
@@ -510,6 +514,40 @@
     return out
 
 
+def point_chain_input_ok(layers):
+    if len(layers) != 3 or _lib.get_option("pw_nochain") or not _lib.get_option("chain_input"):
+        return False
+    if tuple(layers[0][0].shape) != (7, 32) or any(tuple(l[0].shape) != (32, 32) for l in layers[1:]):
+        return False
+    return not any(l[0].requires_grad or not l[0].is_contiguous() or not l[0].is_cuda for l in layers)
+
+
+def point_chain_input(pc, intensity, sn, cluster_mean, min_idx, layers):
+    require_cuda(pc, intensity, sn, cluster_mean, min_idx)
+    for t, name in ((pc, "pc"), (intensity, "intensity"), (sn, "sn"), (cluster_mean, "cluster_mean")):
+        _chk(t, _f32, name)
+    _chk(min_idx, _i32, "min_idx")
+    _shape(pc, (None, 3, None), "pc", "f32[B, 3, N]")
+    B, _, N = pc.shape
+    _shape(intensity, (B, 1, N), "intensity", "f32[B, 1, N] for pc f32[B, 3, N]")
+    _shape(sn, (B, 3, N), "sn", "f32[B, 3, N] for pc f32[B, 3, N]")
+    _shape(cluster_mean, (B, 3, None), "cluster_mean", "f32[B, 3, M] for pc f32[B, 3, N]")
+    _shape(min_idx, (B, N), "min_idx", "i32[B, N] for pc f32[B, 3, N]")
+    (Wt0, sc0, sh0, act0), (Wt1, sc1, sh1, act1), (Wt2, sc2, sh2, act2) = layers
+    require_cuda(Wt0, Wt1, Wt2, sc0, sh0, sc1, sh1, sc2, sh2)
+    M = Wt0.shape[1]
+    e = EpilogueT()
+    e.scale, e.shift = ptr(sc0), ptr(sh0)
+    e.relu, e.group_max, e.transpose_out = int(bool(act0)), 1, 0
+    centers = torch.empty_like(pc)
+    out = torch.empty((B, M, N), dtype=_f32, device=pc.device)
+    _work("di2p_point_chain", B * N * (Wt0.shape[0] * M + 2 * M * M))
+    call("di2p_point_chain_input", ptr(pc), ptr(intensity), ptr(sn), ptr(cluster_mean), ptr(min_idx), cluster_mean.shape[2], ptr(centers),
+         ptr(Wt0), ctypes.byref(e), ptr(Wt1), ptr(sc1), ptr(sh1), int(bool(act1)), ptr(Wt2), ptr(sc2), ptr(sh2), int(bool(act2)), ptr(out),
+         B, M, N, stream(), book="di2p_point_chain")
+    return centers, out
+
+
 def batch_gemv(Wt, k0, v):
     require_cuda(Wt, v)
     B, Kv = v.shape
@@ -526,6 +564,32 @@
     out = torch.empty((B, M), dtype=_f32, device=Wt.device)
     call("di2p_batch_gemv2", ptr(Wt), M, int(k0), ptr(v0), v0.shape[1], int(k1), ptr(v1), v1.shape[1], ptr(out), B, stream())
     return out
+
+
+def batch_gemv_multi(segments):
+    if not 1 <= len(segments) <= 4:
+        raise RuntimeError("batch_gemv_multi takes 1..4 segments")
+    segs = (_lib.GemvSegT * len(segments))()
+    outs = []
+    B = segments[0][2].shape[0]
+    for s, seg in zip(segs, segments):
+        Wt, k0, v0 = seg[0], seg[1], seg[2]
+        k1, v1 = (seg[3], seg[4]) if len(seg) == 5 else (0, None)
+        require_cuda(Wt, v0, v1)
+        for t, name in ((Wt, "Wt"), (v0, "v0"), (v1, "v1")):
+            if t is not None:
+                _chk(t, _f32, "batch_gemv_multi " + name)
+        K, M = Wt.shape
+        for k, v in ((k0, v0), (k1, v1)):
+            if v is not None and (v.dim() != 2 or v.shape[0] != B or int(k) < 0 or int(k) + v.shape[1] > K):
+                raise RuntimeError("batch_gemv_multi: every vector must be f32[%d,Kv] with rows [k, k + Kv) inside Wt f32[%d,%d]" % (B, K, M))
+        out = torch.empty((B, M), dtype=_f32, device=Wt.device)
+        s.Wt, s.M, s.k0, s.v0, s.Kv0 = ptr(Wt), M, int(k0), ptr(v0), v0.shape[1]
+        s.k1, s.v1, s.Kv1 = int(k1), ptr(v1), (v1.shape[1] if v1 is not None else 0)
+        s.out = ptr(out)
+        outs.append(out)
+    call("di2p_batch_gemv_multi", segs, len(segments), B, stream())
+    return outs
 
 
 def attention_pool(feat, score):
@@ -793,13 +857,19 @@
     return a
 
 
-def initial_guess(points64, labels):
-    require_cuda(points64, labels)
-    F, _, N = points64.shape
-    yaw0 = torch.empty((F,), dtype=_f64, device=points64.device)
+def initial_guess(points, labels):
+    require_cuda(points, labels)
+    _chk(labels, _i32, "labels")
+    if points.dtype not in (_f64, _f32):
+        raise RuntimeError("points must be torch.float64 or torch.float32, got %s" % points.dtype)
+    _shape(points, (None, 3, None), "points", "[F, 3, N]")
+    F, _, N = points.shape
+    _shape(labels, (F, N), "labels", "i32[F, N] for points [F, 3, N]")
+    yaw0 = torch.empty((F,), dtype=_f64, device=points.device)
     labels_out = torch.empty_like(labels)
-    has_inside = torch.empty((F,), dtype=_i32, device=points64.device)
-    call("di2p_initial_guess", ptr(points64), ptr(labels), ptr(yaw0), ptr(labels_out), ptr(has_inside), F, N, stream())
+    has_inside = torch.empty((F,), dtype=_i32, device=points.device)
+    call("di2p_initial_guess" if points.dtype == _f64 else "di2p_initial_guess_f32", ptr(points), ptr(labels), ptr(yaw0), ptr(labels_out),
+         ptr(has_inside), F, N, stream())
     return yaw0, labels_out, has_inside
 
 
diff --git a/deepi2p_amd/pipeline.py b/deepi2p_amd/pipeline.py
--- a/deepi2p_amd/pipeline.py
+++ b/deepi2p_amd/pipeline.py
@@ -208,9 +208,8 @@
         if self.pnp:
             coarse, fine = self.mm.detector.predict_labels(d["pc"], d["intensity"], d["sn"], d["node_a"], d["node_b"], d["img"])
             return {"pred": coarse, "fine_pred": fine}
-        logits = self.mm.detector(d["pc"], d["intensity"], d["sn"], d["node_a"], d["node_b"], d["img"])
-        coarse = logits[0] if isinstance(logits, tuple) else logits
-        net = {"pred": ops.argmax_channels(coarse)}
+        logits, pred = self.mm.detector.forward_labels(d["pc"], d["intensity"], d["sn"], d["node_a"], d["node_b"], d["img"])
+        net = {"pred": pred}
         if isinstance(logits, tuple):
             net["fine_pred"] = ops.argmax_channels(logits[1])
         return net
diff --git a/deepi2p_amd/registration.py b/deepi2p_amd/registration.py
--- a/deepi2p_amd/registration.py
+++ b/deepi2p_amd/registration.py
@@ -3,7 +3,7 @@
 import numpy as np
 import torch
 
-from . import ops
+from . import _lib, ops
 
 __version__ = "deepi2p_amd-1"
 
@@ -158,9 +158,12 @@
         if self.enu:
             from . import evaluation
             pc_f32 = evaluation.enu2cam_points(pc_f32)
-        pts64 = torch.empty((F, 3, N), dtype=torch.float64, device=pc_f32.device)
-        ops.call("di2p_f32_to_f64", ops.ptr(pc_f32), ops.ptr(pts64), F * 3 * N, ops.stream())
-        yaw0, lab_front, has_inside = ops.initial_guess(pts64, labels_i32)
+        if _lib.get_option("guess_f32"):
+            yaw0, lab_front, has_inside = ops.initial_guess(pc_f32, labels_i32)
+        else:
+            pts64 = torch.empty((F, 3, N), dtype=torch.float64, device=pc_f32.device)
+            ops.call("di2p_f32_to_f64", ops.ptr(pc_f32), ops.ptr(pts64), F * 3 * N, ops.stream())
+            yaw0, lab_front, has_inside = ops.initial_guess(pts64, labels_i32)
         noise, Ts = restarts
         sweeps = torch.empty(noise.shape, dtype=torch.int32, device=pc_f32.device)
         params, cost, iters = ops.solve_batched(pc_f32, lab_front, K_f64, noise, Ts, self.H, self.W, self.lb, self.ub,
diff --git a/include/deepi2p_hip.h b/include/deepi2p_hip.h
--- a/include/deepi2p_hip.h
+++ b/include/deepi2p_hip.h
@@ -85,9 +85,21 @@
                      const float* W1t, const float* scale1, const float* shift1, int relu1, const float* W2t,
                      const float* scale2, const float* shift2, int relu2, float* Y, int B, int M, int N, void* stream);
 
+int di2p_point_chain_input(const float* pc, const float* intensity, const float* sn, const float* cluster_mean, const int32_t* min_idx,
+                           int nodes, float* pc_centers, const float* W0t, const di2p_epilogue_t* epi0_host, const float* W1t,
+                           const float* scale1, const float* shift1, int relu1, const float* W2t, const float* scale2,
+                           const float* shift2, int relu2, float* Y, int B, int M, int N, void* stream);
+
 int di2p_batch_gemv(const float* Wt, int M, int k0, const float* v, int Kv, float* out, int B, void* stream);
 int di2p_batch_gemv2(const float* Wt, int M, int k0, const float* v0, int Kv0, int k1, const float* v1, int Kv1,
                      float* out, int B, void* stream);
+#define DI2P_MAX_GEMV_SEG 4
+typedef struct {
+    const float* Wt; int M; int k0; const float* v0; int Kv0;
+    int k1; const float* v1; int Kv1;
+    float* out;
+} di2p_gemv_seg_t;
+int di2p_batch_gemv_multi(const di2p_gemv_seg_t* segs_host, int n_seg, int B, void* stream);
 
 int di2p_attention_pool(const float* feat, const float* score, float* out, int B, int C, int HW, int Mn, void* stream);
 
@@ -119,6 +131,7 @@
 long long di2p_head_x3_packed_bytes(int K);
 int di2p_head_x3_pack(const float* Wt, int K, void* Wp, void* stream);
 int di2p_point_head_x3(const di2p_head_x3_t* h, float* out, int B, int N, void* stream);
+int di2p_point_head_x3_labels(const di2p_head_x3_t* h, float* out, int32_t* labels_out, int B, int N, void* stream);
 typedef struct {
     const float* y0; long long batch_stride; int row_stride; int K;
     const void* W1p; const float* scale1; const float* shift1; int relu1;
@@ -146,6 +159,8 @@
 
 int di2p_initial_guess(const double* points, const int32_t* labels, double* yaw0, int32_t* labels_out,
                        int32_t* has_inside, int F, int N, void* stream);
+int di2p_initial_guess_f32(const float* points, const int32_t* labels, double* yaw0, int32_t* labels_out,
+                           int32_t* has_inside, int F, int N, void* stream);
 int di2p_solve_batched(const double* points, const int32_t* labels, const double* K,
                        const double* init_y, const double* init_T, const double* yaw0,
                        double H, double W, const double* lb_host, const double* ub_host,
```

New measurement: 5070. -1.6%, worse.
